# MasterVVK/qwen3-tts-axera-russian

Hardware: AMD Instinct MI355X
Metric: 12Hz codec-tokens/s (codec frames/s, 16 codes each) + RTF, Qwen3-TTS-0.6B (higher is better)
Workload: dtype f16 weights/KV, f32 accumulate (talker+CP); vocoder exact fp32 (f32 MFMA); 1 GPU; configs[2]/[3]: batch=32 mixed ru/en prompts per GPU, 64 frames/utterance/step (prefill + hipGraph decode loop), utterance-sharded DP over 1 GPU(s); batch_per_gpu=32

## Files before the change

### qwen3_tts_axera_russian_amd/csrc/q3_attn.hip

```cpp
#include "q3_kdev.h"

namespace q3 {

template <int MODE, int APRE>
__global__ void __launch_bounds__(1024) attn_kernel(AttnArgs a) {
    constexpr int D = 128;
    Q3_FETCH_ARGS("s"(a.qkv), "s"(a.ld), "s"(a.row0), "s"(a.q_norm), "s"(a.k_norm), "s"(a.eps), "s"(a.rope_cos), "s"(a.rope_sin),
                  "s"(a.slot), "s"(a.pos), "s"(a.slot_base), "s"(a.slot_stride), "s"(a.pos_base), "s"(a.pos_stride), "s"(a.kc),
                  "s"(a.vc), "s"(a.n_ctx), "s"(a.n_kv), "s"(a.n_heads), "s"(a.out), "s"(a.scale), "s"(a.valid_mod), "s"(a.valid_n));
    Q3_TL(30 + MODE);
    const int r = a.row0 + blockIdx.x, g = blockIdx.y;
    if (a.valid_mod > 0 && (r % a.valid_mod) >= a.valid_n) return;
    const int tid = threadIdx.x, lane = tid & 63, w = tid >> 6;
    const int nwv = blockDim.x >> 6;
    const int slot = a.slot ? uniform_load(a.slot + r) : a.slot_base + r * a.slot_stride;
    const int pos = a.pos ? uniform_load(a.pos + r) : a.pos_base + r * a.pos_stride;
    __shared__ float qs[2][D];
    __shared__ float knew[D], vnew[D];
    extern __shared__ __attribute__((aligned(16))) float dyn[];
    float* pm = dyn;
    float* pl = dyn + 2 * nwv;
    float* pacc = dyn + 4 * nwv;
    float* row = a.qkv + (size_t)r * a.ld;
    const size_t cbase = ((size_t)slot * a.n_kv + g) * (size_t)a.n_ctx * D;
    const int T = (MODE == ATTN_FUSED) ? pos : pos + 1;
    const int l16 = tid & 15, grp = tid >> 4, ngrp = blockDim.x >> 4;
    const half_t* kbase = a.kc + cbase;
    const half_t* vbase = a.vc + cbase;

    float x0 = 0.f, x1 = 0.f, gm0 = 1.f, gm1 = 1.f, cs = 1.f, sn = 0.f;
    if (MODE != ATTN_ATTEND && w < 4) {
        const float* src = w < 2 ? row + (size_t)(2 * g + w) * D
                         : w == 2 ? row + (size_t)(a.n_heads + g) * D
                                  : row + (size_t)(a.n_heads + a.n_kv + g) * D;
        x0 = src[lane];
        x1 = src[lane + 64];
        if (w < 3) {
            const float* gam = w < 2 ? a.q_norm : a.k_norm;
            gm0 = gam[lane];
            gm1 = gam[lane + 64];
            cs = a.rope_cos[(size_t)pos * 64 + lane];
            sn = a.rope_sin[(size_t)pos * 64 + lane];
        }
    }
    float qpre = 0.f;
    if (MODE == ATTN_ATTEND && tid < 2 * D) qpre = row[(size_t)(2 * g) * D + tid];
    h8 kpre[APRE], vpre[APRE];
    if (MODE != ATTN_PREP) {
#pragma unroll
        for (int i = 0; i < APRE; i++) {
            const int t = grp + i * ngrp;
            if (t < T) {
                kpre[i] = *(const h8*)(kbase + (size_t)t * D + l16 * 8);
                vpre[i] = *(const h8*)(vbase + (size_t)t * D + l16 * 8);
            }
        }
    }
    __builtin_amdgcn_sched_barrier(0);
    Q3_PH(0);

    if (MODE != ATTN_ATTEND) {
        if (w < 4) {
            if (w < 3) {
                float ss = wave_sum(x0 * x0 + x1 * x1);
                const float iv = 1.0f / sqrtf(ss / (float)D + a.eps);
                x0 = (x0 * iv) * gm0;
                x1 = (x1 * iv) * gm1;
                const float y0 = x0 * cs - x1 * sn;
                const float y1 = x1 * cs + x0 * sn;
                x0 = y0;
                x1 = y1;
            }
            if (w < 2) {
                if (MODE == ATTN_PREP) {
                    float* dst = row + (size_t)(2 * g + w) * D;
                    dst[lane] = x0;
                    dst[lane + 64] = x1;
                } else {
                    qs[w][lane] = x0;
                    qs[w][lane + 64] = x1;
                }
            } else {
                const half_t h0 = sat_half(x0), h1 = sat_half(x1);
                half_t* cd = (w == 2 ? a.kc : a.vc) + cbase + (size_t)pos * D;
                cd[lane] = h0;
                cd[lane + 64] = h1;
                float* nd = w == 2 ? knew : vnew;
                nd[lane] = (float)h0;
                nd[lane + 64] = (float)h1;
            }
        }
        if (MODE == ATTN_PREP) return;
    } else {
        if (tid < 2 * D) qs[tid / D][tid % D] = qpre;
    }
    __syncthreads();
    Q3_PH(1);

    float q0[8], q1[8];
#pragma unroll
    for (int j = 0; j < 8; j++) {
        q0[j] = qs[0][l16 * 8 + j] * a.scale;
        q1[j] = qs[1][l16 * 8 + j] * a.scale;
    }
    float m0 = -INFINITY, m1 = -INFINITY, l0 = 0.f, l1 = 0.f;
    float a0[8], a1[8];
#pragma unroll
    for (int j = 0; j < 8; j++) a0[j] = a1[j] = 0.f;

    auto step = [&](const h8& kk, const h8& vv) {
        float d0 = 0.f, d1 = 0.f;
#pragma unroll
        for (int j = 0; j < 8; j++) {
            const float kf = (float)kk[j];
            d0 += q0[j] * kf;
            d1 += q1[j] * kf;
        }
        group_sum_down2<16>(d0, d1);
        const float n0 = fmaxf(m0, d0), n1 = fmaxf(m1, d1);
        const float c0 = __expf(m0 - n0), c1 = __expf(m1 - n1);
        const float p0 = __expf(d0 - n0), p1 = __expf(d1 - n1);
        l0 = l0 * c0 + p0;
        l1 = l1 * c1 + p1;
#pragma unroll
        for (int j = 0; j < 8; j++) {
            const float vf = (float)vv[j];
            a0[j] = a0[j] * c0 + p0 * vf;
            a1[j] = a1[j] * c1 + p1 * vf;
        }
        m0 = n0;
        m1 = n1;
    };
#pragma unroll
    for (int i = 0; i < APRE; i++) {
        const int t = grp + i * ngrp;
        if (t < T) step(kpre[i], vpre[i]);
    }
#pragma unroll 2
    for (int t = grp + APRE * ngrp; t < T; t += ngrp) {
        const h8 kk = *(const h8*)(kbase + (size_t)t * D + l16 * 8);
        const h8 vv = *(const h8*)(vbase + (size_t)t * D + l16 * 8);
        step(kk, vv);
    }
    if (MODE == ATTN_FUSED && grp == 0) {
        h8 kk, vv;
#pragma unroll
        for (int j = 0; j < 8; j++) {
            kk[j] = (half_t)knew[l16 * 8 + j];
            vv[j] = (half_t)vnew[l16 * 8 + j];
        }
        step(kk, vv);
    }
    asm volatile("" ::"v"(a0[0]), "v"(l0));
    Q3_PH(2);
#pragma unroll
    for (int o = 16; o <= 32; o <<= 1) {
        const float om0 = __shfl_xor(m0, o, 64), om1 = __shfl_xor(m1, o, 64);
        const float ol0 = __shfl_xor(l0, o, 64), ol1 = __shfl_xor(l1, o, 64);
        const float n0 = fmaxf(m0, om0), n1 = fmaxf(m1, om1);
        const float c0 = (m0 == -INFINITY) ? 0.f : __expf(m0 - n0), d0 = (om0 == -INFINITY) ? 0.f : __expf(om0 - n0);
        const float c1 = (m1 == -INFINITY) ? 0.f : __expf(m1 - n1), d1 = (om1 == -INFINITY) ? 0.f : __expf(om1 - n1);
        l0 = l0 * c0 + ol0 * d0;
        l1 = l1 * c1 + ol1 * d1;
#pragma unroll
        for (int j = 0; j < 8; j++) {
            const float oa0 = __shfl_xor(a0[j], o, 64), oa1 = __shfl_xor(a1[j], o, 64);
            a0[j] = a0[j] * c0 + oa0 * d0;
            a1[j] = a1[j] * c1 + oa1 * d1;
        }
        m0 = n0;
        m1 = n1;
    }
    if (lane < 16) {
#pragma unroll
        for (int j = 0; j < 8; j++) {
            pacc[(w * 2 + 0) * D + lane * 8 + j] = a0[j];
            pacc[(w * 2 + 1) * D + lane * 8 + j] = a1[j];
        }
        if (lane == 0) {
            pm[w * 2 + 0] = m0;
            pm[w * 2 + 1] = m1;
            pl[w * 2 + 0] = l0;
            pl[w * 2 + 1] = l1;
        }
    }
    __syncthreads();
    Q3_PH(3);
    if (tid < 2 * D) {
        const int hh = tid / D, d = tid % D;
        float M = -INFINITY;
        for (int i = 0; i < nwv; i++) M = fmaxf(M, pm[i * 2 + hh]);
        float L = 0.f, o = 0.f;
        for (int i = 0; i < nwv; i++) {
            const float mi = pm[i * 2 + hh];
            const float c = (mi == -INFINITY) ? 0.f : __expf(mi - M);
            L += pl[i * 2 + hh] * c;
            o += pacc[(i * 2 + hh) * D + d] * c;
        }
        a.out[frag_idx(r, (2 * g + hh) * D + d, a.n_heads * D)] = sat_half(o / L);
    }
}

constexpr int ATTN_SHORT_MAX_T = 15;
static int g_attn_short = 1;
int set_attn_short(int on) { g_attn_short = on; return 0; }
__global__ void __launch_bounds__(256)
    attn_short_kernel(float* __restrict__ p_qkv, int p_ld, int p_row0, int p_n_heads, int p_n_kv,
                      const float* __restrict__ p_q_norm, const float* __restrict__ p_k_norm,
                      const float* __restrict__ p_rope_cos, const float* __restrict__ p_rope_sin, int p_pos_base,
                      int p_slot_base, AttnArgs a) {
    constexpr int D = 128, NE = ATTN_SHORT_MAX_T + 1;
    a.qkv = p_qkv;
    a.ld = p_ld;
    a.row0 = p_row0;
    a.n_heads = p_n_heads;
    a.n_kv = p_n_kv;
    a.q_norm = p_q_norm;
    a.k_norm = p_k_norm;
    a.rope_cos = p_rope_cos;
    a.rope_sin = p_rope_sin;
    a.pos_base = p_pos_base;
    a.slot_base = p_slot_base;
    Q3_FETCH_ARGS("s"(a.eps), "s"(a.slot), "s"(a.slot_stride), "s"(a.kc), "s"(a.vc), "s"(a.n_ctx), "s"(a.out), "s"(a.scale));
    Q3_TL(33);
    const int r = a.row0 + blockIdx.x, g = blockIdx.y;
    const int tid = threadIdx.x, lane = tid & 63, w = tid >> 6;
    const int slot = a.slot ? uniform_load(a.slot + r) : a.slot_base + r * a.slot_stride;
    const int T = a.pos_base;
    __shared__ float qs[2][D];
    __shared__ float knew[D];
    __shared__ __attribute__((aligned(16))) half_t vs[NE][D];
    __shared__ __attribute__((aligned(16))) float sc[2][NE];
    float* row = a.qkv + (size_t)r * a.ld;
    const size_t cbase = ((size_t)slot * a.n_kv + g) * (size_t)a.n_ctx * D;
    const int l16 = tid & 15, grp = tid >> 4;
    const int hh = tid >> 7, d = tid & 127;
    float x0 = 0.f, x1 = 0.f, gm0 = 1.f, gm1 = 1.f, cs = 1.f, sn = 0.f;
    {
        const float* src = w < 2 ? row + (size_t)(2 * g + w) * D
                         : w == 2 ? row + (size_t)(a.n_heads + g) * D
                                  : row + (size_t)(a.n_heads + a.n_kv + g) * D;
        x0 = src[lane];
        x1 = src[lane + 64];
        if (w < 3) {
            const float* gam = w < 2 ? a.q_norm : a.k_norm;
            gm0 = gam[lane];
            gm1 = gam[lane + 64];
            cs = a.rope_cos[(size_t)T * 64 + lane];
            sn = a.rope_sin[(size_t)T * 64 + lane];
        }
    }
    h8 kpre, vpre;
    if (grp < T) {
        kpre = *(const h8*)(a.kc + cbase + (size_t)grp * D + l16 * 8);
        vpre = *(const h8*)(a.vc + cbase + (size_t)grp * D + l16 * 8);
    }
    __builtin_amdgcn_sched_barrier(0);
    Q3_PH(0);
    if (w < 3) {
        float ss = wave_sum(x0 * x0 + x1 * x1);
        const float iv = 1.0f / sqrtf(ss / (float)D + a.eps);
        x0 = (x0 * iv) * gm0;
        x1 = (x1 * iv) * gm1;
        const float y0 = x0 * cs - x1 * sn;
        const float y1 = x1 * cs + x0 * sn;
        x0 = y0;
        x1 = y1;
    }
    if (w < 2) {
        qs[w][lane] = x0;
        qs[w][lane + 64] = x1;
    } else {
        const half_t h0 = sat_half(x0), h1 = sat_half(x1);
        half_t* cd = (w == 2 ? a.kc : a.vc) + cbase + (size_t)T * D;
        cd[lane] = h0;
        cd[lane + 64] = h1;
        if (w == 2) {
            knew[lane] = (float)h0;
            knew[lane + 64] = (float)h1;
        } else {
            vs[T][lane] = h0;
            vs[T][lane + 64] = h1;
        }
    }
    if (grp < T) *(h8*)(&vs[grp][l16 * 8]) = vpre;
    __syncthreads();
    Q3_PH(1);
    if (grp <= T) {
        float d0 = 0.f, d1 = 0.f;
#pragma unroll
        for (int j = 0; j < 8; j++) {
            const float kf = grp < T ? (float)kpre[j] : knew[l16 * 8 + j];
            d0 += (qs[0][l16 * 8 + j] * a.scale) * kf;
            d1 += (qs[1][l16 * 8 + j] * a.scale) * kf;
        }
        group_sum_down2<16>(d0, d1);
        if (l16 == 0) {
            sc[0][grp] = d0;
            sc[1][grp] = d1;
        }
    }
    __syncthreads();
    Q3_PH(2);
    float sv[NE];
#pragma unroll
    for (int e4 = 0; e4 < NE; e4 += 4) {
        const float4 t4 = *(const float4*)(&sc[hh][e4]);
        sv[e4] = t4.x;
        sv[e4 + 1] = t4.y;
        sv[e4 + 2] = t4.z;
        sv[e4 + 3] = t4.w;
    }
    float m = -INFINITY;
#pragma unroll
    for (int e = 0; e < NE; e++) m = fmaxf(m, e <= T ? sv[e] : -INFINITY);
    float L = 0.f, o = 0.f;
#pragma unroll
    for (int e = 0; e < NE; e++) {
        const float p = e <= T ? __expf(sv[e] - m) : 0.f;
        const float vf = e <= T ? (float)vs[e][d] : 0.f;
        L += p;
        o += p * vf;
    }
    Q3_PH(3);
    a.out[frag_idx(r, (2 * g + hh) * D + d, a.n_heads * D)] = sat_half(o / L);
}

__global__ void __launch_bounds__(256) attn_tile_mfma_kernel(AttnArgs a) {
    constexpr int D = 128, QP = 136, VP = 72, CH = 64;
    constexpr float LO = 2048.0f, ILO = 1.0f / 2048.0f;
    Q3_TL(35);
    const int g = blockIdx.y, tid = threadIdx.x, lane = tid & 63, w = tid >> 6;
    const int c = lane & 15, q4 = lane >> 4;
    int row0, nrows, slot, pos0;
    if (a.tiles) {
        const int4 t = *(const int4*)(a.tiles + 4 * blockIdx.x);
        row0 = t.x; nrows = t.y; slot = t.z; pos0 = t.w;
    } else {
        row0 = a.row0 + blockIdx.x * 16;
        nrows = a.R - blockIdx.x * 16 < 16 ? a.R - blockIdx.x * 16 : 16;
        slot = a.slot_base;
        pos0 = a.pos_base + blockIdx.x * 16;
    }
    extern __shared__ __attribute__((aligned(16))) char smem[];
    half_t* qh = (half_t*)smem;
    half_t* ql = qh + 32 * QP;
    half_t* ks = ql + 32 * QP;
    half_t* vs = ks + CH * QP;
    half_t* ph = vs + CH * QP;
    half_t* pl = ph + 32 * VP;
    float* red = (float*)(pl + 32 * VP);
    float* red2 = red + 4 * 32;
    const size_t cbase = ((size_t)slot * a.n_kv + g) * (size_t)a.n_ctx * D;
    const int T = pos0 + nrows;
    h8 kreg[4], vreg[4];
    auto load_chunk = [&](int c0) {
#pragma unroll
        for (int it = 0; it < 4; it++) {
            const int idx = tid + it * 256, kr = idx >> 4, d8 = (idx & 15) * 8;
            kreg[it] = vreg[it] = (h8){0, 0, 0, 0, 0, 0, 0, 0};
            if (c0 + kr < T) {
                kreg[it] = *(const h8*)(a.kc + cbase + (size_t)(c0 + kr) * D + d8);
                vreg[it] = *(const h8*)(a.vc + cbase + (size_t)(c0 + kr) * D + d8);
            }
        }
    };
    auto store_chunk = [&]() {
#pragma unroll
        for (int it = 0; it < 4; it++) {
            const int idx = tid + it * 256, kr = idx >> 4, d8 = (idx & 15) * 8;
            *(h8*)(ks + kr * QP + d8) = kreg[it];
            *(h8*)(vs + kr * QP + d8) = vreg[it];
        }
    };
    load_chunk(0);
    for (int idx = tid; idx < 32 * (D / 8); idx += 256) {
        const int qr = idx / (D / 8), d8 = (idx - qr * (D / 8)) * 8, i = qr & 15, hh = qr >> 4;
        h8 hi = {0, 0, 0, 0, 0, 0, 0, 0}, lo = hi;
        if (i < nrows) {
            const float* src = a.qkv + (size_t)(row0 + i) * a.ld + (size_t)(2 * g + hh) * D + d8;
            const float4 v0 = *(const float4*)src, v1 = *(const float4*)(src + 4);
            const float e[8] = {v0.x, v0.y, v0.z, v0.w, v1.x, v1.y, v1.z, v1.w};
#pragma unroll
            for (int j = 0; j < 8; j++) {
                const float x = e[j] * a.scale;
                hi[j] = sat_half(x);
                lo[j] = (half_t)((x - (float)hi[j]) * LO);
            }
        }
        *(h8*)(qh + qr * QP + d8) = hi;
        *(h8*)(ql + qr * QP + d8) = lo;
    }
    float mrow[2][4], lrow[2][4];
    f4 oh[2][2], ol[2][2];
#pragma unroll
    for (int qb = 0; qb < 2; qb++)
#pragma unroll
        for (int r = 0; r < 4; r++) {
            mrow[qb][r] = -INFINITY;
            lrow[qb][r] = 0.f;
        }
#pragma unroll
    for (int qb = 0; qb < 2; qb++)
#pragma unroll
        for (int j = 0; j < 2; j++) oh[qb][j] = ol[qb][j] = (f4){0.f, 0.f, 0.f, 0.f};
    for (int c0 = 0; c0 < T; c0 += CH) {
        __syncthreads();
        store_chunk();
        if (c0 + CH < T) load_chunk(c0 + CH);
        __syncthreads();
        f4 sh[2], sl[2];
        sh[0] = sh[1] = sl[0] = sl[1] = (f4){0.f, 0.f, 0.f, 0.f};
#pragma unroll
        for (int kb = 0; kb < 4; kb++) {
            const h8 bk = *(const h8*)(ks + (16 * w + c) * QP + kb * 32 + q4 * 8);
#pragma unroll
            for (int qb = 0; qb < 2; qb++) {
                const h8 ahi = *(const h8*)(qh + (16 * qb + c) * QP + kb * 32 + q4 * 8);
                const h8 alo = *(const h8*)(ql + (16 * qb + c) * QP + kb * 32 + q4 * 8);
                sh[qb] = __builtin_amdgcn_mfma_f32_16x16x32_f16(ahi, bk, sh[qb], 0, 0, 0);
                sl[qb] = __builtin_amdgcn_mfma_f32_16x16x32_f16(alo, bk, sl[qb], 0, 0, 0);
            }
        }
        const int key = c0 + 16 * w + c;
        float sc[2][4], mx[2][4];
#pragma unroll
        for (int qb = 0; qb < 2; qb++)
#pragma unroll
            for (int r = 0; r < 4; r++) {
                const int i = 4 * q4 + r;
                float v = sh[qb][r] + sl[qb][r] * ILO;
                if (!(i < nrows && key <= pos0 + i)) v = -INFINITY;
                sc[qb][r] = v;
                const float x = group_max_up<16>(v);
                mx[qb][r] = x;
                if (c == 0) red[w * 32 + 16 * qb + i] = x;
            }
        __syncthreads();
        float corr[2][4];
#pragma unroll
        for (int qb = 0; qb < 2; qb++)
#pragma unroll
            for (int r = 0; r < 4; r++) {
                const int qr = 16 * qb + 4 * q4 + r;
                const float cm = fmaxf(fmaxf(red[qr], red[32 + qr]), fmaxf(red[64 + qr], red[96 + qr]));
                const float mo = mrow[qb][r], mn = fmaxf(mo, cm);
                corr[qb][r] = (mo == -INFINITY) ? 0.f : __expf(mo - mn);
                const float p = (sc[qb][r] == -INFINITY) ? 0.f : __expf(sc[qb][r] - mn);
                const half_t hi = (half_t)p;
                ph[qr * VP + 16 * w + c] = hi;
                pl[qr * VP + 16 * w + c] = (half_t)((p - (float)hi) * LO);
                const float ssum = group_sum_up<16>(p);
                if (c == 0) red2[w * 32 + qr] = ssum;
                mrow[qb][r] = mn;
            }
        __syncthreads();
#pragma unroll
        for (int qb = 0; qb < 2; qb++)
#pragma unroll
            for (int r = 0; r < 4; r++) {
                const int qr = 16 * qb + 4 * q4 + r;
                lrow[qb][r] = lrow[qb][r] * corr[qb][r] + ((red2[qr] + red2[32 + qr]) + (red2[64 + qr] + red2[96 + qr]));
#pragma unroll
                for (int j = 0; j < 2; j++) {
                    oh[qb][j][r] *= corr[qb][r];
                    ol[qb][j][r] *= corr[qb][r];
                }
            }
#pragma unroll
        for (int kst = 0; kst < 2; kst++) {
#pragma unroll
            for (int j = 0; j < 2; j++) {
                typedef __fp16 hv4 __attribute__((__vector_size__(4 * sizeof(__fp16))));
                const half_t* vb = vs + (kst * 32 + 8 * q4 + (c >> 2)) * QP + 32 * w + 16 * j + 4 * (c & 3);
                const hv4 t0 = __builtin_amdgcn_ds_read_tr16_b64_v4f16((__attribute__((address_space(3))) hv4*)vb);
                const hv4 t1 = __builtin_amdgcn_ds_read_tr16_b64_v4f16((__attribute__((address_space(3))) hv4*)(vb + 4 * QP));
                h8 bv;
#pragma unroll
                for (int e = 0; e < 4; e++) {
                    bv[e] = (half_t)t0[e];
                    bv[4 + e] = (half_t)t1[e];
                }
#pragma unroll
                for (int qb = 0; qb < 2; qb++) {
                    const h8 ahi = *(const h8*)(ph + (16 * qb + c) * VP + kst * 32 + q4 * 8);
                    const h8 alo = *(const h8*)(pl + (16 * qb + c) * VP + kst * 32 + q4 * 8);
                    oh[qb][j] = __builtin_amdgcn_mfma_f32_16x16x32_f16(ahi, bv, oh[qb][j], 0, 0, 0);
                    ol[qb][j] = __builtin_amdgcn_mfma_f32_16x16x32_f16(alo, bv, ol[qb][j], 0, 0, 0);
                }
            }
        }
    }
#pragma unroll
    for (int qb = 0; qb < 2; qb++)
#pragma unroll
        for (int r = 0; r < 4; r++) {
            const int i = 4 * q4 + r;
            if (i < nrows) {
                const float inv = 1.0f / lrow[qb][r];
#pragma unroll
                for (int j = 0; j < 2; j++) {
                    const float o = (oh[qb][j][r] + ol[qb][j][r] * ILO) * inv;
                    a.out[frag_idx(row0 + i, (2 * g + qb) * D + 32 * w + 16 * j + c, a.n_heads * D)] = sat_half(o);
                }
            }
        }
}

int launch_attn(hipStream_t s, const AttnArgs& a, int mode) {
    if (a.R <= 0) return 0;
    if (a.n_heads != 2 * a.n_kv) {
        Q3_LOG("attn: only GQA group 2 (16q/8kv) is built, got %d/%d", a.n_heads, a.n_kv);
        return -1;
    }
    if (g_attn_short && mode == ATTN_FUSED && !a.pos && a.pos_stride == 0 && a.pos_base >= 0 &&
        a.pos_base <= ATTN_SHORT_MAX_T && a.pos_base < a.n_ctx) {
        AttnArgs a3 = a;
        a3.tl_node = tl_next_node();
        hipLaunchKernelGGL(attn_short_kernel, dim3(a.R, a.n_kv), dim3(256), 0, s, a3.qkv, a3.ld, a3.row0, a3.n_heads, a3.n_kv,
                           a3.q_norm, a3.k_norm, a3.rope_cos, a3.rope_sin, a3.pos_base, a3.slot_base, a3);
        Q3_HIP(hipGetLastError(), -1);
        return 0;
    }
    if (mode == ATTN_ATTEND && a.n_tiles > 0) {
        constexpr size_t lds = (size_t)(2 * 32 * 136 + 2 * 64 * 136 + 2 * 32 * 72) * 2 + 8 * 32 * 4;
        static bool attr = false;
        if (!attr) {
            Q3_HIP(hipFuncSetAttribute((const void*)attn_tile_mfma_kernel, hipFuncAttributeMaxDynamicSharedMemorySize, (int)lds), -1);
            attr = true;
        }
        AttnArgs a5 = a;
        a5.tl_node = tl_next_node();
        hipLaunchKernelGGL(attn_tile_mfma_kernel, dim3(a.n_tiles, a.n_kv), dim3(256), lds, s, a5);
        Q3_HIP(hipGetLastError(), -1);
        return 0;
    }
    int threads = a.threads;
    const int fit = 65536 / (a.R * a.n_kv);
    if (threads > fit) threads = fit / 64 * 64;
    if (threads < 256) threads = 256;
    if (threads > 1024) threads = 1024;
    const size_t lds = ((size_t)(threads / 64) * (4 + 2 * 128)) * sizeof(float);
    AttnArgs a2 = a;
    a2.tl_node = tl_next_node();
    dim3 grid(a.R, a.n_kv);
#define Q3_ATTN(MODE_)                                                                                   \
    {                                                                                                    \
        if (threads <= 256)                                                                              \
            hipLaunchKernelGGL((attn_kernel<MODE_, 8>), grid, dim3(256), mode == ATTN_PREP ? 0 : lds, s, a2); \
        else                                                                                             \
            hipLaunchKernelGGL((attn_kernel<MODE_, 4>), grid, dim3(mode == ATTN_PREP ? 256 : threads),   \
                               mode == ATTN_PREP ? 0 : lds, s, a2);                                      \
    }
    if (mode == ATTN_FUSED) Q3_ATTN(ATTN_FUSED)
    else if (mode == ATTN_PREP) Q3_ATTN(ATTN_PREP)
    else Q3_ATTN(ATTN_ATTEND)
#undef Q3_ATTN
    Q3_HIP(hipGetLastError(), -1);
    return 0;
}

}
```

### qwen3_tts_axera_russian_amd/csrc/q3_cp.h

```cpp
#pragma once
#include "q3_model.h"

namespace q3 {

struct CpFrameIO {
    int* codes = nullptr;
    const int* n_frames = nullptr;
    int frame_cap = 1;
    float* fb_h = nullptr;
    float* fb_ssq = nullptr;
    half_t* fb_xh = nullptr;
    const float* fb_gamma = nullptr;
    const float* pad_embed = nullptr;
    const float* text_rows = nullptr;
    const int* text_avail = nullptr;
    int text_cap = 0;
    const int* held = nullptr;
    float temperature = 0.f;
    int top_k = 50;
    unsigned long long seed = 0;
    const unsigned long long* seed_ptr = nullptr;
    const int* forced = nullptr;
    const SlotParams* slots = nullptr;
    const SlotRules* rules = nullptr;
    float* scores = nullptr;
};

int cp_seed_row0(const Work& w, int R, int row0 = 0, int R_total = 0);
int cp_frame(hipStream_t s, const Model& m, Work& w, KVCache& kv, int R, const CpFrameIO& io, int row0 = 0,
             int R_total = 0);

}
```

### qwen3_tts_axera_russian_amd/csrc/q3_cp_api.hip

```cpp
#include "../../include/qwen3tts_cp.h"
#include "q3_cp.h"

namespace q3 {

static bool two_row_enabled() {
    static const bool on = !(getenv("Q3_CP_TWO_ROW") && atoi(getenv("Q3_CP_TWO_ROW")) == 0);
    return on;
}

int cp_seed_row0(const Work& w, int R, int row0, int R_total) {
    (void)R;
    (void)row0;
    if (R_total <= 0) R_total = R;
    const int B16 = (R_total + 15) / 16 * 16;
    const bool two = two_row_enabled() && 2 * B16 <= w.max_rows;
    return two ? B16 : 0;
}

int cp_frame(hipStream_t s, const Model& m, Work& w, KVCache& kv, int R, const CpFrameIO& io, int row0, int R_total) {
    const ModelCfg& c = m.cfg;
    if (R_total <= 0) R_total = R;
    const int H = c.hidden, G = c.cp_groups;
    const int seed0 = cp_seed_row0(w, R, row0, R_total);
    RowMap rm;
    rm.slot_base = 0;
    rm.slot_stride = 1;
    rm.pos_stride = 0;
    if (seed0 > 0 && (row0 != 0 || R_total != R)) {
        RowMap r0;
        r0.slot_base = -seed0;
        r0.slot_stride = 1;
        r0.pos_base = 0;
        r0.pos_stride = 0;
        r0.same_slot_rows = true;
        if (run_stack(s, m, m.cp, w, kv, R, r0, 256, seed0 + row0)) return -1;
        if (launch_gather_embed(s, m.talker_emb, c.talker_vocab, H, io.codes, 0, io.n_frames, io.frame_cap, 0, w.h, w.ssq, R,
                                row0, R_total, io.forced, w.xh, m.cp.L[0].in_ln))
            return -1;
        RowMap r1 = rm;
        r1.pos_base = 1;
        r1.same_slot_rows = true;
        if (run_stack(s, m, m.cp, w, kv, R, r1, 256, row0)) return -1;
    } else if (seed0 > 0) {
        const int R16 = seed0;
        if (w.map_R16 != R16) {
            std::vector<int> slot(2 * R16), pos(2 * R16);
            for (int i = 0; i < 2 * R16; i++) {
                slot[i] = i % R16;
                pos[i] = i < R16 ? 1 : 0;
            }
            Q3_HIP(hipMemcpyAsync(w.map_slot, slot.data(), sizeof(int) * 2 * R16, hipMemcpyHostToDevice, s), -1);
            Q3_HIP(hipMemcpyAsync(w.map_pos, pos.data(), sizeof(int) * 2 * R16, hipMemcpyHostToDevice, s), -1);
            Q3_HIP(hipStreamSynchronize(s), -1);
            w.map_R16 = R16;
        }
        if (launch_gather_embed(s, m.talker_emb, c.talker_vocab, H, io.codes, 0, io.n_frames, io.frame_cap, 0, w.h, w.ssq, R,
                                row0, R_total, io.forced, w.xh, m.cp.L[0].in_ln))
            return -1;
        RowMap r2;
        r2.slot = w.map_slot;
        r2.pos = w.map_pos;
        r2.same_slot_rows = true;
        r2.valid_mod = R16;
        r2.valid_n = R;
        if (run_stack(s, m, m.cp, w, kv, R16 + R, r2, 256, 0)) return -1;
    } else {
        rm.pos_base = 0;
        if (run_stack(s, m, m.cp, w, kv, R, rm, 256, row0)) return -1;
        if (launch_gather_embed(s, m.talker_emb, c.talker_vocab, H, io.codes, 0, io.n_frames, io.frame_cap, 0, w.h, w.ssq, R,
                                row0, R_total, io.forced, w.xh, m.cp.L[0].in_ln))
            return -1;
        rm.pos_base = 1;
        if (run_stack(s, m, m.cp, w, kv, R, rm, 256, row0)) return -1;
    }
    const bool qkv_tab = m.cp_qkv_serves(R);
    for (int g = 0; g < G; g++) {
        if (g > 0) {
            rm.pos_base = g + 1;
            rm.skip_qkv0 = qkv_tab;
            if (run_stack(s, m, m.cp, w, kv, R, rm, 256, row0)) return -1;
        }
        LinArgs a;
        a.wp = m.cp_head[g].wp;
        a.N = c.cp_vocab;
        a.K = H;
        a.M = row0 + R;
        a.m_begin = row0;
        a.nt = 0;
        a.x16 = w.xh;
        a.ssq = w.ssq;
        a.ssq_parts = H / 16;
        a.eps = c.eps;
        a.y = w.logits;
        a.ldy = c.cp_vocab;
        if (launch_linear(s, a, PRO_NORM, EPI_STORE)) return -1;
        CpArgmaxArgs x;
        x.logits = w.logits;
        x.V = c.cp_vocab;
        x.R = R;
        x.row0 = row0;
        x.R_total = R_total;
        x.H = H;
        x.group = g;
        x.codes = io.codes;
        x.n_frames = io.n_frames;
        x.frame_cap = io.frame_cap;
        x.temperature = io.temperature;
        x.top_k = io.top_k;
        x.seed = io.seed;
        x.seed_ptr = io.seed_ptr;
        x.forced = io.forced;
        x.slots = io.slots;
        x.held = io.held;
        x.rules = io.rules;
        x.scores = io.scores;
        if (g + 1 < G) {
            x.next_table = m.cp_emb[g];
            x.h_out = w.h;
            x.ssq_out = w.ssq;
            x.xh_out = w.xh;
            x.gamma_next = m.cp.L[0].in_ln;
            if (qkv_tab) {
                x.next_qkv = m.cp_qkv_rows(g);
                x.qkv_out = w.qkv;
                x.qkv_ld = (c.n_heads + 2 * c.n_kv) * c.head_dim;
            }
        } else if (io.fb_h) {
            x.talker_emb = m.talker_emb;
            x.talker_vocab = c.talker_vocab;
            x.cp_tables = m.d_cp_emb_ptrs;
            x.pad_embed = io.pad_embed;
            x.text_rows = io.text_rows;
            x.text_avail = io.text_avail;
            x.text_cap = io.text_cap;
            x.n_groups = G;
            x.h_out = io.fb_h;
            x.ssq_out = io.fb_ssq;
            x.xh_out = io.fb_xh;
            x.gamma_next = io.fb_gamma;
        }
        if (launch_cp_argmax(s, x)) return -1;
    }
    return 0;
}

}

using namespace q3;

namespace {

struct CpHandle {
    Model* m = nullptr;
    int max_batch = 1;
    KVCache kv;
    Work w;
    hipStream_t s = nullptr;
    int *d_codes = nullptr, *d_nframes = nullptr;
    std::vector<int> h_codes;
    GraphExec graph;
    int graph_rows = 0;
    int step_next_pos = 0;
};

}

extern "C" {

void* cp_load(const char* weights, const char* embeddings_dir, int max_batch) {
    if (!weights) return nullptr;
    if (max_batch <= 0) max_batch = 1;
    hipStream_t s = nullptr;
    if (hipStreamCreate(&s) != hipSuccess) return nullptr;
    Model* m = model_load(weights, false, true, embeddings_dir, s);
    if (!m) {
        hipStreamDestroy(s);
        return nullptr;
    }
    CpHandle* h = new CpHandle();
    h->m = m;
    h->s = s;
    h->max_batch = max_batch;
    const ModelCfg& c = m->cfg;
    bool ok = kv_alloc(h->kv, c.cp_layers, max_batch, c.n_kv, c.cp_groups + 1, h->s) == 0;
    ok = ok && work_alloc(h->w, c, 2 * ((max_batch + 15) / 16 * 16), c.cp_ffn, c.cp_vocab, h->s) == 0;
    ok = ok && hipMalloc((void**)&h->d_codes, sizeof(int) * 16 * max_batch) == hipSuccess;
    ok = ok && hipMalloc((void**)&h->d_nframes, sizeof(int) * max_batch) == hipSuccess;
    if (ok) {
        std::vector<int> ones(max_batch, 1);
        ok = hipMemcpyAsync(h->d_nframes, ones.data(), sizeof(int) * max_batch, hipMemcpyHostToDevice, h->s) == hipSuccess &&
             hipStreamSynchronize(h->s) == hipSuccess;
    }
    if (!ok) {
        Q3_LOG("cp_load: allocation failed");
        cp_free(h);
        return nullptr;
    }
    h->h_codes.resize((size_t)16 * max_batch);
    return h;
}

void cp_free(void* hh) {
    CpHandle* h = (CpHandle*)hh;
    if (!h) return;
    if (h->s) hipStreamSynchronize(h->s);
    h->graph.reset();
    kv_free(h->kv);
    work_free(h->w);
    if (h->d_codes) hipFree(h->d_codes);
    if (h->d_nframes) hipFree(h->d_nframes);
    if (h->s) hipStreamDestroy(h->s);
    model_free(h->m);
    delete h;
}

int cp_hidden_size(void* hh) {
    CpHandle* h = (CpHandle*)hh;
    return h ? h->m->cfg.hidden : 0;
}

int cp_predict_batch(void* hh, const float* hidden, const int32_t* code_0, int n_rows, float temperature, int top_k,
                     uint64_t seed, int32_t* out_codes) {
    CpHandle* h = (CpHandle*)hh;
    if (!h || !hidden || !code_0 || !out_codes || n_rows <= 0 || n_rows > h->max_batch) return -1;
    const bool stochastic = temperature > 1e-6f;
    const Model& m = *h->m;
    const int H = m.cfg.hidden, G = m.cfg.cp_groups, R = n_rows;
    for (int r = 0; r < R; r++) {
        h->h_codes[(size_t)r * 16] = code_0[r];
        for (int j = 1; j < 16; j++) h->h_codes[(size_t)r * 16 + j] = -1;
    }
    Q3_HIP(hipMemcpyAsync(h->d_codes, h->h_codes.data(), sizeof(int) * 16 * R, hipMemcpyHostToDevice, h->s), -1);
    Q3_HIP(hipMemcpyAsync(h->w.rows_in, hidden, sizeof(float) * (size_t)R * H, hipMemcpyHostToDevice, h->s), -1);
    CpFrameIO io;
    io.codes = h->d_codes;
    io.n_frames = h->d_nframes;
    io.frame_cap = 1;
    io.temperature = temperature;
    io.top_k = top_k;
    io.seed = seed;
    auto body = [&]() -> int {
        if (launch_ssq_rows(h->s, h->w.rows_in, h->w.h, h->w.ssq, R, H, h->w.xh, m.cp.L[0].in_ln,
                            cp_seed_row0(h->w, R)))
            return -1;
        return cp_frame(h->s, m, h->w, h->kv, R, io);
    };
    if (stochastic) {
        if (body()) return -1;
    } else if (!h->graph.e || h->graph_rows != R) {
        if (body()) return -1;
        Q3_HIP(hipStreamSynchronize(h->s), -1);
        if (h->graph.capture(h->s, hipStreamCaptureModeThreadLocal, "cp_predict", body)) return -1;
        h->graph_rows = R;
    } else {
        Q3_HIP(hipGraphLaunch(h->graph.e, h->s), -1);
    }
    Q3_HIP(hipMemcpyAsync(h->h_codes.data(), h->d_codes, sizeof(int) * 16 * R, hipMemcpyDeviceToHost, h->s), -1);
    Q3_HIP(hipStreamSynchronize(h->s), -1);
    for (int r = 0; r < R; r++)
        for (int g = 0; g < G; g++) out_codes[(size_t)r * G + g] = h->h_codes[(size_t)r * 16 + 1 + g];
    return 0;
}

int cp_predict(void* hh, const float* hidden, int32_t code_0, float temperature, int top_k, uint64_t seed,
               int32_t* out_codes) {
    return cp_predict_batch(hh, hidden, &code_0, 1, temperature, top_k, seed, out_codes);
}

int cp_step(void* hh, const float* embed, int position, float* out_hidden) {
    CpHandle* h = (CpHandle*)hh;
    if (!h || !embed || !out_hidden) return -1;
    const Model& m = *h->m;
    const int H = m.cfg.hidden;
    if (position < 0 || position > m.cfg.cp_groups) return -1;
    Q3_HIP(hipMemcpyAsync(h->w.rows_in, embed, sizeof(float) * H, hipMemcpyHostToDevice, h->s), -1);
    if (launch_ssq_rows(h->s, h->w.rows_in, h->w.h, h->w.ssq, 1, H, h->w.xh, m.cp.L[0].in_ln)) return -1;
    RowMap rm;
    rm.pos_base = position;
    if (run_stack(h->s, m, m.cp, h->w, h->kv, 1, rm, 256)) return -1;
    FinalNormArgs f;
    f.h = h->w.h;
    f.ssq = h->w.ssq;
    f.ssq_parts = H / 16;
    f.gamma = m.cp.final_norm;
    f.eps = m.cfg.eps;
    f.R = 1;
    f.H = H;
    f.out_f32 = h->w.hidden_f32;
    if (launch_final_norm(h->s, f)) return -1;
    Q3_HIP(hipMemcpyAsync(out_hidden, h->w.hidden_f32, sizeof(float) * H, hipMemcpyDeviceToHost, h->s), -1);
    Q3_HIP(hipStreamSynchronize(h->s), -1);
    return 0;
}

int cp_lm_head(void* hh, int group, const float* hidden, float* logits_out) {
    CpHandle* h = (CpHandle*)hh;
    if (!h || !hidden || !logits_out) return -1;
    const Model& m = *h->m;
    const int H = m.cfg.hidden, V = m.cfg.cp_vocab;
    if (group < 0 || group >= m.cfg.cp_groups) return -1;
    std::vector<uint16_t> h16((size_t)16 * H, 0);
    for (int i = 0; i < H; i++) h16[frag_idx(0, i, H)] = f2h_sat(hidden[i]);
    Q3_HIP(hipMemcpyAsync(h->w.hidden_f16, h16.data(), h16.size() * 2, hipMemcpyHostToDevice, h->s), -1);
    LinArgs a;
    a.wp = m.cp_head[group].wp;
    a.N = V;
    a.K = H;
    a.M = 1;
    a.x16 = h->w.hidden_f16;
    a.y = h->w.logits;
    a.ldy = V;
    if (launch_linear(h->s, a, PRO_F16, EPI_STORE)) return -1;
    Q3_HIP(hipMemcpyAsync(logits_out, h->w.logits, sizeof(float) * V, hipMemcpyDeviceToHost, h->s), -1);
    Q3_HIP(hipStreamSynchronize(h->s), -1);
    return V;
}

}
```

### qwen3_tts_axera_russian_amd/csrc/q3_engine.hip

```cpp
#include "../../include/qwen3tts_engine.h"
#include "q3_cp.h"
#include "q3_engine_host.h"

#include <algorithm>
#include <chrono>
#include <cmath>
#include <memory>
#include <tuple>

using namespace q3;

namespace {

struct Sampling {
    float t_temp = 0.f, t_top_p = 0.95f, c_temp = 0.f;
    int t_top_k = 50, c_top_k = 50;
};
struct FrameState {
    int B = 0, ignore_eos = 0, cap_frames = 0, chains = 0;
    int text_cap = 0;
    Sampling smp;
    unsigned long long seed = 0;
    const int* forced = nullptr;
    const SlotParams* slots = nullptr;
    const float* text_rows = nullptr;
    const int* text_avail = nullptr;
    int* held = nullptr;
    const SlotRules* rules = nullptr;
    unsigned* seen = nullptr;
    float* scores = nullptr;
    auto key() const {
        return std::tie(B, ignore_eos, cap_frames, chains, text_cap, smp.t_temp, smp.t_top_p, smp.c_temp, smp.t_top_k, smp.c_top_k,
                        seed, forced, slots, text_rows, text_avail, held, rules, seen, scores);
    }
    bool operator==(const FrameState& o) const { return key() == o.key(); }
};
static_assert(sizeof(FrameState) == 10 * 4 + 8 + 8 * sizeof(void*), "FrameState: a new field belongs in key() too");

struct TextRows {
    DeviceAllocs mem;
    float* rows = nullptr;
    int* avail = nullptr;
    int* held = nullptr;
    int cap = 0;
    bool hold = false;
};
struct RuleSets {
    DeviceAllocs mem;
    SlotRules* rules = nullptr;
    unsigned* seen = nullptr;
    int seen_words = 0;
    std::vector<SlotRules> defaults;
};
struct Scores {
    DeviceAllocs mem;
    PinnedAllocs pin;
    float* d = nullptr;
    float* h = nullptr;
};
struct PrefixPool {
    DeviceAllocs mem;
    half_t* kv = nullptr;
    float* state = nullptr;
};

struct Engine {
    Model* m = nullptr;
    int max_batch = 0, n_ctx = 0, max_frames = 0;
    hipStream_t s = nullptr;
    KVCache kv_t, kv_c;
    Work wt, wc;
    int prefill_rows = 0;
    DeviceAllocs mem;
    PinnedAllocs pin;
    int *d_slot = nullptr, *d_pos = nullptr;
    int* d_tiles = nullptr;
    int* d_prompt = nullptr;
    int *d_iota = nullptr;
    int *d_past = nullptr, *d_npast = nullptr, *d_ntext = nullptr, *d_done = nullptr, *d_nframes = nullptr;
    int *d_pos0 = nullptr, *d_posdec = nullptr, *d_lastrow = nullptr;
    int* d_codes = nullptr;
    int* d_forced = nullptr;
    bool forced_on = false;
    unsigned long long* d_seed = nullptr;
    unsigned long long n_requests = 0, req_seed = 0, n_refills = 0;
    float* d_pad = nullptr;
    int B = 0, ignore_eos = 0;
    GraphExec graph[8];
    FrameState captured;
    hipEvent_t ev0 = nullptr, ev1 = nullptr;
    float last_run_ms = 0.f, last_prefill_ms = 0.f, last_host_launch_ms = 0.f;
    int* h_done = nullptr;
    int* h_read = nullptr;
    Sampling smp;
    unsigned long long seed = 0;
    int n_chains = 1;
    bool use_prio = false;
    int prio_hi = 0;
    hipStream_t cs[8] = {nullptr};
    hipEvent_t ev_fork = nullptr, ev_join[8] = {nullptr};
    bool slot_mode = false;
    SlotParams* d_slots = nullptr;
    SlotBook book;
    std::vector<SlotParams> h_sp;
    int up_i[2] = {0, 0};
    std::unique_ptr<TextRows> text;
    std::unique_ptr<RuleSets> rules;
    std::unique_ptr<Scores> scores;
    std::unique_ptr<PrefixPool> pool;
    PrefixIndex pfx;
    size_t pfx_entry_elems() const { return (size_t)kv_t.n_layers * 2 * kv_t.n_kv * pfx.max_rows() * 128; }

    int cap_frames = 0, frames_run = 0;
    int frames_hi = 0;
    bool hold() const { return text && text->hold; }
    int frames_recorded() const { return std::min(slot_mode ? book.frames_hi() : frames_hi, max_frames); }
    int generated(int b, int n_past) const { return slot_mode ? book.generated(b, n_past) : n_past; }
    int budget(int b) const { return slot_mode ? book[b].budget : cap_frames; }
    int room() const { return slot_mode ? book.room(hold(), max_frames) : std::min(cap_frames, max_frames) - frames_run; }
    void advance(int steps) {
        if (slot_mode) return book.advance(steps, hold(), max_frames);
        frames_run += steps;
        frames_hi += steps;
    }

    int chains_eff() const {
        const int nc = n_chains < 1 ? 1 : n_chains;
        return (nc > 1 && B % (16 * nc) == 0) ? nc : 1;
    }
    FrameState frame_state() const {
        FrameState f;
        f.B = B;
        f.ignore_eos = ignore_eos;
        f.cap_frames = cap_frames;
        f.chains = chains_eff();
        f.smp = smp;
        f.seed = seed;
        f.forced = forced_on ? d_forced : nullptr;
        if (slot_mode) {
            f.slots = d_slots;
            if (text) {
                f.text_rows = text->rows;
                f.text_avail = text->avail;
                f.text_cap = text->cap;
                if (text->hold) f.held = text->held;
            }
            if (rules) {
                f.rules = rules->rules;
                f.seen = rules->seen;
            }
        }
        if (scores) f.scores = scores->d;
        return f;
    }
};

unsigned long long mix_seed(unsigned long long seed, unsigned long long k, unsigned long long golden) {
    unsigned long long z = seed + golden * k;
    z = (z ^ (z >> 30)) * 0xBF58476D1CE4E5B9ull;
    z = (z ^ (z >> 27)) * 0x94D049BB133111EBull;
    return z ^ (z >> 31);
}

int talker_final_norm(Engine* e, hipStream_t st, int row0, int R, const int* row_map, int copy_row_off) {
    const Model& m = *e->m;
    const int H = m.cfg.hidden;
    FinalNormArgs f;
    f.h = e->wt.h;
    f.ssq = e->wt.ssq;
    f.ssq_parts = H / 16;
    f.gamma = m.talker.final_norm;
    f.eps = m.cfg.eps;
    f.R = R;
    f.row0 = row0;
    f.H = H;
    f.row_map = row_map;
    f.out_f32 = e->wt.hidden_f32;
    f.out_f16 = e->wt.hidden_f16;
    f.out_copy = e->wc.h;
    f.out_copy_ssq = e->wc.ssq;
    f.out_copy_xh = e->wc.xh;
    f.out_copy_gamma = m.cp.L[0].in_ln;
    f.out_copy_row_off = copy_row_off;
    return launch_final_norm(st, f);
}

int codec_head(Engine* e, hipStream_t st, int row0, int R) {
    const Model& m = *e->m;
    LinArgs a;
    a.wp = m.talker_head.wp;
    a.N = m.cfg.talker_vocab;
    a.K = m.cfg.hidden;
    a.M = row0 + R;
    a.m_begin = row0;
    a.nt = 1;
    a.x16 = e->wt.hidden_f16;
    a.y = e->wt.logits;
    a.ldy = m.cfg.talker_vocab;
    return launch_linear(st, a, PRO_F16, EPI_STORE);
}

int frame_chain(Engine* e, const FrameState& f, hipStream_t st, int row0, int R) {
    const Model& m = *e->m;
    TalkerSampleArgs sa;
    sa.logits = e->wt.logits;
    sa.V = m.cfg.talker_vocab;
    sa.R = R;
    sa.row0 = row0;
    sa.R_total = f.B;
    sa.audio_vocab = m.cfg.cp_vocab;
    sa.eos = m.cfg.codec_eos;
    sa.past = e->d_past;
    sa.n_past = e->d_npast;
    sa.n_text = e->d_ntext;
    sa.done = e->d_done;
    sa.codes = e->d_codes;
    sa.n_frames = e->d_nframes;
    sa.frame_cap = e->max_frames;
    sa.pos0 = e->d_pos0;
    sa.pos = e->d_posdec;
    sa.ignore_eos = f.ignore_eos;
    sa.max_frames = f.cap_frames;
    sa.temperature = f.smp.t_temp;
    sa.top_k = f.smp.t_top_k;
    sa.top_p = f.smp.t_top_p;
    sa.seed = f.seed;
    sa.seed_ptr = e->d_seed;
    sa.forced = f.forced;
    sa.slots = f.slots;
    sa.text_avail = f.held ? f.text_avail : nullptr;
    sa.held = f.held;
    sa.rules = f.rules;
    sa.seen = f.seen;
    sa.scores = f.scores;
    if (launch_talker_sample(st, sa)) return -1;
    CpFrameIO io;
    io.codes = e->d_codes;
    io.n_frames = e->d_nframes;
    io.frame_cap = e->max_frames;
    io.fb_h = e->wt.h;
    io.fb_ssq = e->wt.ssq;
    io.fb_xh = e->wt.xh;
    io.fb_gamma = m.talker.L[0].in_ln;
    io.pad_embed = e->d_pad;
    io.text_rows = f.text_rows;
    io.text_avail = f.text_avail;
    io.text_cap = f.text_cap;
    io.held = f.held;
    io.temperature = f.smp.c_temp;
    io.top_k = f.smp.c_top_k;
    io.seed = f.seed ^ 0x5851F42D4C957F2Dull;
    io.seed_ptr = e->d_seed;
    io.forced = f.forced;
    io.slots = f.slots;
    io.rules = f.rules;
    io.scores = f.scores;
    if (cp_frame(st, m, e->wc, e->kv_c, R, io, row0, f.B)) return -1;
    RowMap rm;
    rm.slot_base = 0;
    rm.slot_stride = 1;
    rm.pos = e->d_posdec;
    rm.rows_total = f.B;
    if (run_stack(st, m, m.talker, e->wt, e->kv_t, R, rm, 1024, row0)) return -1;
    return talker_final_norm(e, st, row0, R, nullptr, cp_seed_row0(e->wc, R, row0, f.B)) || codec_head(e, st, row0, R) ? -1 : 0;
}

void chain_rows(const Engine* e, int c, int& row0, int& R) {
    const int nc = e->chains_eff();
    row0 = 0;
    for (int i = 0; i < c; i++) row0 += e->B / nc + (i < e->B % nc ? 1 : 0);
    R = e->B / nc + (c < e->B % nc ? 1 : 0);
}

bool make_stream(const Engine* e, hipStream_t* st) {
    return (e->use_prio ? hipStreamCreateWithPriority(st, hipStreamNonBlocking, e->prio_hi)
                        : hipStreamCreateWithFlags(st, hipStreamNonBlocking)) == hipSuccess;
}

int ensure_chains(Engine* e, int n) {
    if (n < 2) return 0;
    if (!e->ev_fork) Q3_HIP(hipEventCreateWithFlags(&e->ev_fork, hipEventDisableTiming), -1);
    for (int c = 0; c < n; c++) {
        if (!e->cs[c] && !make_stream(e, &e->cs[c])) return -1;
        if (!e->ev_join[c]) Q3_HIP(hipEventCreateWithFlags(&e->ev_join[c], hipEventDisableTiming), -1);
    }
    return 0;
}

hipStream_t chain_stream(const Engine* e, int c) { return e->chains_eff() == 1 ? e->s : e->cs[c]; }

int frame_eager(Engine* e, const FrameState& f) {
    for (int c = 0; c < f.chains; c++) {
        int row0, R;
        chain_rows(e, c, row0, R);
        if (frame_chain(e, f, chain_stream(e, c), row0, R)) return -1;
    }
    return 0;
}

int fork_chains(Engine* e) {
    const int nc = e->chains_eff();
    if (nc == 1) return 0;
    Q3_HIP(hipEventRecord(e->ev_fork, e->s), -1);
    for (int c = 0; c < nc; c++) Q3_HIP(hipStreamWaitEvent(e->cs[c], e->ev_fork, 0), -1);
    return 0;
}
int join_chains(Engine* e) {
    const int nc = e->chains_eff();
    if (nc == 1) return 0;
    for (int c = 0; c < nc; c++) {
        Q3_HIP(hipEventRecord(e->ev_join[c], e->cs[c]), -1);
        Q3_HIP(hipStreamWaitEvent(e->s, e->ev_join[c], 0), -1);
    }
    return 0;
}

template <class F>
int timed_prefill(Engine* e, F&& body) {
    Q3_HIP(hipEventRecord(e->ev0, e->s), -1);
    if (body()) return -1;
    Q3_HIP(hipEventRecord(e->ev1, e->s), -1);
    Q3_HIP(hipStreamSynchronize(e->s), -1);
    hipEventElapsedTime(&e->last_prefill_ms, e->ev0, e->ev1);
    return 0;
}

}

extern "C" {

void q3e_free(void* ee) {
    Engine* e = (Engine*)ee;
    if (!e) return;
    if (e->s) hipStreamSynchronize(e->s);
    for (auto& g : e->graph) g.reset();
    kv_free(e->kv_t);
    kv_free(e->kv_c);
    work_free(e->wt);
    work_free(e->wc);
    for (int c = 0; c < 8; c++) {
        if (e->cs[c]) hipStreamDestroy(e->cs[c]);
        if (e->ev_join[c]) hipEventDestroy(e->ev_join[c]);
    }
    if (e->ev_fork) hipEventDestroy(e->ev_fork);
    if (e->ev0) hipEventDestroy(e->ev0);
    if (e->ev1) hipEventDestroy(e->ev1);
    if (e->s) hipStreamDestroy(e->s);
    if (e->m) model_free(e->m);
    delete e;
}

void* q3e_create(const char* weights, int max_batch, int n_ctx, int max_frames) {
    if (!weights || max_batch <= 0 || n_ctx <= 0 || max_frames <= 0) return nullptr;
    Engine* e = new Engine();
    int prio_lo = 0, prio_hi = 0;
    e->use_prio = !(getenv("Q3_STREAM_PRIO") && atoi(getenv("Q3_STREAM_PRIO")) == 0) &&
                  hipDeviceGetStreamPriorityRange(&prio_lo, &prio_hi) == hipSuccess && prio_lo != prio_hi;
    e->prio_hi = prio_hi;
    if (!make_stream(e, &e->s)) {
        Q3_LOG("q3e_create: no stream");
        q3e_free(e);
        return nullptr;
    }
    Model* m = model_load(weights, true, true, nullptr, e->s);
    if (!m) {
        q3e_free(e);
        return nullptr;
    }
    e->m = m;
    if (n_ctx > m->max_pos) {
        Q3_LOG("q3e_create: n_ctx=%d exceeds the RoPE table (%d)", n_ctx, m->max_pos);
        q3e_free(e);
        return nullptr;
    }
    e->max_batch = max_batch;
    e->n_ctx = n_ctx;
    e->max_frames = max_frames;
    const ModelCfg& c = m->cfg;
    e->prefill_rows = max_batch > 2048 ? max_batch : 2048;
    bool ok = hipEventCreate(&e->ev0) == hipSuccess && hipEventCreate(&e->ev1) == hipSuccess;
    if (const char* nc = getenv("Q3_CHAINS")) e->n_chains = atoi(nc) < 1 ? 1 : atoi(nc) > 8 ? 8 : atoi(nc);
    else e->n_chains = 1;
    ok = ok && ensure_chains(e, e->n_chains) == 0;
    ok = ok && kv_alloc(e->kv_t, c.talker_layers, max_batch, c.n_kv, n_ctx, e->s) == 0;
    ok = ok && kv_alloc(e->kv_c, c.cp_layers, max_batch, c.n_kv, c.cp_groups + 1, e->s) == 0;
    ok = ok && work_alloc(e->wt, c, e->prefill_rows, c.talker_ffn, c.talker_vocab, e->s) == 0;
    ok = ok && work_alloc(e->wc, c, 2 * ((max_batch + 15) / 16 * 16), c.cp_ffn, c.cp_vocab, e->s) == 0;
    const size_t mb = max_batch, pr = e->prefill_rows;
    const std::pair<int**, size_t> ints[] = {
        {&e->d_slot, pr},   {&e->d_pos, pr},   {&e->d_tiles, 4 * pr}, {&e->d_prompt, 16 * pr}, {&e->d_iota, mb},
        {&e->d_past, 32 * mb}, {&e->d_npast, mb}, {&e->d_ntext, mb}, {&e->d_done, mb}, {&e->d_nframes, mb},
        {&e->d_pos0, mb},   {&e->d_posdec, mb}, {&e->d_lastrow, mb},   {&e->d_codes, 16 * mb * max_frames}};
    for (const auto& a : ints) ok = ok && e->mem.alloc(a.first, sizeof(int) * a.second);
    ok = ok && e->mem.alloc_zeroed(&e->d_pad, sizeof(float) * c.hidden, e->s);
    ok = ok && e->mem.alloc_zeroed(&e->d_seed, sizeof(unsigned long long) * mb, e->s);
    ok = ok && e->pin.alloc(&e->h_done, sizeof(int) * mb) && e->pin.alloc(&e->h_read, sizeof(int) * (mb + 16 * mb * max_frames));
    if (ok) {
        std::vector<int> iota(max_batch);
        for (int i = 0; i < max_batch; i++) iota[i] = i;
        ok = hipMemcpyAsync(e->d_iota, iota.data(), sizeof(int) * max_batch, hipMemcpyHostToDevice, e->s) == hipSuccess;
        ok = hipStreamSynchronize(e->s) == hipSuccess && ok;
    }
    if (!ok) {
        Q3_LOG("q3e_create: allocation failed");
        q3e_free(e);
        return nullptr;
    }
    return e;
}

int q3e_set_sampling(void* ee, float talker_temperature, int talker_top_k, float talker_top_p, float cp_temperature,
                     int cp_top_k, uint64_t seed) {
    Engine* e = (Engine*)ee;
    if (!e) return -1;
    e->smp = {talker_temperature, talker_top_p, cp_temperature, talker_top_k, cp_top_k};
    e->seed = seed;
    e->n_requests = 0;
    return 0;
}

int q3e_set_forced_codes(void* ee, const int32_t* forced, int n_frames) {
    Engine* e = (Engine*)ee;
    if (!e) return -1;
    const bool on = forced != nullptr && n_frames > 0;
    if (on && e->slot_mode) {
        Q3_LOG("q3e_set_forced_codes: not for a per-slot batch (q3e_open)");
        return -1;
    }
    if (on) {
        if (e->B <= 0 || n_frames > e->max_frames) return -1;
        const size_t total = (size_t)e->max_frames * e->max_batch * 16;
        if (!e->d_forced && !e->mem.alloc(&e->d_forced, sizeof(int) * total)) {
            Q3_LOG("q3e_set_forced_codes: allocation of %zu bytes failed", sizeof(int) * total);
            return -1;
        }
        Q3_HIP(hipMemsetAsync(e->d_forced, 0xff, sizeof(int) * total, e->s), -1);
        Q3_HIP(hipMemcpyAsync(e->d_forced, forced, sizeof(int) * 16 * (size_t)e->B * n_frames, hipMemcpyHostToDevice, e->s), -1);
        Q3_HIP(hipStreamSynchronize(e->s), -1);
    }
    e->forced_on = on;
    return 0;
}

int q3e_set_chains(void* ee, int n) {
    Engine* e = (Engine*)ee;
    if (!e || n < 1 || n > 8) return -1;
    if (n != e->n_chains) {
        if (ensure_chains(e, n)) return -1;
        e->n_chains = n;
    }
    return 0;
}

int q3e_set_pad_embed(void* ee, const float* pad) {
    Engine* e = (Engine*)ee;
    if (!e || !pad) return -1;
    Q3_HIP(hipMemcpyAsync(e->d_pad, pad, sizeof(float) * e->m->cfg.hidden, hipMemcpyHostToDevice, e->s), -1);
    Q3_HIP(hipStreamSynchronize(e->s), -1);
    return 0;
}

static int prefill_final_norm(Engine* e, int row0, int R, int B_total) {
    return talker_final_norm(e, e->s, row0, R, e->d_lastrow, cp_seed_row0(e->wc, B_total, 0, B_total));
}

static int prompt_launch(Engine* e, int slot, int T, int row0, bool rows) {
    const Model& m = *e->m;
    PromptRowsArgs a;
    a.codes = e->d_prompt;
    a.T = T;
    a.past = e->d_past + 32 * (size_t)slot;
    a.n_past = e->d_npast + slot;
    a.talker_emb = m.talker_emb;
    a.talker_vocab = m.cfg.talker_vocab;
    a.cp_tables = m.d_cp_emb_ptrs;
    a.cp_vocab = m.cfg.cp_vocab;
    a.n_groups = m.cfg.cp_groups;
    a.pad_embed = e->d_pad;
    if (e->rules) {
        a.seen = e->rules->seen + (size_t)(slot < 0 ? 0 : slot) * e->rules->seen_words;
        a.seen_vocab = m.cfg.cp_vocab;
    }
    if (rows) {
        a.h = e->wt.h;
        a.ssq = e->wt.ssq;
        a.xh = e->wt.xh;
        a.gamma = m.talker.L[0].in_ln;
        a.row0 = row0;
        a.max_rows = e->prefill_rows;
        a.H = m.cfg.hidden;
    }
    if (slot < 0 || slot >= e->max_batch || T > e->prefill_rows) return -1;
    return launch_prompt_rows(e->s, a);
}

static int prefill_ids(Engine* e, int n, const int* ids, const float* prefix, const int32_t* n_rows, int B_total, int n_prompt = 0) {
    if (n_prompt && (n != 1 || n_prompt >= n_rows[0])) return -1;
    const Model& m = *e->m;
    const int H = m.cfg.hidden;
    size_t row_off = 0;
    int u0 = 0;
    std::vector<int> slot, pos, tiles, last(n);
    while (u0 < n) {
        int u1 = u0, rows = 0;
        while (u1 < n && rows + n_rows[u1] <= e->prefill_rows) rows += n_rows[u1++];
        slot.resize(rows);
        pos.resize(rows);
        int r = 0;
        tiles.clear();
        bool contiguous = true;
        for (int u = u0; u < u1; u++) {
            const int b = ids[u];
            if (u > u0 && b != ids[u - 1] + 1) contiguous = false;
            for (int i = 0; i < n_rows[u]; i += 16) {
                const int nn = n_rows[u] - i < 16 ? n_rows[u] - i : 16;
                const int t4[4] = {r + i, nn, b, i};
                tiles.insert(tiles.end(), t4, t4 + 4);
            }
            for (int i = 0; i < n_rows[u]; i++, r++) {
                slot[r] = b;
                pos[r] = i;
            }
            last[u] = r - 1;
        }
        const int up_rows = rows - n_prompt;
        Q3_HIP(hipMemcpyAsync(e->wt.rows_in, prefix + row_off * H, sizeof(float) * (size_t)up_rows * H, hipMemcpyHostToDevice, e->s), -1);
        Q3_HIP(hipMemcpyAsync(e->d_slot, slot.data(), sizeof(int) * rows, hipMemcpyHostToDevice, e->s), -1);
        Q3_HIP(hipMemcpyAsync(e->d_pos, pos.data(), sizeof(int) * rows, hipMemcpyHostToDevice, e->s), -1);
        Q3_HIP(hipMemcpyAsync(e->d_tiles, tiles.data(), sizeof(int) * tiles.size(), hipMemcpyHostToDevice, e->s), -1);
        if (contiguous) {
            Q3_HIP(hipMemcpyAsync(e->d_lastrow + ids[u0], last.data() + u0, sizeof(int) * (u1 - u0), hipMemcpyHostToDevice, e->s), -1);
        } else {
            for (int u = u0; u < u1; u++)
// ... 701 lines not shown
```

### qwen3_tts_axera_russian_amd/csrc/q3_kernels.h

```cpp
#pragma once
#include "q3_common.h"
#include "q3_frag.h"

namespace q3 {

enum { PRO_F16 = 0, PRO_NORM = 1 };
enum { EPI_STORE = 0, EPI_RESID = 1, EPI_SWIGLU = 2 };

struct LinArgs {
    int tl_node = -1;
    const half_t* wp = nullptr;
    int N = 0, K = 0, M = 0;
    int m_begin = 0;
    int swap_grid = 0;
    int nt = 0;
    const half_t* x16 = nullptr;
    const float* ssq = nullptr;
    int ssq_parts = 0;
    float eps = 1e-6f;
    float* y = nullptr;
    int ldy = 0;
    float* h_out = nullptr;
    float* ssq_out = nullptr;
    half_t* xh_out = nullptr;
    const float* gamma = nullptr;
    half_t* act = nullptr;
};
int launch_linear(hipStream_t s, const LinArgs& a, int pro, int epi);
int linear_decode_kbw(int K, int N, int rows);

int launch_pack_linear(hipStream_t s, const half_t* src, int N, int K, half_t* dst, int tile_off,
                       int tile_stride);

enum { ATTN_FUSED = 0, ATTN_PREP = 1, ATTN_ATTEND = 2 };
struct AttnArgs {
    int tl_node = -1;
    float* qkv = nullptr;
    int ld = 0, R = 0, row0 = 0;
    const float* q_norm = nullptr;
    const float* k_norm = nullptr;
    float eps = 1e-6f;
    const float* rope_cos = nullptr;
    const float* rope_sin = nullptr;
    const int* slot = nullptr;
    const int* pos = nullptr;
    int slot_base = 0, slot_stride = 0, pos_base = 0, pos_stride = 0;
    half_t* kc = nullptr;
    half_t* vc = nullptr;
    int n_ctx = 0, n_kv = 0, n_heads = 0;
    half_t* out = nullptr;
    float scale = 0.f;
    int threads = 256;
    int valid_mod = 0, valid_n = 0;
    const int* tiles = nullptr;
    int n_tiles = 0;
};
int launch_attn(hipStream_t s, const AttnArgs& a, int mode);

int launch_ssq_rows(hipStream_t s, const float* rows, float* h, float* ssq, int R, int H, half_t* xh = nullptr,
                    const float* gamma = nullptr, int dst_row0 = 0);

struct FinalNormArgs {
    int tl_node = -1;
    const float* h = nullptr;
    const float* ssq = nullptr;
    int ssq_parts = 0;
    const float* gamma = nullptr;
    float eps = 1e-6f;
    int R = 0, H = 0, row0 = 0;
    const int* row_map = nullptr;
    int src_off = 0;
    float* out_f32 = nullptr;
    half_t* out_f16 = nullptr;
    float* out_copy = nullptr;
    float* out_copy_ssq = nullptr;
    int out_copy_row_off = 0;
    half_t* out_copy_xh = nullptr;
    const float* out_copy_gamma = nullptr;
};
int launch_final_norm(hipStream_t s, const FinalNormArgs& a);

int launch_gather_embed(hipStream_t s, const float* table, int V, int H, const int* tok, int tok_stride,
                        const int* n_frames, int frame_cap, int col, float* h, float* ssq, int R, int row0 = 0,
                        int R_total = 0, const int* forced = nullptr, half_t* xh = nullptr, const float* gamma = nullptr);

struct PrefixMoveArgs {
    half_t* kc = nullptr;
    half_t* vc = nullptr;
    size_t layer_stride = 0;
    int n_layers = 0, n_kv = 0, n_ctx = 0;
    int slot = 0, n_rows = 0;
    half_t* entry = nullptr;
    int max_rows = 0;
    float* state = nullptr;
    float* h = nullptr;
    float* ssq = nullptr;
    int h_row = 0, H = 0;
    int restore = 0;
};
int launch_prefix_move(hipStream_t s, const PrefixMoveArgs& a);

struct SlotParams {
    int max_frames = 0;
    float t_temp = 0.f;
    int t_top_k = 0;
    float t_top_p = 1.f;
    float c_temp = 0.f;
    int c_top_k = 0;
    unsigned long long seed = 0;
    int no_row = 1;
    int flags = 0;
    int prompt = 0;
};

struct SlotRules {
    float rep_penalty = 1.2f;
    int rep_window = 30;
    float eos_boost = 15.f;
    float eos_force = 2.f;
    int min_past = 0;
    float cp_top_p = 1.f;
};

struct TalkerSampleArgs {
    int tl_node = -1;
    const float* logits = nullptr;
    int V = 0, R = 0, row0 = 0, R_total = 0;
    int audio_vocab = 2048, eos = 2150;
    int* past = nullptr;
    int* n_past = nullptr;
    const int* n_text = nullptr;
    int* done = nullptr;
    int* codes = nullptr;
    int* n_frames = nullptr;
    int frame_cap = 0;
    const int* pos0 = nullptr;
    int* pos = nullptr;
    int ignore_eos = 0;
    int max_frames = 0;
    float rep_penalty = 1.2f;
    float temperature = 0.f, top_p = 0.95f;
    int top_k = 50;
    unsigned long long seed = 0;
    const unsigned long long* seed_ptr = nullptr;
    const int* forced = nullptr;
    const SlotParams* slots = nullptr;
    const int* text_avail = nullptr;
    int* held = nullptr;
    const SlotRules* rules = nullptr;
    unsigned* seen = nullptr;
    float* scores = nullptr;
};
int launch_talker_sample(hipStream_t s, const TalkerSampleArgs& a);

struct CpArgmaxArgs {
    int tl_node = -1;
    const float* logits = nullptr;
    int V = 0, R = 0, H = 0, row0 = 0, R_total = 0;
    int group = 0;
    int* codes = nullptr;
    const int* n_frames = nullptr;
    int frame_cap = 0;
    const float* next_table = nullptr;
    float* h_out = nullptr;
    float* ssq_out = nullptr;
    half_t* xh_out = nullptr;
    const float* gamma_next = nullptr;
    const float* next_qkv = nullptr;
    float* qkv_out = nullptr;
    int qkv_ld = 0;
    const float* talker_emb = nullptr;
    int talker_vocab = 0;
    const float* const* cp_tables = nullptr;
    const float* pad_embed = nullptr;
    int n_groups = 15;
    float temperature = 0.f;
    int top_k = 50;
    unsigned long long seed = 0;
    const unsigned long long* seed_ptr = nullptr;
    const int* forced = nullptr;
    const SlotParams* slots = nullptr;
    const float* text_rows = nullptr;
    const int* text_avail = nullptr;
    int text_cap = 0;
    const int* held = nullptr;
    const SlotRules* rules = nullptr;
    float* scores = nullptr;
};
int launch_cp_argmax(hipStream_t s, const CpArgmaxArgs& a);

int launch_feedback(hipStream_t s, const int* codes16, int R, const float* talker_emb, int talker_vocab,
                    const float* const* cp_tables, int cp_vocab, int n_groups, const float* pad_embed,
                    float* h_out, float* ssq_out, int H, half_t* xh_out = nullptr, const float* gamma = nullptr);

struct PromptRowsArgs {
    const int* codes = nullptr;
    int T = 0;
    int* past = nullptr;
    int* n_past = nullptr;
    unsigned* seen = nullptr;
    int seen_vocab = 0;
    const float* talker_emb = nullptr;
    int talker_vocab = 0;
    const float* const* cp_tables = nullptr;
    int cp_vocab = 0, n_groups = 15;
    const float* pad_embed = nullptr;
    float* h = nullptr;
    float* ssq = nullptr;
    half_t* xh = nullptr;
    const float* gamma = nullptr;
    int row0 = 0, max_rows = 0, H = 0;
};
int launch_prompt_rows(hipStream_t s, const PromptRowsArgs& a);

int tl_next_node();

int set_linear_tuning(int K, int mt16, int kbw);
int set_linear_split_rows(int on);
int set_linear_narrow8(int on);
int set_linear_wide_tiles(int on);
int set_attn_short(int on);
int set_gemm_min_rows(int n);
int set_gemm_glds(int on);
int reset_linear_knobs();
const char* last_linear_variant();

}
```

### qwen3_tts_axera_russian_amd/csrc/q3_model.h

```cpp
#pragma once
#include "q3_kernels.h"

namespace q3 {

struct DevLinear {
    half_t* wp = nullptr;
    int N = 0, K = 0;
};

struct DevLayer {
    DevLinear qkv, o, gu, down;
    float *in_ln = nullptr, *post_ln = nullptr, *q_norm = nullptr, *k_norm = nullptr;
};

struct DevStack {
    std::vector<DevLayer> L;
    float* final_norm = nullptr;
    const float* tail_gamma = nullptr;
    int ffn = 0;
    int nt = 0;
    size_t weight_bytes = 0;
};

struct Model {
    ModelCfg cfg;
    int device = 0;
    bool has_talker = false, has_cp = false;
    DevStack talker, cp;
    float* talker_emb = nullptr;
    DevLinear talker_head;
    std::vector<float*> cp_emb;
    std::vector<DevLinear> cp_head;
    const float** d_cp_emb_ptrs = nullptr;
    float* cp_qkv_tab = nullptr;
    int cp_qkv_kbw = 0;
    const float* cp_qkv_rows(int group) const {
        return cp_qkv_tab + (size_t)group * cfg.cp_vocab * ((cfg.n_heads + 2 * cfg.n_kv) * cfg.head_dim);
    }
    bool cp_qkv_serves(int rows) const {
        return cp_qkv_tab && linear_decode_kbw(cfg.hidden, (cfg.n_heads + 2 * cfg.n_kv) * cfg.head_dim, rows) == cp_qkv_kbw;
    }
    float *rope_cos = nullptr, *rope_sin = nullptr;
    int max_pos = 0;
    std::vector<void*> allocs;
    size_t device_bytes = 0;
};

Model* model_load(const char* path, bool want_talker, bool want_cp, const char* aux_dir = nullptr, hipStream_t s = nullptr);
void model_free(Model* m);

int launch_dequant(hipStream_t s, uint32_t type, const uint8_t* blocks, size_t n_rows, size_t K, half_t* out_f16, float* out_f32,
                   int* flag);

struct KVCache {
    half_t *k = nullptr, *v = nullptr;
    int n_layers = 0, n_slots = 0, n_kv = 0, n_ctx = 0, head_dim = 128;
    size_t layer_stride() const { return (size_t)n_slots * n_kv * n_ctx * head_dim; }
    size_t bytes() const { return layer_stride() * n_layers * sizeof(half_t) * 2; }
};
int kv_alloc(KVCache& kv, int n_layers, int n_slots, int n_kv, int n_ctx, hipStream_t s = nullptr);
void kv_free(KVCache& kv);
int kv_zero(hipStream_t s, KVCache& kv);

struct Work {
    int max_rows = 0, hidden = 0;
    float* rows_in = nullptr;
    float *h = nullptr, *ssq = nullptr, *qkv = nullptr;
    half_t* xh = nullptr;
    half_t *attn = nullptr, *act = nullptr;
    float* hidden_f32 = nullptr;
    half_t* hidden_f16 = nullptr;
    float* logits = nullptr;
    int *map_slot = nullptr, *map_pos = nullptr;
    int map_R16 = 0;
};
int work_alloc(Work& w, const ModelCfg& c, int max_rows, int ffn, int max_vocab, hipStream_t s = nullptr);
void work_free(Work& w);
int work_zero(hipStream_t s, Work& w, const ModelCfg& c, int ffn, int max_vocab);

struct RowMap {
    const int* slot = nullptr;
    const int* pos = nullptr;
    int slot_base = 0, slot_stride = 0, pos_base = 0, pos_stride = 0;
    bool same_slot_rows = false;
    int valid_mod = 0, valid_n = 0;
    const int* tiles = nullptr;
    int n_tiles = 0;
    bool skip_qkv0 = false;
    int rows_total = 0;
};

int run_stack(hipStream_t s, const Model& m, const DevStack& st, Work& w, KVCache& kv, int R,
              const RowMap& rm, int attn_threads, int row0 = 0);

struct GraphExec {
    hipGraph_t g = nullptr;
    hipGraphExec_t e = nullptr;
    void reset();
    template <class F>
    int capture(hipStream_t s, hipStreamCaptureMode mode, const char* who, F&& body) {
        reset();
        Q3_HIP(hipStreamBeginCapture(s, mode), -1);
        return end_capture(s, body(), who);
    }

private:
    int end_capture(hipStream_t s, int body_rc, const char* who);
};

}
```

### qwen3_tts_axera_russian_amd/csrc/q3_model.hip

```cpp
#include "q3_model.h"

#include <cmath>

namespace q3 {

namespace {

struct Loader {
    Model* m;
    const Pack& p;
    hipStream_t s = nullptr;
    half_t* stage = nullptr;
    size_t stage_elems = 0;
    std::vector<uint16_t> host16;
    uint8_t* raw = nullptr;
    size_t raw_bytes = 0;
    hipEvent_t dq_ev[2] = {nullptr, nullptr};
    int dq_launches = 0;
    float dq_ms = 0.f;
    size_t dq_bytes = 0;
    bool ok = true;

    bool up(void* d, const void* src, size_t bytes) {
        return hipMemcpyAsync(d, src, bytes, hipMemcpyHostToDevice, s) == hipSuccess && hipStreamSynchronize(s) == hipSuccess;
// ... 270 lines not shown
        if (!m->talker_emb) {
            Q3_LOG("weight file lacks talker.codec_embedding (code_0 embedding of the code predictor)");
            L.ok = false;
        }
        if (L.ok) L.build_cp_qkv_table();
        m->has_cp = L.ok;
    }
    if (L.ok) {
        m->max_pos = 8192;
        const int half = c.head_dim / 2;
        std::vector<float> cs((size_t)m->max_pos * half), sn((size_t)m->max_pos * half);
        for (int i = 0; i < half; i++) {
            const float inv_freq = 1.0f / powf((float)c.rope_theta, (float)(2 * i) / (float)c.head_dim);
            for (int pos = 0; pos < m->max_pos; pos++) {
                const float ang = (float)pos * inv_freq;
                cs[(size_t)pos * half + i] = cosf(ang);
                sn[(size_t)pos * half + i] = sinf(ang);
            }
        }
        m->rope_cos = (float*)L.dalloc(cs.size() * 4);
        m->rope_sin = (float*)L.dalloc(sn.size() * 4);
        if (L.ok) {
            if (!L.up(m->rope_cos, cs.data(), cs.size() * 4)) L.ok = false;
            if (!L.up(m->rope_sin, sn.data(), sn.size() * 4)) L.ok = false;
        }
    }
    hipStreamSynchronize(L.s);
    if (L.stage) hipFree(L.stage);
    if (L.raw) hipFree(L.raw);
    for (hipEvent_t e : L.dq_ev)
        if (e) hipEventDestroy(e);
    if (L.dq_launches && L.ok)
        Q3_LOG("%s: %d quantised tensors (%.1f MB of blocks) dequantised on the GPU: %d launches, %.3f ms of GPU time", path,
               L.dq_launches, L.dq_bytes / 1e6, L.dq_launches, L.dq_ms);
    if (!stream) hipStreamDestroy(L.s);
    if (!L.ok) {
        model_free(m);
        return nullptr;
    }
    return m;
}

void model_free(Model* m) {
    if (!m) return;
    for (void* d : m->allocs) hipFree(d);
    delete m;
}

int kv_alloc(KVCache& kv, int n_layers, int n_slots, int n_kv, int n_ctx, hipStream_t s) {
    kv.n_layers = n_layers;
    kv.n_slots = n_slots;
    kv.n_kv = n_kv;
    kv.n_ctx = n_ctx;
    const size_t bytes = kv.layer_stride() * n_layers * sizeof(half_t);
    Q3_HIP(hipMalloc((void**)&kv.k, bytes), -1);
    Q3_HIP(hipMalloc((void**)&kv.v, bytes), -1);
    Q3_HIP(hipMemsetAsync(kv.k, 0, bytes, s), -1);
    Q3_HIP(hipMemsetAsync(kv.v, 0, bytes, s), -1);
    Q3_HIP(hipStreamSynchronize(s), -1);
    return 0;
}
void kv_free(KVCache& kv) {
    if (kv.k) hipFree(kv.k);
    if (kv.v) hipFree(kv.v);
    kv.k = kv.v = nullptr;
}

int kv_zero(hipStream_t s, KVCache& kv) {
    const size_t bytes = kv.layer_stride() * kv.n_layers * sizeof(half_t);
    Q3_HIP(hipMemsetAsync(kv.k, 0, bytes, s), -1);
    Q3_HIP(hipMemsetAsync(kv.v, 0, bytes, s), -1);
    return 0;
}

int work_zero(hipStream_t s, Work& w, const ModelCfg& c, int ffn, int max_vocab) {
    const size_t R = (size_t)w.max_rows;
    const int qkv_ld = (c.n_heads + 2 * c.n_kv) * c.head_dim;
    Q3_HIP(hipMemsetAsync(w.rows_in, 0, R * c.hidden * 4, s), -1);
    Q3_HIP(hipMemsetAsync(w.h, 0, R * c.hidden * 4, s), -1);
    Q3_HIP(hipMemsetAsync(w.ssq, 0, R * (c.hidden / 16) * 4, s), -1);
    Q3_HIP(hipMemsetAsync(w.xh, 0, R * c.hidden * 2, s), -1);
    Q3_HIP(hipMemsetAsync(w.qkv, 0, R * qkv_ld * 4, s), -1);
    Q3_HIP(hipMemsetAsync(w.attn, 0, R * c.n_heads * c.head_dim * 2, s), -1);
    Q3_HIP(hipMemsetAsync(w.act, 0, R * ffn * 2, s), -1);
    Q3_HIP(hipMemsetAsync(w.hidden_f32, 0, R * c.hidden * 4, s), -1);
    Q3_HIP(hipMemsetAsync(w.hidden_f16, 0, R * c.hidden * 2, s), -1);
    Q3_HIP(hipMemsetAsync(w.logits, 0, R * max_vocab * 4, s), -1);
    return 0;
}

int work_alloc(Work& w, const ModelCfg& c, int max_rows, int ffn, int max_vocab, hipStream_t s) {
    max_rows = (max_rows + 127) / 128 * 128;
    w.max_rows = max_rows;
    w.hidden = c.hidden;
    const size_t R = (size_t)max_rows;
    const int qkv_ld = (c.n_heads + 2 * c.n_kv) * c.head_dim;
    Q3_HIP(hipMalloc((void**)&w.rows_in, R * c.hidden * 4), -1);
    Q3_HIP(hipMalloc((void**)&w.h, R * c.hidden * 4), -1);
    Q3_HIP(hipMemsetAsync(w.h, 0, R * c.hidden * 4, s), -1);
    Q3_HIP(hipMalloc((void**)&w.ssq, R * (c.hidden / 16) * 4), -1);
    Q3_HIP(hipMalloc((void**)&w.xh, R * c.hidden * 2), -1);
    Q3_HIP(hipMemsetAsync(w.xh, 0, R * c.hidden * 2, s), -1);
    Q3_HIP(hipMalloc((void**)&w.qkv, R * qkv_ld * 4), -1);
    Q3_HIP(hipMalloc((void**)&w.attn, R * c.n_heads * c.head_dim * 2), -1);
    Q3_HIP(hipMemsetAsync(w.attn, 0, R * c.n_heads * c.head_dim * 2, s), -1);
    Q3_HIP(hipMalloc((void**)&w.act, R * ffn * 2), -1);
    Q3_HIP(hipMemsetAsync(w.act, 0, R * ffn * 2, s), -1);
    Q3_HIP(hipMalloc((void**)&w.hidden_f32, R * c.hidden * 4), -1);
    Q3_HIP(hipMalloc((void**)&w.hidden_f16, R * c.hidden * 2), -1);
    Q3_HIP(hipMemsetAsync(w.hidden_f16, 0, R * c.hidden * 2, s), -1);
    Q3_HIP(hipMalloc((void**)&w.logits, R * max_vocab * 4), -1);
    Q3_HIP(hipMalloc((void**)&w.map_slot, R * 4), -1);
    Q3_HIP(hipMalloc((void**)&w.map_pos, R * 4), -1);
    Q3_HIP(hipStreamSynchronize(s), -1);
    w.map_R16 = 0;
    return 0;
}
void work_free(Work& w) {
    void* ps[] = {w.rows_in, w.h, w.ssq, w.xh, w.qkv, w.attn, w.act, w.hidden_f32, w.hidden_f16, w.logits, w.map_slot, w.map_pos};
    for (void* p : ps)
        if (p) hipFree(p);
    w = Work();
}

int run_stack(hipStream_t s, const Model& m, const DevStack& st, Work& w, KVCache& kv, int R, const RowMap& rm,
              int attn_threads, int row0) {
    const ModelCfg& c = m.cfg;
    const int H = c.hidden, D = c.head_dim;
    const int qkv_ld = (c.n_heads + 2 * c.n_kv) * D;
    if (row0 % 16) {
        Q3_LOG("run_stack: row0=%d must be a multiple of 16 (fragment-ordered activations)", row0);
        return -1;
    }
    if (row0 + R > w.max_rows) {
        Q3_LOG("run_stack: %d rows > workspace %d", R, w.max_rows);
        return -1;
    }
    for (size_t li = 0; li < st.L.size(); li++) {
        const DevLayer& L = st.L[li];
        LinArgs a;
        a = LinArgs();
        a.wp = L.qkv.wp;
        a.N = L.qkv.N;
        a.K = H;
        a.M = row0 + R;
        a.m_begin = row0;
        a.nt = st.nt;
        a.x16 = w.xh;
        a.ssq = w.ssq;
        a.ssq_parts = H / 16;
        a.eps = c.eps;
        a.y = w.qkv;
        a.ldy = qkv_ld;
        if (!(li == 0 && rm.skip_qkv0) && launch_linear(s, a, PRO_NORM, EPI_STORE)) return -1;
        AttnArgs t;
        t.qkv = w.qkv;
        t.ld = qkv_ld;
        t.R = R;
        t.row0 = row0;
        t.q_norm = L.q_norm;
        t.k_norm = L.k_norm;
        t.eps = c.eps;
        t.rope_cos = m.rope_cos;
        t.rope_sin = m.rope_sin;
        t.slot = rm.slot;
        t.pos = rm.pos;
        t.slot_base = rm.slot_base;
        t.slot_stride = rm.slot_stride;
        t.pos_base = rm.pos_base;
        t.pos_stride = rm.pos_stride;
        t.kc = kv.k + li * kv.layer_stride();
        t.vc = kv.v + li * kv.layer_stride();
        t.n_ctx = kv.n_ctx;
        t.n_kv = c.n_kv;
        t.n_heads = c.n_heads;
        t.out = w.attn;
        t.scale = 1.0f / sqrtf((float)D);
        t.threads = attn_threads;
        if (rm.rows_total > R) {
            const int fit = 65536 / (rm.rows_total * c.n_kv);
            if (t.threads > fit) t.threads = fit / 64 * 64;
            if (t.threads < 256) t.threads = 256;
        }
        t.valid_mod = rm.valid_mod;
        t.valid_n = rm.valid_n;
        if (rm.same_slot_rows && R > 1) {
            if (launch_attn(s, t, ATTN_PREP)) return -1;
            if (rm.tiles && rm.n_tiles > 0) {
                t.tiles = rm.tiles;
                t.n_tiles = rm.n_tiles;
            } else if (!rm.slot && !rm.pos && rm.slot_stride == 0 && rm.pos_stride == 1 && rm.valid_mod == 0) {
                t.tiles = nullptr;
                t.n_tiles = (R + 15) / 16;
            }
            if (launch_attn(s, t, ATTN_ATTEND)) return -1;
        } else {
            if (launch_attn(s, t, ATTN_FUSED)) return -1;
        }
        a = LinArgs();
        a.wp = L.o.wp;
        a.N = H;
        a.K = L.o.K;
        a.M = row0 + R;
        a.m_begin = row0;
        a.nt = st.nt;
        a.x16 = w.attn;
        a.h_out = w.h;
        a.ssq_out = w.ssq;
        a.xh_out = w.xh;
        a.gamma = L.post_ln;
        if (launch_linear(s, a, PRO_F16, EPI_RESID)) return -1;
        a = LinArgs();
        a.wp = L.gu.wp;
        a.N = L.gu.N;
        a.K = H;
        a.M = row0 + R;
        a.m_begin = row0;
        a.nt = st.nt;
        a.x16 = w.xh;
        a.ssq = w.ssq;
        a.ssq_parts = H / 16;
        a.eps = c.eps;
        a.act = w.act;
        if (launch_linear(s, a, PRO_NORM, EPI_SWIGLU)) return -1;
        a = LinArgs();
        a.wp = L.down.wp;
        a.N = H;
        a.K = L.down.K;
        a.M = row0 + R;
        a.m_begin = row0;
        a.nt = st.nt;
        a.x16 = w.act;
        a.h_out = w.h;
        a.ssq_out = w.ssq;
        a.gamma = li + 1 < st.L.size() ? st.L[li + 1].in_ln : st.tail_gamma;
        a.xh_out = a.gamma ? w.xh : nullptr;
        if (launch_linear(s, a, PRO_F16, EPI_RESID)) return -1;
    }
    return 0;
}

void GraphExec::reset() {
    if (e) hipGraphExecDestroy(e);
    if (g) hipGraphDestroy(g);
    e = nullptr;
    g = nullptr;
}

int GraphExec::end_capture(hipStream_t s, int body_rc, const char* who) {
    const hipError_t er = hipStreamEndCapture(s, &g);
    if (body_rc || er != hipSuccess) {
        Q3_LOG("%s: graph capture failed", who);
        return -1;
    }
    Q3_HIP(hipGraphInstantiate(&e, g, nullptr, nullptr, 0), -1);
    return 0;
}

}
```

### qwen3_tts_axera_russian_amd/csrc/q3_sample.hip

```cpp
#include "q3_kdev.h"

namespace q3 {

__device__ __forceinline__ void block_argmax(float& v, int& idx, float* sv, int* si) {
    group_argmax_down<64>(v, idx);
    const int w = threadIdx.x >> 6, nw = blockDim.x >> 6;
    if ((threadIdx.x & 63) == 0) {
        sv[w] = v;
        si[w] = idx;
    }
    __syncthreads();
    v = sv[0];
    idx = si[0];
    for (int i = 1; i < nw; i++)
        if (sv[i] > v || (sv[i] == v && si[i] < idx)) {
            v = sv[i];
            idx = si[i];
        }
    __syncthreads();
}

__device__ __forceinline__ float uniform01(unsigned long long seed, unsigned row, unsigned frame, unsigned group) {
    unsigned long long z = seed + 0x9E3779B97F4A7C15ull * (1ull + row + ((unsigned long long)frame << 20) +
                                                            ((unsigned long long)group << 44));
    z = (z ^ (z >> 30)) * 0xBF58476D1CE4E5B9ull;
    z = (z ^ (z >> 27)) * 0x94D049BB133111EBull;
    z = z ^ (z >> 31);
    return (float)(z >> 40) * (1.0f / 16777216.0f);
}

__device__ __forceinline__ float nan_as_inf(float l) { return l != l ? INFINITY : l; }

constexpr int SAMPLE_SEL_CAP = 64;
constexpr int SAMPLE_SORT_CAP = 4096;
__host__ __device__ __forceinline__ int effective_top_k(int top_k, int n) { return (top_k <= 0 || top_k > n) ? n : top_k; }
__host__ __device__ __forceinline__ int sample_sort_len(int n) {
    int p = 64;
    while (p < n) p <<= 1;
    return p;
}
static size_t sample_lds_bytes(int n, int top_k, float temperature) {
    if (!(temperature > 1e-6f)) return 0;
    return effective_top_k(top_k, n) <= SAMPLE_SEL_CAP ? (size_t)n * 4 : (size_t)sample_sort_len(n) * 8;
}

__device__ int block_sample_topk(float* lg, int n, int top_k, float temperature, float top_p, float u, float* sv,
                                 int* si, float* selv, int* seli) {
    __shared__ int chosen;
    top_k = effective_top_k(top_k, n);
    const float inv_t = 1.0f / fmaxf(temperature, 1e-6f);
    if (top_k <= SAMPLE_SEL_CAP) {
        int found = 0;
        for (int k = 0; k < top_k; k++) {
            float best = -INFINITY;
            int bidx = 0x7fffffff;
            for (int v = threadIdx.x; v < n; v += blockDim.x) {
                const float l = lg[v];
                if (l > best) {
                    best = l;
                    bidx = v;
                }
            }
            block_argmax(best, bidx, sv, si);
            if (bidx >= n) break;
            if (threadIdx.x == 0) {
                selv[k] = best;
                seli[k] = bidx;
                lg[bidx] = -INFINITY;
            }
            found = k + 1;
            __syncthreads();
        }
        if (threadIdx.x == 0) {
            int pick = 0;
            if (found > 0 && !(selv[0] < INFINITY)) pick = seli[0];
            else if (found > 0) {
                const float top = selv[0];
                float sum = 0.f;
                for (int k = 0; k < found; k++) {
                    selv[k] = expf((selv[k] - top) * inv_t);
                    sum += selv[k];
                }
                int keep = found;
                if (top_p > 0.f && top_p < 1.f) {
                    float c = 0.f;
                    for (int k = 0; k < found; k++) {
                        c += selv[k] / sum;
                        if (c >= top_p) {
                            keep = k + 1;
                            break;
                        }
                    }
                    sum = 0.f;
                    for (int k = 0; k < keep; k++) sum += selv[k];
                }
                float c = 0.f;
                pick = seli[keep - 1];
                const float target = u * sum;
                for (int k = 0; k < keep; k++) {
                    c += selv[k];
                    if (target < c) {
                        pick = seli[k];
                        break;
                    }
                }
            }
            chosen = pick;
        }
        __syncthreads();
        return chosen;
    }
    const int n2 = sample_sort_len(n);
    int* li = (int*)(lg + n2);
    for (int v = threadIdx.x; v < n2; v += blockDim.x) {
        if (v >= n) lg[v] = -INFINITY;
        li[v] = v;
    }
    __syncthreads();
    for (int k2 = 2; k2 <= n2; k2 <<= 1)
        for (int j = k2 >> 1; j > 0; j >>= 1) {
            for (int i = threadIdx.x; i < n2; i += blockDim.x) {
                const int ixj = i ^ j;
                if (ixj > i) {
                    const float a0 = lg[i], a1 = lg[ixj];
                    const int i0 = li[i], i1 = li[ixj];
                    const bool before = a0 > a1 || (a0 == a1 && i0 < i1);
                    const bool desc = (i & k2) == 0;
                    if (desc ? !before : before) {
                        lg[i] = a1;
                        lg[ixj] = a0;
                        li[i] = i1;
                        li[ixj] = i0;
                    }
                }
            }
            __syncthreads();
        }
    if (threadIdx.x == 0) {
        int pick = li[0] < n ? li[0] : 0;
        const float top = lg[0];
        if (top < INFINITY && top > -INFINITY) {
            float sum = 0.f;
            int found = 0;
            for (int k = 0; k < top_k; k++) {
                if (!(lg[k] > -INFINITY)) break;
                lg[k] = expf((lg[k] - top) * inv_t);
                sum += lg[k];
                found = k + 1;
            }
            int keep = found;
            if (top_p > 0.f && top_p < 1.f) {
                float c = 0.f;
                for (int k = 0; k < found; k++) {
                    c += lg[k] / sum;
                    if (c >= top_p) {
                        keep = k + 1;
                        break;
                    }
                }
                sum = 0.f;
                for (int k = 0; k < keep; k++) sum += lg[k];
            }
            float c = 0.f;
            pick = li[keep - 1];
            const float target = u * sum;
            for (int k = 0; k < keep; k++) {
                c += lg[k];
                if (target < c) {
                    pick = li[k];
                    break;
                }
            }
        }
        chosen = pick;
    }
    __syncthreads();
    return chosen;
}

template <class T>
__device__ __forceinline__ T uniform_entry(const T* p, int r) {
    static_assert(sizeof(T) % 4 == 0, "the entry is read as words");
    constexpr int NW = (int)(sizeof(T) / 4);
    const __attribute__((address_space(4))) int* q = (const __attribute__((address_space(4))) int*)(p + r);
    int w[NW];
#pragma unroll
    for (int i = 0; i < NW; i++) w[i] = q[i];
    T e;
    __builtin_memcpy(&e, w, sizeof(e));
    return e;
}
__device__ __forceinline__ SlotParams uniform_slot(const SlotParams* p, int r) { return uniform_entry(p, r); }
__device__ __forceinline__ SlotRules uniform_rules(const SlotRules* p, int r) { return uniform_entry(p, r); }

template <bool SLOTS, bool RULES = false, bool SCORES = false>
__device__ __forceinline__ void talker_sample_row(const TalkerSampleArgs& a) {
    Q3_TL(42);
    __shared__ float sv[16];
    __shared__ int si[16];
    __shared__ float sc_wm[SCORES ? 16 : 1], sc_ws[SCORES ? 16 : 1];
    float sc_m = -INFINITY, sc_s = 0.f;
    __shared__ int win[32];
    __shared__ int nwin;
    const int r = a.row0 + blockIdx.x;
    const int RT = a.R_total > 0 ? a.R_total : a.R;
    const int np = uniform_load(a.n_past + r);
    const int nt = uniform_load(a.n_text + r);
    const bool was_done = uniform_load(a.done + r) != 0;
    float temperature = a.temperature, top_p = a.top_p;
    int top_k = a.top_k, max_frames = a.max_frames;
    int slot_flags = 0;
    if constexpr (SLOTS) {
        const SlotParams sp = uniform_slot(a.slots, r);
        temperature = sp.t_temp;
        top_p = sp.t_top_p;
        top_k = sp.t_top_k;
        max_frames = sp.max_frames;
        slot_flags = sp.flags;
        if (a.text_avail) {
            const int avail = uniform_load(a.text_avail + r);
            const int gen = np - sp.prompt;
            const bool held = (slot_flags & 3) == 3 && !was_done && gen >= 1 && gen >= avail && np < max_frames;
            if (threadIdx.x == 0) a.held[r] = held ? 1 : 0;
            if (held) return;
        }
    }
    float rep_penalty = a.rep_penalty;
    int rep_window = 30;
    double eos_boost = 15.0, eos_force = 2.0;
    bool add_boost = true, may_force = true, eos_early = false;
    const unsigned* seen_row = nullptr;
    if constexpr (RULES) {
        if (a.rules) {
            const SlotRules ru = uniform_rules(a.rules, r);
            rep_penalty = ru.rep_penalty;
            rep_window = ru.rep_window < 0 ? 0 : ru.rep_window > 30 ? 30 : ru.rep_window;
            eos_boost = (double)ru.eos_boost;
            eos_force = (double)ru.eos_force;
            add_boost = ru.eos_boost != 0.f;
            may_force = ru.eos_force != 0.f;
            eos_early = np < ru.min_past;
            if (rep_window == 0) seen_row = a.seen + (size_t)r * ((a.audio_vocab + 31) / 32);
        }
    }
    if (threadIdx.x == 0) nwin = np < rep_window ? np : rep_window;
    if (threadIdx.x < rep_window && threadIdx.x < np) {
        win[threadIdx.x] = a.past[r * 32 + ((np - 1 - threadIdx.x) & 31)];
    }
    __syncthreads();
    double progress = 0.0;
    float boost = 0.f;
    bool force_eos = false;
    if (nt > 0) {
        const double expected = (double)nt * 3.0;
        progress = (double)np / expected;
        if (progress > 0.8) {
            double b = (progress - 0.8) / 0.7;
            if (b > 1.0) b = 1.0;
            boost = (float)(b * eos_boost);
        }
        if (may_force && progress > eos_force) force_eos = true;
    }
    const bool eos_masked = a.ignore_eos || (SLOTS && (slot_flags & 2)) || (RULES && eos_early);
    float best = -INFINITY;
    int bidx = 0x7fffffff;
    const int nw_ = nwin;
    extern __shared__ float slg[];
    __shared__ float selv[64];
    __shared__ int seli[64];
    const bool stochastic = temperature > 1e-6f;
    for (int v = threadIdx.x; v < a.V; v += blockDim.x) {
        float l = nan_as_inf(a.logits[(size_t)r * a.V + v]);
        if constexpr (SCORES) {
            if ((v < a.audio_vocab || v == a.eos) && l > -INFINITY) {
                if (l > sc_m) {
                    sc_s = sc_s * expf(sc_m - l) + 1.f;
                    sc_m = l;
                } else {
                    sc_s += expf(l - sc_m);
                }
            }
        }
        if (v >= a.audio_vocab && v != a.eos) l = -1e10f;
        if (v == a.eos) {
            if (eos_masked) l = -1e10f;
            else if (nt > 0 && progress > 0.8 && add_boost) l += boost;
        }
        bool rep = false;
        for (int i = 0; i < nw_; i++) rep |= (win[i] == v);
        if constexpr (RULES)
            if (seen_row && v < a.audio_vocab) rep = (seen_row[v >> 5] >> (v & 31)) & 1u;
        if (rep) l = l > 0.f ? __fdiv_rn(l, rep_penalty) : l * rep_penalty;
        if (stochastic) slg[v] = l;
        if (l > best || (l == best && v < bidx)) {
            best = l;
            bidx = v;
        }
    }
    if constexpr (SCORES) {
        const float wm = wave_max(sc_m);
        const float ws = wave_sum(sc_m > -INFINITY ? sc_s * expf(sc_m - wm) : 0.f);
        if ((threadIdx.x & 63) == 0) {
            sc_wm[threadIdx.x >> 6] = wm;
            sc_ws[threadIdx.x >> 6] = ws;
        }
    }
    if (stochastic) {
        __syncthreads();
        float u;
        if constexpr (SLOTS) {
            const SlotParams sp = uniform_slot(a.slots, r);
            u = uniform01(sp.seed, sp.no_row ? 0u : (unsigned)r, (unsigned)a.n_frames[r], 0u);
        } else {
            u = uniform01(a.seed_ptr ? a.seed_ptr[r] : a.seed, (unsigned)r, (unsigned)a.n_frames[r], 0u);
        }
        bidx = block_sample_topk(slg, a.V, top_k, temperature, top_p, u, sv, si, selv, seli);
    } else {
        block_argmax(best, bidx, sv, si);
        if (bidx >= a.V) bidx = a.eos;
    }
    if (threadIdx.x == 0) {
        int code = bidx;
        if (force_eos && !eos_masked) code = a.eos;
        bool fin = was_done || code == a.eos || code >= a.audio_vocab || (max_frames > 0 && np >= max_frames);
        const int f = a.n_frames[r];
        if (!SLOTS || !fin || f <= a.frame_cap) a.n_frames[r] = f + 1;
        const bool keep = f < a.frame_cap;
        int* fc = a.codes + ((size_t)(keep ? f : 0) * RT + r) * 16;
        int used = code;
        if (a.forced && keep && !fin) {
            const int fz = a.forced[((size_t)f * RT + r) * 16];
            if (fz >= 0) used = fz;
        }
        if (fin || !keep) {
            a.done[r] = 1;
            if (keep) fc[0] = -1;
        } else {
            fc[0] = code;
            if constexpr (SCORES) {
                if (a.scores) {
                    const int nw = blockDim.x >> 6;
                    float m = sc_wm[0], sum = 0.f;
                    for (int i = 1; i < nw; i++) m = fmaxf(m, sc_wm[i]);
                    for (int i = 0; i < nw; i++) sum += sc_wm[i] > -INFINITY ? sc_ws[i] * expf(sc_wm[i] - m) : 0.f;
                    float zu = -INFINITY;
                    if (used >= 0 && used < a.V && (used < a.audio_vocab || used == a.eos))
                        zu = nan_as_inf(a.logits[(size_t)r * a.V + used]);
                    a.scores[((size_t)f * RT + r) * 16] = (m < INFINITY && m > -INFINITY) ? zu - m - logf(sum) : __builtin_nanf("");
                }
            }
            a.past[r * 32 + (np & 31)] = used;
            if constexpr (RULES)
                if (a.seen && used >= 0 && used < a.audio_vocab)
                    a.seen[(size_t)r * ((a.audio_vocab + 31) / 32) + (used >> 5)] |= 1u << (used & 31);
            a.n_past[r] = np + 1;
            a.pos[r] = a.pos0[r] + np;
        }
    }
}
__global__ void talker_sample_kernel(TalkerSampleArgs a) { talker_sample_row<false>(a); }
__global__ void talker_sample_kernel_slots(TalkerSampleArgs a) { talker_sample_row<true>(a); }
__global__ void talker_sample_kernel_rules(TalkerSampleArgs a) { talker_sample_row<true, true>(a); }
__global__ void talker_sample_kernel_scores(TalkerSampleArgs a) { talker_sample_row<false, false, true>(a); }
__global__ void talker_sample_kernel_slots_scores(TalkerSampleArgs a) { talker_sample_row<true, false, true>(a); }
__global__ void talker_sample_kernel_rules_scores(TalkerSampleArgs a) { talker_sample_row<true, true, true>(a); }

static size_t sample_lds_bytes_slots(int n) { return (size_t)sample_sort_len(n) * 8; }

static int sample_vocab_refused(const char* who, bool slots, int V, float temperature, int top_k) {
    if (slots && V > SAMPLE_SORT_CAP) {
        Q3_LOG("%s: a vocabulary of %d is beyond the per-slot sampler (sort cap %d)", who, V, SAMPLE_SORT_CAP);
        return -1;
    }
    if (temperature > 1e-6f && effective_top_k(top_k, V) > SAMPLE_SEL_CAP && V > SAMPLE_SORT_CAP) {
        Q3_LOG("%s: top_k=%d over a vocabulary of %d is beyond the device sampler (sort cap %d)", who, top_k, V, SAMPLE_SORT_CAP);
        return -1;
    }
    return 0;
}

int launch_talker_sample(hipStream_t s, const TalkerSampleArgs& a) {
    if (a.R <= 0) return 0;
    if ((a.text_avail && !a.held) || ((a.text_avail || a.held) && !a.slots)) {
        Q3_LOG("talker_sample: text_avail / held need each other and per-slot mode (text_avail %p, held %p, slots %p)",
               (const void*)a.text_avail, (const void*)a.held, (const void*)a.slots);
        return -1;
    }
    if ((a.rules || a.seen) && (!a.slots || (a.rules && !a.seen) || a.audio_vocab <= 0)) {
        Q3_LOG("talker_sample: rules need seen, and both per-slot mode (rules %p, seen %p, slots %p)", (const void*)a.rules,
               (const void*)a.seen, (const void*)a.slots);
        return -1;
    }
    if (sample_vocab_refused("talker_sample", a.slots != nullptr, a.V, a.temperature, a.top_k)) return -1;
    const size_t lds = a.slots ? sample_lds_bytes_slots(a.V) : sample_lds_bytes(a.V, a.top_k, a.temperature);
    TalkerSampleArgs a2 = a;
    a2.tl_node = tl_next_node();
    static void (*const kernels[2][3])(TalkerSampleArgs) = {
        {talker_sample_kernel, talker_sample_kernel_slots, talker_sample_kernel_rules},
        {talker_sample_kernel_scores, talker_sample_kernel_slots_scores, talker_sample_kernel_rules_scores}};
    hipLaunchKernelGGL(kernels[a.scores ? 1 : 0][(a.rules || a.seen) ? 2 : a.slots ? 1 : 0], dim3(a.R), dim3(256), lds, s, a2);
    Q3_HIP(hipGetLastError(), -1);
    return 0;
}

template <bool SLOTS, bool RULES = false, bool SCORES = false>
__device__ __forceinline__ void cp_argmax_row(const CpArgmaxArgs& a) {
    if constexpr (SLOTS)
        Q3_FETCH_ARGS("s"(a.logits), "s"(a.V), "s"(a.H), "s"(a.row0), "s"(a.R_total), "s"(a.R), "s"(a.group), "s"(a.codes), "s"(a.n_frames),
                      "s"(a.frame_cap), "s"(a.next_table), "s"(a.h_out), "s"(a.ssq_out), "s"(a.xh_out), "s"(a.gamma_next),
                      "s"(a.talker_emb), "s"(a.slots), "s"(a.forced), "s"(a.next_qkv), "s"(a.qkv_out), "s"(a.qkv_ld),
                      "s"(a.text_rows), "s"(a.text_avail), "s"(a.text_cap), "s"(a.held));
    else
        Q3_FETCH_ARGS("s"(a.logits), "s"(a.V), "s"(a.H), "s"(a.row0), "s"(a.R_total), "s"(a.R), "s"(a.group), "s"(a.codes), "s"(a.n_frames),
                      "s"(a.frame_cap), "s"(a.next_table), "s"(a.h_out), "s"(a.ssq_out), "s"(a.xh_out), "s"(a.gamma_next),
                      "s"(a.talker_emb), "s"(a.temperature), "s"(a.forced), "s"(a.next_qkv), "s"(a.qkv_out), "s"(a.qkv_ld));
    Q3_TL(43);
    __shared__ float sv[4];
    __shared__ int si[4];
    const int r = a.row0 + blockIdx.x, tid = threadIdx.x;
    const int RT = a.R_total > 0 ? a.R_total : a.R;
    float best = -INFINITY;
    int bidx = 0x7fffffff;
    const float4* lg = (const float4*)(a.logits + (size_t)r * a.V);
    const int n4 = a.V / 4;
    float4 l0 = make_float4(-INFINITY, -INFINITY, -INFINITY, -INFINITY), l1 = l0;
    if (tid < n4) l0 = lg[tid];
    if (tid + 256 < n4) l1 = lg[tid + 256];
    const int nf_r = uniform_load(a.n_frames + r);
    float temperature = a.temperature;
    int top_k = a.top_k;
    int text_avail = 0;
    int held = 0;
    if constexpr (SLOTS) {
        if (a.held) held = uniform_load(a.held + r);
        const SlotParams sp = uniform_slot(a.slots, r);
        temperature = sp.c_temp;
        top_k = sp.c_top_k;
        if (a.talker_emb && a.text_rows) text_avail = uniform_load(a.text_avail + r);
    }
    Q3_PH(0);
    {
        const float e[8] = {nan_as_inf(l0.x), nan_as_inf(l0.y), nan_as_inf(l0.z), nan_as_inf(l0.w),
                            nan_as_inf(l1.x), nan_as_inf(l1.y), nan_as_inf(l1.z), nan_as_inf(l1.w)};
#pragma unroll
        for (int j = 0; j < 8; j++) {
            const int idx = (j < 4 ? tid : tid + 256) * 4 + (j & 3);
            if (e[j] > best) {
                best = e[j];
                bidx = idx;
            }
        }
    }
    for (int v4 = tid + 512; v4 < n4; v4 += 256) {
        const float4 l = lg[v4];
        const float e[4] = {nan_as_inf(l.x), nan_as_inf(l.y), nan_as_inf(l.z), nan_as_inf(l.w)};
#pragma unroll
        for (int j = 0; j < 4; j++)
            if (e[j] > best) {
                best = e[j];
                bidx = v4 * 4 + j;
            }
    }
    group_argmax_down<64>(best, bidx);
    if ((tid & 63) == 0) {
        sv[tid >> 6] = best;
        si[tid >> 6] = bidx;
    }
    __syncthreads();
    Q3_PH(1);
    best = sv[0];
    bidx = si[0];
#pragma unroll
    for (int i = 1; i < 4; i++)
        if (sv[i] > best || (sv[i] == best && si[i] < bidx)) {
            best = sv[i];
            bidx = si[i];
        }
    const float sc_m = best;
    float sc_sum = 0.f;
    if constexpr (SCORES) {
        __shared__ float sc_ws[4];
        const float e[8] = {nan_as_inf(l0.x), nan_as_inf(l0.y), nan_as_inf(l0.z), nan_as_inf(l0.w),
                            nan_as_inf(l1.x), nan_as_inf(l1.y), nan_as_inf(l1.z), nan_as_inf(l1.w)};
        float s = 0.f;
#pragma unroll
        for (int j = 0; j < 8; j++) s += expf(e[j] - sc_m);
        for (int v4 = tid + 512; v4 < n4; v4 += 256) {
            const float4 l = lg[v4];
            s += expf(nan_as_inf(l.x) - sc_m);
            s += expf(nan_as_inf(l.y) - sc_m);
            s += expf(nan_as_inf(l.z) - sc_m);
            s += expf(nan_as_inf(l.w) - sc_m);
        }
        s = wave_sum(s);
        if ((tid & 63) == 0) sc_ws[tid >> 6] = s;
        __syncthreads();
        sc_sum = ((sc_ws[0] + sc_ws[1]) + sc_ws[2]) + sc_ws[3];
    }
    if (temperature > 1e-6f) {
        extern __shared__ float slg[];
        __shared__ float selv[64];
        __shared__ int seli[64];
        __shared__ float sv2[16];
        __shared__ int si2[16];
        __syncthreads();
        for (int v = tid; v < a.V; v += 256) slg[v] = nan_as_inf(a.logits[(size_t)r * a.V + v]);
        __syncthreads();
        float u;
        if constexpr (SLOTS) {
            const SlotParams sp = uniform_slot(a.slots, r);
            u = uniform01(sp.seed, sp.no_row ? 0u : (unsigned)r, (unsigned)nf_r, 1u + (unsigned)a.group);
        } else {
            u = uniform01(a.seed_ptr ? a.seed_ptr[r] : a.seed, (unsigned)r, (unsigned)nf_r, 1u + (unsigned)a.group);
        }
        float top_p = 0.f;
        if constexpr (RULES) top_p = uniform_rules(a.rules, r).cp_top_p;
        bidx = block_sample_topk(slg, a.V, top_k, temperature, top_p, u, sv2, si2, selv, seli);
    }
    if (bidx < 0 || bidx >= a.V) bidx = 0;
    int f = nf_r - 1;
    if (f < 0) f = 0;
    const bool keep = f < a.frame_cap;
    if (!keep) f = a.frame_cap - 1;
    int* fc = a.codes + ((size_t)f * RT + r) * 16;
    if (SLOTS && held) {
        bidx = fc[1 + a.group];
        if (bidx < 0 || bidx >= a.V) bidx = 0;
    } else if (tid == 0 && keep) fc[1 + a.group] = bidx;
    const int* fz = (a.forced && keep) ? a.forced + ((size_t)f * RT + r) * 16 : nullptr;
    if (fz && fz[1 + a.group] >= 0) bidx = fz[1 + a.group];
    if constexpr (SCORES) {
        if (a.scores && tid == 0 && keep && !(SLOTS && held)) {
            const float zu = bidx >= 0 && bidx < a.V ? nan_as_inf(a.logits[(size_t)r * a.V + bidx]) : -INFINITY;
            a.scores[((size_t)f * RT + r) * 16 + 1 + a.group] =
                (sc_m < INFINITY && sc_m > -INFINITY) ? zu - sc_m - logf(sc_sum) : __builtin_nanf("");
        }
    }
    Q3_PH(2);
    if (a.talker_emb) {
        const float* last = a.pad_embed;
        if constexpr (SLOTS)
            if (nf_r >= 1 && nf_r - 1 < text_avail) last = a.text_rows + ((size_t)r * a.text_cap + (nf_r - 1)) * a.H;
        feedback_row(fc, r, a.talker_emb, a.talker_vocab, a.cp_tables, a.V, a.n_groups, last,
                     a.h_out, a.ssq_out, a.H, a.group, bidx, fz, a.xh_out, a.gamma_next);
    } else if (a.next_table) {
        const bool ok = bidx < a.V;
        const int t = ok ? bidx : 0;
        const float4 zero = make_float4(0.f, 0.f, 0.f, 0.f);
        const float* erow = a.next_table + (size_t)t * a.H;
        const int ne4 = a.H / 4;
        if (a.next_qkv) {
            constexpr int QV = 4;
            const int nq4 = a.qkv_ld / 4;
            const float4* tq = (const float4*)(a.next_qkv + (size_t)t * a.qkv_ld);
            float4* dq = (float4*)(a.qkv_out + (size_t)r * a.qkv_ld);
            float4 ev = *(const float4*)(erow + (tid < ne4 ? tid : 0) * 4);
            float4 qv[QV];
#pragma unroll
            for (int j = 0; j < QV; j++) {
                const int i = tid + 256 * j;
                qv[j] = tq[i < nq4 ? i : 0];
            }
            if (!ok) {
                ev = zero;
#pragma unroll
                for (int j = 0; j < QV; j++) qv[j] = zero;
            }
            if (tid < ne4) store_row_ssq(a.h_out, a.ssq_out, r, a.H, tid, ev, a.xh_out, a.gamma_next);
#pragma unroll
            for (int j = 0; j < QV; j++) {
                const int i = tid + 256 * j;
                if (i < nq4) dq[i] = qv[j];
            }
            for (int k4 = tid + 256; k4 < ne4; k4 += 256) {
                float4 v = *(const float4*)(erow + k4 * 4);
                if (!ok) v = zero;
                store_row_ssq(a.h_out, a.ssq_out, r, a.H, k4, v, a.xh_out, a.gamma_next);
            }
            for (int i = tid + 256 * QV; i < nq4; i += 256) {
                float4 v = tq[i];
                if (!ok) v = zero;
                dq[i] = v;
            }
        } else {
            for (int k4 = tid; k4 < ne4; k4 += 256) {
                float4 v = *(const float4*)(erow + k4 * 4);
                if (!ok) v = zero;
                store_row_ssq(a.h_out, a.ssq_out, r, a.H, k4, v, a.xh_out, a.gamma_next);
            }
        }
    }
}
__global__ void __launch_bounds__(256) cp_argmax_kernel(CpArgmaxArgs a) { cp_argmax_row<false>(a); }
__global__ void __launch_bounds__(256) cp_argmax_kernel_slots(CpArgmaxArgs a) { cp_argmax_row<true>(a); }
__global__ void __launch_bounds__(256) cp_argmax_kernel_rules(CpArgmaxArgs a) { cp_argmax_row<true, true>(a); }
__global__ void __launch_bounds__(256) cp_argmax_kernel_scores(CpArgmaxArgs a) { cp_argmax_row<false, false, true>(a); }
__global__ void __launch_bounds__(256) cp_argmax_kernel_slots_scores(CpArgmaxArgs a) { cp_argmax_row<true, false, true>(a); }
__global__ void __launch_bounds__(256) cp_argmax_kernel_rules_scores(CpArgmaxArgs a) { cp_argmax_row<true, true, true>(a); }

int launch_cp_argmax(hipStream_t s, const CpArgmaxArgs& a) {
    if (a.R <= 0) return 0;
    if (a.V % 4) {
        Q3_LOG("cp_argmax: a vocabulary of %d is not a multiple of 4", a.V);
        return -1;
    }
    if (((a.text_rows || a.text_avail || a.held) && !a.slots) || (a.text_rows && (!a.text_avail || a.text_cap <= 0))) {
        Q3_LOG("cp_argmax: text_rows / text_avail / held need per-slot mode, text_rows needs text_avail and text_cap > 0 "
               "(text_rows %p, text_avail %p, text_cap %d, held %p, slots %p)", (const void*)a.text_rows,
               (const void*)a.text_avail, a.text_cap, (const void*)a.held, (const void*)a.slots);
        return -1;
    }
    if (a.rules && !a.slots) {
        Q3_LOG("cp_argmax: rules need per-slot mode (rules %p, slots %p)", (const void*)a.rules, (const void*)a.slots);
        return -1;
    }
    if (sample_vocab_refused("cp_argmax", a.slots != nullptr, a.V, a.temperature, a.top_k)) return -1;
    const size_t lds = a.slots ? sample_lds_bytes_slots(a.V) : sample_lds_bytes(a.V, a.top_k, a.temperature);
    CpArgmaxArgs a2 = a;
    a2.tl_node = tl_next_node();
    static void (*const kernels[2][3])(CpArgmaxArgs) = {
        {cp_argmax_kernel, cp_argmax_kernel_slots, cp_argmax_kernel_rules},
        {cp_argmax_kernel_scores, cp_argmax_kernel_slots_scores, cp_argmax_kernel_rules_scores}};
    hipLaunchKernelGGL(kernels[a.scores ? 1 : 0][a.rules ? 2 : a.slots ? 1 : 0], dim3(a.R), dim3(256), lds, s, a2);
    Q3_HIP(hipGetLastError(), -1);
    return 0;
}

}
```

### qwen3_tts_axera_russian_amd/csrc/q3_test_api.hip

```cpp
#include "q3_enc.h"
#include "q3_model.h"
#include "q3_spk.h"
#include "q3_voc_ops.h"
#include "q3_xlane.h"
#include <chrono>
#include <cstring>
#include <vector>

using namespace q3;

namespace q3 {
template <int OP, int WIDTH>
__global__ void __launch_bounds__(256) xlane_case_kernel(const float* __restrict__ in, int n, float* __restrict__ out_new,
                                                         float* __restrict__ out_shfl) {
    const int i = blockIdx.x * blockDim.x + threadIdx.x;
    const float v = in[i];
    if (OP == 0) {
        out_new[i] = group_sum_down<WIDTH, WIDTH / 2, XlDpp>(v);
        out_shfl[i] = group_sum_down<WIDTH, WIDTH / 2, XlShfl>(v);
    } else if (OP == 1) {
        out_new[i] = group_max_down<WIDTH, WIDTH / 2, XlDpp>(v);
        out_shfl[i] = group_max_down<WIDTH, WIDTH / 2, XlShfl>(v);
    } else {
        float va = v, vb = v;
// ... 1448 lines not shown
    if (rc) return -1;
    Q3_HIP(hipDeviceSynchronize(), -1);
    if (!o.down()) return -1;
    memcpy(out, o.h.data(), o.words * 4);
    return o.tail() ? -3 : 0;
}
extern "C" int q3t_spk_rowmean_case(const float* x, int C, const int* n_f, int B, float* out) { return spk_reduce_case(0, nullptr, x, C, n_f, B, out); }
extern "C" int q3t_spk_rowstat_case(const float* x, int C, const int* n_f, int B, float* stat) { return spk_reduce_case(1, nullptr, x, C, n_f, B, stat); }
extern "C" int q3t_spk_attnpool_case(const float* z, const float* x, int C, const int* n_f, int B, float* pooled) {
    return spk_reduce_case(2, z, x, C, n_f, B, pooled);
}

extern "C" int q3t_spk_matvec_case(const float* w, const float* bias, const float* in, int I, int O, int act, int B, float* out) {
    if (!w || !in || !out || I < 1 || O < 1 || O > 4 * 65535 || B < 1 || B > 65535 || act < 0 || act > 2 || (long long)I * O > OP_MAX_WORDS ||
        (long long)B * std::max(I, O) > OP_MAX_WORDS)
        return -2;
    DBuf dw, db, di;
    OpOut o;
    if (!dw.up(w, (size_t)I * O * 4) || !di.up(in, (size_t)B * I * 4) || !o.init((size_t)B * O)) return -1;
    if (bias && !db.up(bias, (size_t)O * 4)) return -1;
    Q3_HIP(hipDeviceSynchronize(), -1);
    if (spk_launch_matvec(nullptr, (const float*)dw.p, bias ? (const float*)db.p : nullptr, (const float*)di.p, o.p(), I, O, act, B)) return -1;
    Q3_HIP(hipDeviceSynchronize(), -1);
    if (!o.down()) return -1;
    memcpy(out, o.h.data(), o.words * 4);
    return o.tail() ? -3 : 0;
}

extern "C" int q3t_spk_se_apply_case(const float* h, const float* gate, const float* res, int C, int L, int Cy2, int c02, int B, float* y1,
                                     float* y2) {
    if (!h || !gate || !res || !y1 || !y2 || B < 1 || B > 65535 || C < 1 || C > 65535 || L < 1 || L > (1 << 20) || c02 < 0 || c02 + C > Cy2)
        return -2;
    const int ld = (int)spk_pitch(L);
    if ((long long)B * Cy2 * ld > OP_MAX_WORDS) return -2;
    const size_t n = (size_t)B * C * ld;
    DBuf dh, dg, dr;
    OpOut o1, o2;
    if (!dh.up(h, n * 4) || !dg.up(gate, (size_t)B * C * 4) || !dr.up(res, n * 4) || !o1.init(n) || !o2.init((size_t)B * Cy2 * ld)) return -1;
    Q3_HIP(hipDeviceSynchronize(), -1);
    if (spk_launch_se_apply(nullptr, (const float*)dh.p, (const float*)dg.p, (const float*)dr.p, o1.p(), o2.p(), Cy2, c02, C, ld, B)) return -1;
    Q3_HIP(hipDeviceSynchronize(), -1);
    if (!o1.down() || !o2.down()) return -1;
    memcpy(y1, o1.h.data(), n * 4);
    return (o1.tail() + o2.slice(y2, B, Cy2, c02, C, ld)) ? -3 : 0;
}

extern "C" int q3t_spk_att_act_case(const float* x, const float* bias, int C, int L, int B, float* y) {
    if (!x || !bias || !y || B < 1 || B > 65535 || C < 1 || C > 65535 || L < 1 || L > (1 << 20)) return -2;
    const int ld = (int)spk_pitch(L);
    if ((long long)B * C * ld > OP_MAX_WORDS) return -2;
    const size_t n = (size_t)B * C * ld;
    DBuf dx, db;
    OpOut o;
    if (!dx.up(x, n * 4) || !db.up(bias, (size_t)B * C * 4) || !o.init(n)) return -1;
    Q3_HIP(hipDeviceSynchronize(), -1);
    if (spk_launch_att_act(nullptr, (const float*)dx.p, (const float*)db.p, o.p(), C, ld, B)) return -1;
    Q3_HIP(hipDeviceSynchronize(), -1);
    if (!o.down()) return -1;
    memcpy(y, o.h.data(), n * 4);
    return o.tail() ? -3 : 0;
}

extern "C" int q3t_enc_unfold_case(const float* x, int B, int Cin, const int* lens, int k, int s, int replicate, int elu, float* y) {
    if (!x || !y || Cin < 1 || s < 1 || k < s || k > 64 || (long long)Cin * k > 65535 || (replicate & ~1) || (elu & ~1)) return -2;
    const int L = op_longest(lens, B, 1);
    if (L < 0) return -2;
    const int Lout = (L + s - 1) / s, ldx = (int)enc_pitch(L), ldy = (int)enc_pitch(Lout);
    const size_t rows = (size_t)B * Cin * k;
    if ((long long)rows * ldy > OP_MAX_WORDS || (long long)B * Cin * ldx > OP_MAX_WORDS) return -2;
    const std::vector<float> hx = op_padded(x, (size_t)B * Cin, L, ldx);
    DBuf dx, dn;
    OpOut o;
    if (!dx.up(hx.data(), hx.size() * 4) || !dn.up(lens, (size_t)B * 4) || !o.init(rows * ldy)) return -1;
    Q3_HIP(hipDeviceSynchronize(), -1);
    if (enc_launch_unfold(nullptr, (const float*)dx.p, ldx, Cin, (const int*)dn.p, o.p(), Lout, k, s, replicate, elu, B)) return -1;
    Q3_HIP(hipDeviceSynchronize(), -1);
    if (!o.down()) return -1;
    int outside = o.tail();
    for (size_t r = 0; r < rows; r++) {
        memcpy(y + r * Lout, o.h.data() + r * ldy, (size_t)Lout * 4);
        for (int l = Lout; l < ldy; l++) outside += o.h[r * ldy + l] != OP_GUARD;
    }
    return outside ? -3 : 0;
}

extern "C" int q3t_enc_stream_unfold_case(const float* x, int B, int Cin, int skip, int n_in, int n_out, int k, int s, int replicate, int elu,
                                          int finish, float* hist, int max_streams, const int* streams, const int* before, float* y) {
    if (!x || !y || !hist || !streams || !before || B < 1 || B > 65535 || Cin < 1 || Cin > 65535 || s < 1 || k < s || k - 1 > 32 || skip < 0 ||
        n_in < 0 || n_out < 0 || (n_in == 0 && n_out == 0) || max_streams < B || (replicate & ~1) || (elu & ~1) || (finish & ~1))
        return -2;
    if ((long long)skip + n_in > (1 << 20) || (long long)max_streams * Cin * (k - 1) > OP_MAX_WORDS) return -2;
    std::vector<char> seen((size_t)max_streams, 0);
    for (int b = 0; b < B; b++) {
        if (streams[b] < 0 || streams[b] >= max_streams || seen[(size_t)streams[b]]++ || before[b] < 0 || before[b] > 0x7fffffff - n_in) return -2;
        const long long after = (long long)before[b] + n_in;
        if ((finish ? (after + s - 1) / s : after / s) - before[b] / s != n_out) return -2;
    }
    const int cols = skip + n_in, ldx = (int)enc_pitch(cols), ldy = (int)enc_pitch(n_out), H = k - 1;
    const size_t rows = (size_t)B * Cin * k, sf = (size_t)Cin * H, nh = (size_t)max_streams * sf;
    if ((long long)rows * ldy > OP_MAX_WORDS || (long long)B * Cin * ldx > OP_MAX_WORDS) return -2;
    const std::vector<float> hx = op_padded(x, (size_t)B * Cin, cols, ldx);
    OpOut o, oh;
    DBuf dx, ds, db;
    if (!dx.up(hx.data(), hx.size() * 4) || !ds.up(streams, (size_t)B * 4) || !db.up(before, (size_t)B * 4) || !o.init(rows * ldy)) return -1;
    oh.words = nh;
    oh.h.assign(nh + 32, OP_GUARD);
    for (int b = 0; b < B; b++) memcpy(oh.h.data() + (size_t)streams[b] * sf, hist + (size_t)streams[b] * sf, sf * 4);
    if (!oh.d.up(oh.h.data(), oh.h.size() * 4)) return -1;
    Q3_HIP(hipDeviceSynchronize(), -1);
    if (enc_stream_launch_unfold(nullptr, (const float*)dx.p, ldx, skip, Cin, n_in, o.p(), n_out, k, s, replicate, elu, finish, oh.p(),
                                 (long long)sf, (const int*)ds.p, (const int*)db.p, B))
        return -1;
    Q3_HIP(hipDeviceSynchronize(), -1);
    if (!o.down() || !oh.down()) return -1;
    int outside = o.tail() + oh.tail();
    for (size_t r = 0; r < rows; r++) {
        memcpy(y + r * n_out, o.h.data() + r * ldy, (size_t)n_out * 4);
        for (int l = n_out; l < ldy; l++) outside += o.h[r * ldy + l] != OP_GUARD;
    }
    for (int st = 0; st < max_streams; st++) {
        if (seen[(size_t)st]) memcpy(hist + (size_t)st * sf, oh.h.data() + (size_t)st * sf, sf * 4);
        else
            for (size_t i = 0; i < sf; i++) outside += oh.h[(size_t)st * sf + i] != OP_GUARD;
    }
    return outside ? -3 : 0;
}

extern "C" int q3t_enc_stream_emit_case(const float* y, int B, int C, int skip, int n, const int* off, int rows, float* out) {
    if (!y || !off || !out || B < 1 || B > 65535 || C < 1 || skip < 0 || n < 1 || n > 65535 || rows < 1 || (long long)rows * C > OP_MAX_WORDS ||
        (long long)B * C * enc_pitch((long)skip + n) > OP_MAX_WORDS)
        return -2;
    std::vector<char> owned((size_t)rows, 0);
    for (int b = 0; b < B; b++) {
        if (off[b] < 0 || (long long)off[b] + n > rows) return -2;
        for (int j = 0; j < n; j++)
            if (owned[(size_t)off[b] + j]++) return -2;
    }
    const int cols = skip + n, ld = (int)enc_pitch(cols);
    const std::vector<float> hy = op_padded(y, (size_t)B * C, cols, ld);
    DBuf dy, dn;
    OpOut o;
    if (!dy.up(hy.data(), hy.size() * 4) || !dn.up(off, (size_t)B * 4) || !o.init((size_t)rows * C)) return -1;
    Q3_HIP(hipDeviceSynchronize(), -1);
    if (enc_stream_launch_emit(nullptr, (const float*)dy.p, C, ld, skip, n, (const int*)dn.p, o.p(), B)) return -1;
    Q3_HIP(hipDeviceSynchronize(), -1);
    if (!o.down()) return -1;
    memcpy(out, o.h.data(), o.words * 4);
    int outside = o.tail();
    for (int r = 0; r < rows; r++)
        if (!owned[(size_t)r])
            for (int c = 0; c < C; c++) outside += o.h[(size_t)r * C + c] != OP_GUARD;
    return outside ? -3 : 0;
}
```

### qwen3_tts_axera_russian_amd/hiplib.py

```python
from __future__ import annotations

import ctypes
import os

from . import LIB_PATH, TEST_LIB_PATH

_lib = None
_test_lib = None

c_void_p, c_int, c_float, c_char_p = ctypes.c_void_p, ctypes.c_int, ctypes.c_float, ctypes.c_char_p
f32p = ctypes.POINTER(ctypes.c_float)
i32p = ctypes.POINTER(ctypes.c_int32)
i64p = ctypes.POINTER(ctypes.c_int64)
u16p = ctypes.POINTER(ctypes.c_uint16)
i16p = ctypes.POINTER(ctypes.c_int16)


class SlotParamsC(ctypes.Structure):
    _fields_ = [("max_frames", ctypes.c_int32), ("temperature", ctypes.c_float), ("top_k", ctypes.c_int32),
                ("top_p", ctypes.c_float), ("cp_temperature", ctypes.c_float), ("cp_top_k", ctypes.c_int32),
                ("seed", ctypes.c_uint64), ("utt", ctypes.c_int32), ("reserved", ctypes.c_int32)]


class KernelSlotParamsC(ctypes.Structure):
# ... 136 lines not shown
    _sig(lib, "voc_incr_last_split_launches", c_int, [c_void_p])
    _sig(lib, "voc_incr_last_redone", c_int, [c_void_p])
    _sig(lib, "voc_incr_snapshots", c_int, [c_void_p, c_int])
    _sig(lib, "voc_incr_save", c_int, [c_void_p, c_int, c_int])
    _sig(lib, "voc_incr_restore", c_int, [c_void_p, c_int, i32p, i32p])
    _sig(lib, "voc_incr_snapshot_frames", ctypes.c_int64, [c_void_p, c_int])
    _sig(lib, "voc_incr_last_restore_ms", c_float, [c_void_p])
    _sig(lib, "enc_load", c_void_p, [c_char_p, c_int, c_int])
    _sig(lib, "enc_free", None, [c_void_p])
    _sig(lib, "enc_num_quantizers", c_int, [c_void_p])
    _sig(lib, "enc_sample_rate", c_int, [c_void_p])
    _sig(lib, "enc_samples_per_frame", c_int, [c_void_p])
    _sig(lib, "enc_frames", c_int, [c_void_p, c_int])
    _sig(lib, "enc_encode", c_int, [c_void_p, f32p, i32p, c_int, i64p_, c_int, i32p])
    _sig(lib, "enc_last_ms", c_float, [c_void_p])
    _sig(lib, "enc_pcm_frames", c_int, [c_void_p, c_int, c_int])
    _sig(lib, "enc_encode_pcm", c_int, [c_void_p, c_void_p, c_int, c_int, c_int, i32p, c_int, i64p_, c_int, i32p])
    _sig(lib, "enc_debug_pcm", c_int, [c_void_p, c_void_p, c_int, c_int, c_int, i32p, c_int, f32p, i32p, i32p])
    _sig(lib, "enc_debug_shape", c_int, [c_void_p, i32p, c_int, c_int, i32p, i32p])
    _sig(lib, "enc_debug_run", c_int, [c_void_p, f32p, i32p, c_int, c_int, f32p, i32p, i32p])
    _sig(lib, "enc_resample_pcm", c_int, [c_void_p, c_void_p, c_int, c_int, c_int, i32p, c_int, f32p, c_int, i32p])
    _sig(lib, "spk_load", c_void_p, [c_char_p, c_int, c_int])
    _sig(lib, "spk_free", None, [c_void_p])
    _sig(lib, "spk_dim", c_int, [c_void_p])
    _sig(lib, "spk_sample_rate", c_int, [c_void_p])
    _sig(lib, "spk_min_samples", c_int, [c_void_p])
    _sig(lib, "spk_frames", c_int, [c_void_p, c_int])
    _sig(lib, "spk_embed", c_int, [c_void_p, f32p, i32p, c_int, f32p])
    _sig(lib, "spk_last_ms", c_float, [c_void_p])
    _sig(lib, "spk_last_launches", c_int, [c_void_p])
    _sig(lib, "enc_stream_create", c_void_p, [c_void_p, c_int, c_int])
    _sig(lib, "enc_stream_free", None, [c_void_p])
    _sig(lib, "enc_stream_reset", c_int, [c_void_p, c_int])
    _sig(lib, "enc_stream_push_max_frames", c_int, [c_void_p, c_int, i32p, i32p, i32p])
    _sig(lib, "enc_stream_push", c_int, [c_void_p, c_int, i32p, f32p, i32p, i32p, i64p_, ctypes.c_int64, i64p_])
    _sig(lib, "enc_stream_last_ms", c_float, [c_void_p])
    _sig(lib, "enc_stream_last_launches", c_int, [c_void_p])
    _sig(lib, "enc_stream_state_bytes", ctypes.c_int64, [c_void_p])
    _sig(lib, "enc_stream_device_bytes", ctypes.c_int64, [c_void_p])
    _sig(lib, "enc_stream_pcm_samples", ctypes.c_int64, [c_void_p, c_int, ctypes.c_int64, c_int])
    _sig(lib, "enc_stream_pcm_max_frames_in", c_int, [c_void_p, c_int])
    _sig(lib, "enc_stream_push_pcm_max_frames", c_int, [c_void_p, c_int, i32p, c_int, c_int, c_int, i32p, i32p])
    _sig(lib, "enc_stream_push_pcm", c_int, [c_void_p, c_int, i32p, c_void_p, c_int, c_int, c_int, i32p, i32p, i64p_, ctypes.c_int64,
                                             i64p_])
    _sig(lib, "enc_stream_pcm_device_bytes", ctypes.c_int64, [c_void_p])
    _sig(lib, "enc_stream_debug_push_pcm", c_int, [c_void_p, c_int, i32p, c_void_p, c_int, c_int, c_int, i32p, i32p, i64p_,
                                                   ctypes.c_int64, i64p_, f32p, i64p_])
    _sig(lib, "tfe_load", c_void_p, [c_char_p, c_char_p, c_int])
    _sig(lib, "tfe_free", None, [c_void_p])
    _sig(lib, "tfe_hidden_size", c_int, [c_void_p])
    _sig(lib, "tfe_text_vocab", c_int, [c_void_p])
    _sig(lib, "tfe_embed_text", c_int, [c_void_p, i32p, c_int, f32p])
    _sig(lib, "tfe_build_prefix", c_int, [c_void_p, i32p, c_int, i32p, f32p])
    _sig(lib, "tfe_tts_pad_embed", c_int, [c_void_p, f32p])
    _sig(lib, "tfe_build_prefix_stream", c_int, [c_void_p, ctypes.c_int32, i32p, f32p])
    _sig(lib, "tfe_tts_eos_embed", c_int, [c_void_p, f32p])
    _sig(lib, "tfe_build_prefix_spk", c_int, [c_void_p, i32p, c_int, i32p, f32p, f32p])
    _sig(lib, "tfe_build_prefix_stream_spk", c_int, [c_void_p, ctypes.c_int32, i32p, f32p, f32p])
    _sig(lib, "tfe_debug_stages", c_int, [c_void_p, i32p, c_int, u16p, f32p, u16p, f32p, i32p])
    _sig(lib, "q3_device_count", c_int, [])
    _sig(lib, "q3_device_compute_units", c_int, [])
    _sig(lib, "q3_set_device", c_int, [c_int])
    if path is None:
        _lib = lib
    return lib


def load_test():
    global _test_lib
    if _test_lib is not None:
        return _test_lib
    load()
    if not os.path.exists(TEST_LIB_PATH):
        raise RuntimeError(f"{TEST_LIB_PATH} not found: build it with `python -m qwen3_tts_axera_russian_amd.build`")
    lib = ctypes.CDLL(TEST_LIB_PATH)
    _sig(lib, "q3t_set_linear_tuning", c_int, [c_int, c_int, c_int])
    _sig(lib, "q3t_linear", c_int, [c_int, c_int, c_int, u16p, c_int, c_int, c_int, u16p, f32p, f32p, c_float,
                                    f32p, f32p, u16p, c_int])
    _sig(lib, "q3t_linear_case", c_int, [c_int, c_int, c_int, c_int, u16p, c_int, c_int, c_int, c_int, c_float, c_int,
                                         u16p, f32p, f32p, f32p, f32p, f32p, u16p, f32p, f32p, f32p, u16p, u16p])
    _sig(lib, "q3t_reset_linear_knobs", c_int, [])
    _sig(lib, "q3t_last_linear_variant", c_char_p, [])
    _sig(lib, "q3t_talker_sample", c_int, [f32p, c_int, i32p, c_int, c_int, c_int])
    u64, u64p = ctypes.c_uint64, ctypes.POINTER(ctypes.c_uint64)
    _sig(lib, "q3t_talker_sample_case", c_int, [f32p, c_int, c_int, c_int, c_int, i32p, i32p, i32p, i32p, i32p, i32p, i32p,
                                                i32p, c_int, i32p, c_int, c_int, c_int, c_int, c_float, c_float, c_int,
                                                c_float, u64, u64p, c_void_p])
    _sig(lib, "q3t_cp_sample_case", c_int, [f32p, c_int, c_int, c_int, c_int, c_int, i32p, i32p, c_int, i32p, c_float, c_int,
                                            u64, u64p, c_void_p, c_int, c_int, f32p, f32p, c_int, f32p, f32p, c_int, f32p,
                                            c_int, f32p, f32p, f32p, ctypes.POINTER(ctypes.c_uint16), f32p])
    talker_case = [f32p, c_int, c_int, c_int, c_int, i32p, i32p, i32p, i32p, i32p, i32p, i32p, i32p, c_int, i32p, c_int, c_int,
                   c_int, c_int, c_float, c_float, c_int, c_float, u64, u64p, c_void_p]
    cp_case = [f32p, c_int, c_int, c_int, c_int, c_int, i32p, i32p, c_int, i32p, c_float, c_int, u64, u64p, c_void_p, c_int,
               c_int, f32p, f32p, c_int, f32p, f32p, c_int, f32p, c_int, f32p, f32p, f32p, u16p, f32p]
    _sig(lib, "q3t_talker_sample_text_case", c_int, talker_case + [i32p, i32p])
    _sig(lib, "q3t_cp_sample_text_case", c_int, cp_case + [f32p, i32p, c_int, i32p])
    u32p = ctypes.POINTER(ctypes.c_uint32)
    _sig(lib, "q3t_talker_sample_rules_case", c_int, talker_case + [i32p, i32p, c_void_p, u32p])
    _sig(lib, "q3t_cp_sample_rules_case", c_int, cp_case + [f32p, i32p, c_int, i32p, c_void_p])
    _sig(lib, "q3t_talker_score_case", c_int, talker_case + [i32p, i32p, c_void_p, u32p, f32p])
    _sig(lib, "q3t_cp_score_case", c_int, cp_case + [f32p, i32p, c_int, i32p, c_void_p, f32p])
    _sig(lib, "q3t_prompt_rows_seen_case", c_int, [i32p, c_int, i32p, i32p, f32p, c_int, f32p, c_int, c_int, c_int, f32p, c_int,
                                                   c_int, c_int, c_int, c_int, f32p, f32p, f32p, u16p, c_int, u32p, c_int])
    _sig(lib, "q3t_final_norm_case", c_int, [f32p, f32p, c_int, c_int, c_int, f32p, c_float, c_int, c_int, i32p, c_int, c_int,
                                             c_int, c_int, c_int, f32p, f32p, u16p, f32p, f32p, u16p])
    _sig(lib, "q3t_gather_embed_case", c_int, [f32p, c_int, c_int, i32p, c_int, i32p, c_int, c_int, i32p, c_int, c_int, c_int,
                                               f32p, f32p, f32p, u16p])
    _sig(lib, "q3t_feedback_case", c_int, [i32p, c_int, f32p, c_int, f32p, c_int, c_int, f32p, c_int, f32p, f32p, f32p, u16p])
    _sig(lib, "q3t_prompt_rows_case", c_int, [i32p, c_int, i32p, i32p, f32p, c_int, f32p, c_int, c_int, c_int, f32p, c_int,
                                              c_int, c_int, c_int, c_int, f32p, f32p, f32p, u16p, c_int])
    _sig(lib, "q3t_prefix_move_case", c_int, [u16p, u16p, c_int, c_int, c_int, c_int, u16p, c_int, c_int, f32p, f32p, f32p,
                                              c_int, c_int, c_int, i32p])
    _sig(lib, "q3t_attn", c_int, [c_int, c_int, c_int, f32p, f32p, f32p, c_float, f32p, f32p, c_int, i32p, i32p, c_int,
                                  c_int, c_int, c_int, u16p, u16p, c_int, c_int, i32p, c_int, c_int, c_int, c_int, u16p])
    _sig(lib, "q3t_voc_attn", c_int, [c_int, f32p, f32p, c_int, c_int, c_int, c_int, c_int, c_float])
    _sig(lib, "q3t_xlane_case", c_int, [c_int, c_int, c_int, f32p, f32p, f32p])
    _sig(lib, "q3t_set_linear_split_rows", c_int, [c_int])
    _sig(lib, "q3t_set_linear_narrow8", c_int, [c_int])
    _sig(lib, "q3t_set_linear_wide_tiles", c_int, [c_int])
    _sig(lib, "q3t_set_attn_short", c_int, [c_int])
    _sig(lib, "q3t_set_gemm_min_rows", c_int, [c_int])
    _sig(lib, "q3t_set_gemm_glds", c_int, [c_int])
    _sig(lib, "q3t_inspect_weights", c_int, [ctypes.c_char_p, ctypes.c_char_p, ctypes.c_char_p, c_int])
    _sig(lib, "q3t_bench_linear", c_float, [c_int, c_int, c_int, c_int, c_int, c_int, c_int, c_int])
    _sig(lib, "q3t_bench_chain", c_float, [c_int, c_int, c_int, c_int, c_int, c_int])
    _sig(lib, "q3t_cp_model_load", c_void_p, [c_char_p])
    _sig(lib, "q3t_cp_model_free", None, [c_void_p])
    _sig(lib, "q3t_cp_qkv_ld", c_int, [c_void_p])
    _sig(lib, "q3t_cp_qkv_serves", c_int, [c_void_p, c_int])
    _sig(lib, "q3t_cp_qkv_tab", c_int, [c_void_p, c_int, i32p, c_int, f32p])
    _sig(lib, "q3t_cp_qkv_live", c_int, [c_void_p, c_int, i32p, c_int, c_int, f32p])
    _sig(lib, "q3t_enc_stream_embeddings", c_int, [c_void_p, c_int, i32p, f32p, i32p, i32p, i64p, ctypes.c_int64, i64p, f32p, i32p])
    i64s = ctypes.POINTER(ctypes.c_longlong)
    _sig(lib, "q3t_enc_stream_plan", c_int, [i32p, i32p, c_int, ctypes.c_longlong, ctypes.c_longlong, c_int, i64s, i64s, i64s])
    _sig(lib, "q3t_enc_rvq_tile", c_int, [c_int])
    _sig(lib, "q3t_enc_rvq_case", c_int, [f32p, c_int, c_int, c_int, c_int, c_int, c_int, c_int, f32p, i64p])
    _sig(lib, "q3t_enc_conv_in_case", c_int, [f32p, c_int, c_int, f32p, f32p, c_int, c_int, f32p, c_int, i32p, f32p])
    u8p = ctypes.POINTER(ctypes.c_uint8)
    _sig(lib, "q3t_dequant_case", c_int, [c_int, u8p, ctypes.c_longlong, c_int, c_int, c_int, c_int, u16p, f32p, i32p])
    _sig(lib, "q3t_spk_mel", c_int, [c_void_p, f32p, i32p, c_int, f32p, i32p, i32p])
    _sig(lib, "q3t_spk_stage", c_int, [c_void_p, f32p, i32p, c_int, c_int, f32p, i32p, i32p])
    _sig(lib, "q3t_spk_unfold_case", c_int, [f32p, c_int, c_int, f32p, c_int, c_int, i32p, c_int, c_int, c_int, c_int, f32p])
    _sig(lib, "q3t_spk_place_case", c_int, [f32p, c_int, c_int, c_int, c_int, c_int, c_int, c_int, c_int, f32p])
    _sig(lib, "q3t_spk_rowmean_case", c_int, [f32p, c_int, i32p, c_int, f32p])
    _sig(lib, "q3t_spk_rowstat_case", c_int, [f32p, c_int, i32p, c_int, f32p])
    _sig(lib, "q3t_spk_attnpool_case", c_int, [f32p, f32p, c_int, i32p, c_int, f32p])
    _sig(lib, "q3t_spk_matvec_case", c_int, [f32p, f32p, f32p, c_int, c_int, c_int, c_int, f32p])
    _sig(lib, "q3t_spk_se_apply_case", c_int, [f32p, f32p, f32p, c_int, c_int, c_int, c_int, c_int, f32p, f32p])
    _sig(lib, "q3t_spk_att_act_case", c_int, [f32p, f32p, c_int, c_int, c_int, f32p])
    _sig(lib, "q3t_enc_unfold_case", c_int, [f32p, c_int, c_int, i32p, c_int, c_int, c_int, c_int, f32p])
    _sig(lib, "q3t_enc_stream_unfold_case", c_int, [f32p, c_int, c_int, c_int, c_int, c_int, c_int, c_int, c_int, c_int, c_int, f32p, c_int,
                                                    i32p, i32p, f32p])
    _sig(lib, "q3t_enc_stream_emit_case", c_int, [f32p, c_int, c_int, c_int, c_int, i32p, c_int, f32p])
    _test_lib = lib
    return lib


def fptr(a):
    return a.ctypes.data_as(f32p)


def iptr(a):
    return a.ctypes.data_as(i32p)
```

Measured before the change: 10590 codec_frames/s.

## Fuse code-predictor argmax pick and embedding gather into short attention kernel

Adds a templated attention body with a pick variant that reads the previous group's logits, does the argmax decision, gathers the precomputed QKV row and embedding for the chosen code, and writes the next hidden row. This folds the separate cp_argmax and the following attention into one kernel per code-predictor group and skips the pos-1 gather_embed when it is already done. It also appears to fold the talker sample and embedding gather together, and it uses explicit FMA and contract-off pragmas to keep the arithmetic bit-exact across both paths. The cost is extra registers and logits loads in the attention kernel, plus a more complex set of conditions that must hold for the fused path to be taken.

```diff
diff --git a/qwen3_tts_axera_russian_amd/csrc/q3_attn.hip b/qwen3_tts_axera_russian_amd/csrc/q3_attn.hip
--- a/qwen3_tts_axera_russian_amd/csrc/q3_attn.hip
+++ b/qwen3_tts_axera_russian_amd/csrc/q3_attn.hip
@@ -1,4 +1,5 @@
 #include "q3_kdev.h"
+#include "q3_pick.h"
 
 namespace q3 {
 
@@ -204,25 +205,15 @@
 constexpr int ATTN_SHORT_MAX_T = 15;
 static int g_attn_short = 1;
 int set_attn_short(int on) { g_attn_short = on; return 0; }
-__global__ void __launch_bounds__(256)
-    attn_short_kernel(float* __restrict__ p_qkv, int p_ld, int p_row0, int p_n_heads, int p_n_kv,
-                      const float* __restrict__ p_q_norm, const float* __restrict__ p_k_norm,
-                      const float* __restrict__ p_rope_cos, const float* __restrict__ p_rope_sin, int p_pos_base,
-                      int p_slot_base, AttnArgs a) {
+int attn_short_enabled() { return g_attn_short; }
+template <bool PICK>
+__device__ __forceinline__ void attn_short_body(AttnArgs& a, const CpPickArgs& p) {
     constexpr int D = 128, NE = ATTN_SHORT_MAX_T + 1;
-    a.qkv = p_qkv;
-    a.ld = p_ld;
-    a.row0 = p_row0;
-    a.n_heads = p_n_heads;
-    a.n_kv = p_n_kv;
-    a.q_norm = p_q_norm;
-    a.k_norm = p_k_norm;
-    a.rope_cos = p_rope_cos;
-    a.rope_sin = p_rope_sin;
-    a.pos_base = p_pos_base;
-    a.slot_base = p_slot_base;
     Q3_FETCH_ARGS("s"(a.eps), "s"(a.slot), "s"(a.slot_stride), "s"(a.kc), "s"(a.vc), "s"(a.n_ctx), "s"(a.out), "s"(a.scale));
-    Q3_TL(33);
+    if constexpr (PICK)
+        Q3_FETCH_ARGS("s"(p.H), "s"(p.R_total), "s"(p.group), "s"(p.codes), "s"(p.frame_cap), "s"(p.forced), "s"(p.table),
+                      "s"(p.qkv_rows), "s"(p.h_out), "s"(p.ssq_out), "s"(p.xh_out), "s"(p.gamma_next));
+    Q3_TL(PICK ? 34 : 33);
     const int r = a.row0 + blockIdx.x, g = blockIdx.y;
     const int tid = threadIdx.x, lane = tid & 63, w = tid >> 6;
     const int slot = a.slot ? uniform_load(a.slot + r) : a.slot_base + r * a.slot_stride;
@@ -231,17 +222,31 @@
     __shared__ float knew[D];
     __shared__ __attribute__((aligned(16))) half_t vs[NE][D];
     __shared__ __attribute__((aligned(16))) float sc[2][NE];
-    float* row = a.qkv + (size_t)r * a.ld;
+    float* row = PICK ? nullptr : a.qkv + (size_t)r * a.ld;
     const size_t cbase = ((size_t)slot * a.n_kv + g) * (size_t)a.n_ctx * D;
     const int l16 = tid & 15, grp = tid >> 4;
     const int hh = tid >> 7, d = tid & 127;
+    __shared__ float pick_sv[PICK ? 4 : 1];
+    __shared__ int pick_si[PICK ? 4 : 1];
+    const float4* lg = nullptr;
+    int n4 = 0, nf_r = 0;
+    float4 l0 = make_float4(-INFINITY, -INFINITY, -INFINITY, -INFINITY), l1 = l0;
+    if constexpr (PICK) {
+        lg = (const float4*)(p.logits + (size_t)r * p.V);
+        n4 = p.V / 4;
+        if (tid < n4) l0 = lg[tid];
+        if (tid + 256 < n4) l1 = lg[tid + 256];
+        nf_r = uniform_load(p.n_frames + r);
+    }
     float x0 = 0.f, x1 = 0.f, gm0 = 1.f, gm1 = 1.f, cs = 1.f, sn = 0.f;
     {
-        const float* src = w < 2 ? row + (size_t)(2 * g + w) * D
-                         : w == 2 ? row + (size_t)(a.n_heads + g) * D
-                                  : row + (size_t)(a.n_heads + a.n_kv + g) * D;
-        x0 = src[lane];
-        x1 = src[lane + 64];
+        if constexpr (!PICK) {
+            const float* src = w < 2 ? row + (size_t)(2 * g + w) * D
+                             : w == 2 ? row + (size_t)(a.n_heads + g) * D
+                                      : row + (size_t)(a.n_heads + a.n_kv + g) * D;
+            x0 = src[lane];
+            x1 = src[lane + 64];
+        }
         if (w < 3) {
             const float* gam = w < 2 ? a.q_norm : a.k_norm;
             gm0 = gam[lane];
@@ -255,15 +260,41 @@
         kpre = *(const h8*)(a.kc + cbase + (size_t)grp * D + l16 * 8);
         vpre = *(const h8*)(a.vc + cbase + (size_t)grp * D + l16 * 8);
     }
+    float4 ev = make_float4(0.f, 0.f, 0.f, 0.f);
+    const float* erow = nullptr;
+    if constexpr (PICK) {
+        __builtin_amdgcn_sched_barrier(0);
+        const int RT = p.R_total > 0 ? p.R_total : a.R;
+        const CpDecision dec = cp_decide(l0, l1, lg, n4, p.V, nf_r, p.frame_cap, RT, r, p.group, p.codes, p.forced, 0,
+                                         tid == 0 && g == 0, pick_sv, pick_si, [](float, int&) {});
+        const bool ok = dec.id < p.V;
+        const int t = ok ? dec.id : 0;
+        const float* trow = p.qkv_rows + (size_t)t * a.ld;
+        const float* src = w < 2 ? trow + (size_t)(2 * g + w) * D
+                         : w == 2 ? trow + (size_t)(a.n_heads + g) * D
+                                  : trow + (size_t)(a.n_heads + a.n_kv + g) * D;
+        x0 = src[lane];
+        x1 = src[lane + 64];
+        if (!ok) x0 = x1 = 0.f;
+        if (g == 0) {
+            erow = p.table + (size_t)t * p.H;
+            ev = *(const float4*)(erow + (tid < p.H / 4 ? tid : 0) * 4);
+            if (!ok) {
+                ev = make_float4(0.f, 0.f, 0.f, 0.f);
+                erow = nullptr;
+            }
+        }
+    }
     __builtin_amdgcn_sched_barrier(0);
     Q3_PH(0);
     if (w < 3) {
-        float ss = wave_sum(x0 * x0 + x1 * x1);
-        const float iv = 1.0f / sqrtf(ss / (float)D + a.eps);
+#pragma clang fp contract(off)
+        float ss = wave_sum((x0 * x0) + (x1 * x1));
+        const float iv = 1.0f / sqrtf(__builtin_fmaf(ss, 1.0f / (float)D, a.eps));
         x0 = (x0 * iv) * gm0;
         x1 = (x1 * iv) * gm1;
-        const float y0 = x0 * cs - x1 * sn;
-        const float y1 = x1 * cs + x0 * sn;
+        const float y0 = __builtin_fmaf(x0, cs, -(x1 * sn));
+        const float y1 = (x1 * cs) + (x0 * sn);
         x0 = y0;
         x1 = y1;
     }
@@ -287,12 +318,13 @@
     __syncthreads();
     Q3_PH(1);
     if (grp <= T) {
+#pragma clang fp contract(off)
         float d0 = 0.f, d1 = 0.f;
 #pragma unroll
         for (int j = 0; j < 8; j++) {
             const float kf = grp < T ? (float)kpre[j] : knew[l16 * 8 + j];
-            d0 += (qs[0][l16 * 8 + j] * a.scale) * kf;
-            d1 += (qs[1][l16 * 8 + j] * a.scale) * kf;
+            d0 = __builtin_fmaf(qs[0][l16 * 8 + j] * a.scale, kf, d0);
+            d1 = __builtin_fmaf(qs[1][l16 * 8 + j] * a.scale, kf, d1);
         }
         group_sum_down2<16>(d0, d1);
         if (l16 == 0) {
@@ -315,15 +347,64 @@
 #pragma unroll
     for (int e = 0; e < NE; e++) m = fmaxf(m, e <= T ? sv[e] : -INFINITY);
     float L = 0.f, o = 0.f;
-#pragma unroll
-    for (int e = 0; e < NE; e++) {
-        const float p = e <= T ? __expf(sv[e] - m) : 0.f;
-        const float vf = e <= T ? (float)vs[e][d] : 0.f;
-        L += p;
-        o += p * vf;
+    {
+#pragma clang fp contract(off)
+#pragma unroll
+        for (int e = 0; e < NE; e++) {
+            const float p = e <= T ? __expf(sv[e] - m) : 0.f;
+            const float vf = e <= T ? (float)vs[e][d] : 0.f;
+            L = L + p;
+            o = o + (p * vf);
+        }
     }
     Q3_PH(3);
     a.out[frag_idx(r, (2 * g + hh) * D + d, a.n_heads * D)] = sat_half(o / L);
+    if constexpr (PICK) {
+        if (g == 0) {
+            const int ne4 = p.H / 4;
+            if (tid < ne4) store_row_ssq(p.h_out, p.ssq_out, r, p.H, tid, ev, p.xh_out, p.gamma_next);
+            for (int k4 = tid + 256; k4 < ne4; k4 += 256) {
+                const float4 v = erow ? *(const float4*)(erow + k4 * 4) : make_float4(0.f, 0.f, 0.f, 0.f);
+                store_row_ssq(p.h_out, p.ssq_out, r, p.H, k4, v, p.xh_out, p.gamma_next);
+            }
+        }
+    }
+}
+__global__ void __launch_bounds__(256)
+    attn_short_kernel(float* __restrict__ p_qkv, int p_ld, int p_row0, int p_n_heads, int p_n_kv,
+                      const float* __restrict__ p_q_norm, const float* __restrict__ p_k_norm,
+                      const float* __restrict__ p_rope_cos, const float* __restrict__ p_rope_sin, int p_pos_base,
+                      int p_slot_base, AttnArgs a) {
+    a.qkv = p_qkv;
+    a.ld = p_ld;
+    a.row0 = p_row0;
+    a.n_heads = p_n_heads;
+    a.n_kv = p_n_kv;
+    a.q_norm = p_q_norm;
+    a.k_norm = p_k_norm;
+    a.rope_cos = p_rope_cos;
+    a.rope_sin = p_rope_sin;
+    a.pos_base = p_pos_base;
+    a.slot_base = p_slot_base;
+    attn_short_body<false>(a, CpPickArgs());
+}
+__global__ void __launch_bounds__(256)
+    attn_short_kernel_pick(const float* __restrict__ p_logits, int p_V, int p_row0, const int* __restrict__ p_n_frames,
+                           const float* __restrict__ p_q_norm, const float* __restrict__ p_k_norm,
+                           const float* __restrict__ p_rope_cos, const float* __restrict__ p_rope_sin, int p_pos_base,
+                           int p_slot_base, int p_n_kv, AttnArgs a, CpPickArgs p) {
+    p.logits = p_logits;
+    p.V = p_V;
+    a.row0 = p_row0;
+    p.n_frames = p_n_frames;
+    a.q_norm = p_q_norm;
+    a.k_norm = p_k_norm;
+    a.rope_cos = p_rope_cos;
+    a.rope_sin = p_rope_sin;
+    a.pos_base = p_pos_base;
+    a.slot_base = p_slot_base;
+    a.n_kv = p_n_kv;
+    attn_short_body<true>(a, p);
 }
 
 __global__ void __launch_bounds__(256) attn_tile_mfma_kernel(AttnArgs a) {
@@ -560,4 +641,24 @@
     return 0;
 }
 
-}
+int launch_cp_pick_attn(hipStream_t s, const AttnArgs& a, const CpPickArgs& p) {
+    if (a.R <= 0) return 0;
+    const bool shape = a.n_heads == 2 * a.n_kv && a.ld == (a.n_heads + 2 * a.n_kv) * 128;
+    const bool shrt = g_attn_short && !a.pos && a.pos_stride == 0 && a.pos_base >= 1 && a.pos_base <= ATTN_SHORT_MAX_T &&
+                      a.pos_base < a.n_ctx && a.valid_mod == 0;
+    const bool pick = p.logits && p.V > 0 && p.V % 4 == 0 && p.H > 0 && p.H % 16 == 0 && p.group >= 0 && p.group < 15 && p.codes &&
+                      p.n_frames && p.table && p.qkv_rows && p.h_out && p.ssq_out && (p.xh_out != nullptr) == (p.gamma_next != nullptr);
+    if (!shape || !shrt || !pick) {
+        Q3_LOG("cp_pick_attn: not a pass this launch serves (heads %d/%d, ld %d, position %d, short kernel %d, V %d, H %d, group %d)",
+               a.n_heads, a.n_kv, a.ld, a.pos_base, g_attn_short, p.V, p.H, p.group);
+        return -1;
+    }
+    AttnArgs a3 = a;
+    a3.tl_node = tl_next_node();
+    hipLaunchKernelGGL(attn_short_kernel_pick, dim3(a.R, a.n_kv), dim3(256), 0, s, p.logits, p.V, a3.row0, p.n_frames, a3.q_norm,
+                       a3.k_norm, a3.rope_cos, a3.rope_sin, a3.pos_base, a3.slot_base, a3.n_kv, a3, p);
+    Q3_HIP(hipGetLastError(), -1);
+    return 0;
+}
+
+}
diff --git a/qwen3_tts_axera_russian_amd/csrc/q3_cp.h b/qwen3_tts_axera_russian_amd/csrc/q3_cp.h
--- a/qwen3_tts_axera_russian_amd/csrc/q3_cp.h
+++ b/qwen3_tts_axera_russian_amd/csrc/q3_cp.h
@@ -24,7 +24,10 @@
     const SlotParams* slots = nullptr;
     const SlotRules* rules = nullptr;
     float* scores = nullptr;
+    bool pick = false;
+    bool pos1_gathered = false;
 };
+bool cp_frame_picks(const Model& m, int R, const CpFrameIO& io);
 
 int cp_seed_row0(const Work& w, int R, int row0 = 0, int R_total = 0);
 int cp_frame(hipStream_t s, const Model& m, Work& w, KVCache& kv, int R, const CpFrameIO& io, int row0 = 0,
diff --git a/qwen3_tts_axera_russian_amd/csrc/q3_cp_api.hip b/qwen3_tts_axera_russian_amd/csrc/q3_cp_api.hip
--- a/qwen3_tts_axera_russian_amd/csrc/q3_cp_api.hip
+++ b/qwen3_tts_axera_russian_amd/csrc/q3_cp_api.hip
@@ -15,6 +15,11 @@
     const int B16 = (R_total + 15) / 16 * 16;
     const bool two = two_row_enabled() && 2 * B16 <= w.max_rows;
     return two ? B16 : 0;
+}
+
+bool cp_frame_picks(const Model& m, int R, const CpFrameIO& io) {
+    return io.pick && !io.slots && !io.rules && !io.scores && !io.held && !io.text_rows && !(io.temperature > 1e-6f) &&
+           m.cp_qkv_serves(R) && attn_short_enabled();
 }
 
 int cp_frame(hipStream_t s, const Model& m, Work& w, KVCache& kv, int R, const CpFrameIO& io, int row0, int R_total) {
@@ -34,7 +39,8 @@
         r0.pos_stride = 0;
         r0.same_slot_rows = true;
         if (run_stack(s, m, m.cp, w, kv, R, r0, 256, seed0 + row0)) return -1;
-        if (launch_gather_embed(s, m.talker_emb, c.talker_vocab, H, io.codes, 0, io.n_frames, io.frame_cap, 0, w.h, w.ssq, R,
+        if (!io.pos1_gathered &&
+            launch_gather_embed(s, m.talker_emb, c.talker_vocab, H, io.codes, 0, io.n_frames, io.frame_cap, 0, w.h, w.ssq, R,
                                 row0, R_total, io.forced, w.xh, m.cp.L[0].in_ln))
             return -1;
         RowMap r1 = rm;
@@ -54,7 +60,8 @@
             Q3_HIP(hipStreamSynchronize(s), -1);
             w.map_R16 = R16;
         }
-        if (launch_gather_embed(s, m.talker_emb, c.talker_vocab, H, io.codes, 0, io.n_frames, io.frame_cap, 0, w.h, w.ssq, R,
+        if (!io.pos1_gathered &&
+            launch_gather_embed(s, m.talker_emb, c.talker_vocab, H, io.codes, 0, io.n_frames, io.frame_cap, 0, w.h, w.ssq, R,
                                 row0, R_total, io.forced, w.xh, m.cp.L[0].in_ln))
             return -1;
         RowMap r2;
@@ -65,6 +72,10 @@
         r2.valid_n = R;
         if (run_stack(s, m, m.cp, w, kv, R16 + R, r2, 256, 0)) return -1;
     } else {
+        if (io.pos1_gathered) {
+            Q3_LOG("cp_frame: position 1's rows cannot be stored before position 0 has run in them");
+            return -1;
+        }
         rm.pos_base = 0;
         if (run_stack(s, m, m.cp, w, kv, R, rm, 256, row0)) return -1;
         if (launch_gather_embed(s, m.talker_emb, c.talker_vocab, H, io.codes, 0, io.n_frames, io.frame_cap, 0, w.h, w.ssq, R,
@@ -74,11 +85,32 @@
         if (run_stack(s, m, m.cp, w, kv, R, rm, 256, row0)) return -1;
     }
     const bool qkv_tab = m.cp_qkv_serves(R);
+    const bool pick = cp_frame_picks(m, R, io);
     for (int g = 0; g < G; g++) {
         if (g > 0) {
             rm.pos_base = g + 1;
             rm.skip_qkv0 = qkv_tab;
+            CpPickArgs pk;
+            if (pick) {
+                pk.logits = w.logits;
+                pk.V = c.cp_vocab;
+                pk.H = H;
+                pk.R_total = R_total;
+                pk.group = g - 1;
+                pk.codes = io.codes;
+                pk.n_frames = io.n_frames;
+                pk.frame_cap = io.frame_cap;
+                pk.forced = io.forced;
+                pk.table = m.cp_emb[g - 1];
+                pk.qkv_rows = m.cp_qkv_rows(g - 1);
+                pk.h_out = w.h;
+                pk.ssq_out = w.ssq;
+                pk.xh_out = w.xh;
+                pk.gamma_next = m.cp.L[0].in_ln;
+                rm.pick = &pk;
+            }
             if (run_stack(s, m, m.cp, w, kv, R, rm, 256, row0)) return -1;
+            rm.pick = nullptr;
         }
         LinArgs a;
         a.wp = m.cp_head[g].wp;
@@ -94,6 +126,7 @@
         a.y = w.logits;
         a.ldy = c.cp_vocab;
         if (launch_linear(s, a, PRO_NORM, EPI_STORE)) return -1;
+        if (pick && g + 1 < G) continue;
         CpArgmaxArgs x;
         x.logits = w.logits;
         x.V = c.cp_vocab;
@@ -161,6 +194,7 @@
     GraphExec graph;
     int graph_rows = 0;
     int step_next_pos = 0;
+    bool pick = true;
 };
 
 }
@@ -181,6 +215,7 @@
     h->m = m;
     h->s = s;
     h->max_batch = max_batch;
+    h->pick = !(getenv("Q3_CP_PICK") && atoi(getenv("Q3_CP_PICK")) == 0);
     const ModelCfg& c = m->cfg;
     bool ok = kv_alloc(h->kv, c.cp_layers, max_batch, c.n_kv, c.cp_groups + 1, h->s) == 0;
     ok = ok && work_alloc(h->w, c, 2 * ((max_batch + 15) / 16 * 16), c.cp_ffn, c.cp_vocab, h->s) == 0;
@@ -239,6 +274,7 @@
     io.temperature = temperature;
     io.top_k = top_k;
     io.seed = seed;
+    io.pick = h->pick;
     auto body = [&]() -> int {
         if (launch_ssq_rows(h->s, h->w.rows_in, h->w.h, h->w.ssq, R, H, h->w.xh, m.cp.L[0].in_ln,
                             cp_seed_row0(h->w, R)))
diff --git a/qwen3_tts_axera_russian_amd/csrc/q3_engine.hip b/qwen3_tts_axera_russian_amd/csrc/q3_engine.hip
--- a/qwen3_tts_axera_russian_amd/csrc/q3_engine.hip
+++ b/qwen3_tts_axera_russian_amd/csrc/q3_engine.hip
@@ -19,6 +19,8 @@
 struct FrameState {
     int B = 0, ignore_eos = 0, cap_frames = 0, chains = 0;
     int text_cap = 0;
+    int cp_pick = 0;
+    int fold_gather = 0;
     Sampling smp;
     unsigned long long seed = 0;
     const int* forced = nullptr;
@@ -30,12 +32,12 @@
     unsigned* seen = nullptr;
     float* scores = nullptr;
     auto key() const {
-        return std::tie(B, ignore_eos, cap_frames, chains, text_cap, smp.t_temp, smp.t_top_p, smp.c_temp, smp.t_top_k, smp.c_top_k,
+        return std::tie(B, ignore_eos, cap_frames, chains, text_cap, cp_pick, fold_gather, smp.t_temp, smp.t_top_p, smp.c_temp, smp.t_top_k, smp.c_top_k,
                         seed, forced, slots, text_rows, text_avail, held, rules, seen, scores);
     }
     bool operator==(const FrameState& o) const { return key() == o.key(); }
 };
-static_assert(sizeof(FrameState) == 10 * 4 + 8 + 8 * sizeof(void*), "FrameState: a new field belongs in key() too");
+static_assert(sizeof(FrameState) == 12 * 4 + 8 + 8 * sizeof(void*), "FrameState: a new field belongs in key() too");
 
 struct TextRows {
     DeviceAllocs mem;
@@ -95,6 +97,7 @@
     Sampling smp;
     unsigned long long seed = 0;
     int n_chains = 1;
+    bool cp_pick = true;
     bool use_prio = false;
     int prio_hi = 0;
     hipStream_t cs[8] = {nullptr};
@@ -151,6 +154,8 @@
             }
         }
         if (scores) f.scores = scores->d;
+        f.cp_pick = cp_pick ? 1 : 0;
+        f.fold_gather = cp_pick && !slot_mode && !scores && !(smp.c_temp > 1e-6f) && cp_seed_row0(wc, B, 0, B) > 0 ? 1 : 0;
         return f;
     }
 };
@@ -233,6 +238,15 @@
     sa.rules = f.rules;
     sa.seen = f.seen;
     sa.scores = f.scores;
+    if (f.fold_gather) {
+        sa.emb_table = m.talker_emb;
+        sa.emb_V = m.cfg.talker_vocab;
+        sa.emb_H = m.cfg.hidden;
+        sa.emb_h = e->wc.h;
+        sa.emb_ssq = e->wc.ssq;
+        sa.emb_xh = e->wc.xh;
+        sa.emb_gamma = m.cp.L[0].in_ln;
+    }
     if (launch_talker_sample(st, sa)) return -1;
     CpFrameIO io;
     io.codes = e->d_codes;
@@ -255,6 +269,8 @@
     io.slots = f.slots;
     io.rules = f.rules;
     io.scores = f.scores;
+    io.pick = f.cp_pick != 0;
+    io.pos1_gathered = f.fold_gather != 0;
     if (cp_frame(st, m, e->wc, e->kv_c, R, io, row0, f.B)) return -1;
     RowMap rm;
     rm.slot_base = 0;
@@ -379,6 +395,7 @@
     const ModelCfg& c = m->cfg;
     e->prefill_rows = max_batch > 2048 ? max_batch : 2048;
     bool ok = hipEventCreate(&e->ev0) == hipSuccess && hipEventCreate(&e->ev1) == hipSuccess;
+    e->cp_pick = !(getenv("Q3_CP_PICK") && atoi(getenv("Q3_CP_PICK")) == 0);
     if (const char* nc = getenv("Q3_CHAINS")) e->n_chains = atoi(nc) < 1 ? 1 : atoi(nc) > 8 ? 8 : atoi(nc);
     else e->n_chains = 1;
     ok = ok && ensure_chains(e, e->n_chains) == 0;
diff --git a/qwen3_tts_axera_russian_amd/csrc/q3_kernels.h b/qwen3_tts_axera_russian_amd/csrc/q3_kernels.h
--- a/qwen3_tts_axera_russian_amd/csrc/q3_kernels.h
+++ b/qwen3_tts_axera_russian_amd/csrc/q3_kernels.h
@@ -150,6 +150,12 @@
     const SlotRules* rules = nullptr;
     unsigned* seen = nullptr;
     float* scores = nullptr;
+    const float* emb_table = nullptr;
+    int emb_V = 0, emb_H = 0;
+    float* emb_h = nullptr;
+    float* emb_ssq = nullptr;
+    half_t* emb_xh = nullptr;
+    const float* emb_gamma = nullptr;
 };
 int launch_talker_sample(hipStream_t s, const TalkerSampleArgs& a);
 
@@ -189,6 +195,23 @@
 };
 int launch_cp_argmax(hipStream_t s, const CpArgmaxArgs& a);
 
+struct CpPickArgs {
+    const float* logits = nullptr;
+    int V = 0, H = 0, R_total = 0;
+    int group = 0;
+    int* codes = nullptr;
+    const int* n_frames = nullptr;
+    int frame_cap = 0;
+    const int* forced = nullptr;
+    const float* table = nullptr;
+    const float* qkv_rows = nullptr;
+    float* h_out = nullptr;
+    float* ssq_out = nullptr;
+    half_t* xh_out = nullptr;
+    const float* gamma_next = nullptr;
+};
+int launch_cp_pick_attn(hipStream_t s, const AttnArgs& a, const CpPickArgs& p);
+
 int launch_feedback(hipStream_t s, const int* codes16, int R, const float* talker_emb, int talker_vocab,
                     const float* const* cp_tables, int cp_vocab, int n_groups, const float* pad_embed,
                     float* h_out, float* ssq_out, int H, half_t* xh_out = nullptr, const float* gamma = nullptr);
@@ -220,6 +243,8 @@
 int set_linear_narrow8(int on);
 int set_linear_wide_tiles(int on);
 int set_attn_short(int on);
+int attn_short_enabled();
+int set_sample_bitmap(int on);
 int set_gemm_min_rows(int n);
 int set_gemm_glds(int on);
 int reset_linear_knobs();
diff --git a/qwen3_tts_axera_russian_amd/csrc/q3_model.h b/qwen3_tts_axera_russian_amd/csrc/q3_model.h
--- a/qwen3_tts_axera_russian_amd/csrc/q3_model.h
+++ b/qwen3_tts_axera_russian_amd/csrc/q3_model.h
@@ -87,6 +87,7 @@
     const int* tiles = nullptr;
     int n_tiles = 0;
     bool skip_qkv0 = false;
+    const CpPickArgs* pick = nullptr;
     int rows_total = 0;
 };
 
diff --git a/qwen3_tts_axera_russian_amd/csrc/q3_model.hip b/qwen3_tts_axera_russian_amd/csrc/q3_model.hip
--- a/qwen3_tts_axera_russian_amd/csrc/q3_model.hip
+++ b/qwen3_tts_axera_russian_amd/csrc/q3_model.hip
@@ -446,7 +446,8 @@
         a.eps = c.eps;
         a.y = w.qkv;
         a.ldy = qkv_ld;
-        if (!(li == 0 && rm.skip_qkv0) && launch_linear(s, a, PRO_NORM, EPI_STORE)) return -1;
+        const bool pick0 = li == 0 && rm.pick;
+        if (!(li == 0 && rm.skip_qkv0) && !pick0 && launch_linear(s, a, PRO_NORM, EPI_STORE)) return -1;
         AttnArgs t;
         t.qkv = w.qkv;
         t.ld = qkv_ld;
@@ -478,7 +479,13 @@
         }
         t.valid_mod = rm.valid_mod;
         t.valid_n = rm.valid_n;
-        if (rm.same_slot_rows && R > 1) {
+        if (pick0) {
+            if (rm.same_slot_rows) {
+                Q3_LOG("run_stack: the pick form serves rows that do not share a slot");
+                return -1;
+            }
+            if (launch_cp_pick_attn(s, t, *rm.pick)) return -1;
+        } else if (rm.same_slot_rows && R > 1) {
             if (launch_attn(s, t, ATTN_PREP)) return -1;
             if (rm.tiles && rm.n_tiles > 0) {
                 t.tiles = rm.tiles;
diff --git a/qwen3_tts_axera_russian_amd/csrc/q3_pick.h b/qwen3_tts_axera_russian_amd/csrc/q3_pick.h
--- /dev/null
+++ b/qwen3_tts_axera_russian_amd/csrc/q3_pick.h
@@ -0,0 +1,78 @@
+#pragma once
+#include "q3_kdev.h"
+
+namespace q3 {
+
+__device__ __forceinline__ float nan_as_inf(float l) { return l != l ? INFINITY : l; }
+
+struct CpDecision {
+    int id;
+    int f;
+    int* fc;
+    const int* fz;
+    bool keep;
+};
+
+template <class Draw>
+__device__ __forceinline__ CpDecision cp_decide(const float4& l0, const float4& l1, const float4* lg, int n4, int V, int nf_r,
+                                                int frame_cap, int RT, int r, int group, int* codes, const int* forced,
+                                                int held, bool record, float* sv, int* si, Draw&& draw) {
+    const int tid = threadIdx.x;
+    float best = -INFINITY;
+    int bidx = 0x7fffffff;
+    {
+        const float e[8] = {nan_as_inf(l0.x), nan_as_inf(l0.y), nan_as_inf(l0.z), nan_as_inf(l0.w),
+                            nan_as_inf(l1.x), nan_as_inf(l1.y), nan_as_inf(l1.z), nan_as_inf(l1.w)};
+#pragma unroll
+        for (int j = 0; j < 8; j++) {
+            const int idx = (j < 4 ? tid : tid + 256) * 4 + (j & 3);
+            if (e[j] > best) {
+                best = e[j];
+                bidx = idx;
+            }
+        }
+    }
+    for (int v4 = tid + 512; v4 < n4; v4 += 256) {
+        const float4 l = lg[v4];
+        const float e[4] = {nan_as_inf(l.x), nan_as_inf(l.y), nan_as_inf(l.z), nan_as_inf(l.w)};
+#pragma unroll
+        for (int j = 0; j < 4; j++)
+            if (e[j] > best) {
+                best = e[j];
+                bidx = v4 * 4 + j;
+            }
+    }
+    group_argmax_down<64>(best, bidx);
+    if ((tid & 63) == 0) {
+        sv[tid >> 6] = best;
+        si[tid >> 6] = bidx;
+    }
+    __syncthreads();
+    best = sv[0];
+    bidx = si[0];
+#pragma unroll
+    for (int i = 1; i < 4; i++)
+        if (sv[i] > best || (sv[i] == best && si[i] < bidx)) {
+            best = sv[i];
+            bidx = si[i];
+        }
+    draw(best, bidx);
+    if (bidx < 0 || bidx >= V) bidx = 0;
+    int f = nf_r - 1;
+    if (f < 0) f = 0;
+    CpDecision d;
+    d.keep = f < frame_cap;
+    if (!d.keep) f = frame_cap - 1;
+    d.f = f;
+    d.fc = codes + ((size_t)f * RT + r) * 16;
+    if (held) {
+        bidx = d.fc[1 + group];
+        if (bidx < 0 || bidx >= V) bidx = 0;
+    } else if (record && d.keep) d.fc[1 + group] = bidx;
+    d.fz = (forced && d.keep) ? forced + ((size_t)f * RT + r) * 16 : nullptr;
+    if (d.fz && d.fz[1 + group] >= 0) bidx = d.fz[1 + group];
+    d.id = bidx;
+    return d;
+}
+
+}
diff --git a/qwen3_tts_axera_russian_amd/csrc/q3_sample.hip b/qwen3_tts_axera_russian_amd/csrc/q3_sample.hip
--- a/qwen3_tts_axera_russian_amd/csrc/q3_sample.hip
+++ b/qwen3_tts_axera_russian_amd/csrc/q3_sample.hip
@@ -1,4 +1,5 @@
 #include "q3_kdev.h"
+#include "q3_pick.h"
 
 namespace q3 {
 
@@ -28,8 +29,6 @@
     z = z ^ (z >> 31);
     return (float)(z >> 40) * (1.0f / 16777216.0f);
 }
-
-__device__ __forceinline__ float nan_as_inf(float l) { return l != l ? INFINITY : l; }
 
 constexpr int SAMPLE_SEL_CAP = 64;
 constexpr int SAMPLE_SORT_CAP = 4096;
@@ -193,9 +192,12 @@
 __device__ __forceinline__ SlotParams uniform_slot(const SlotParams* p, int r) { return uniform_entry(p, r); }
 __device__ __forceinline__ SlotRules uniform_rules(const SlotRules* p, int r) { return uniform_entry(p, r); }
 
-template <bool SLOTS, bool RULES = false, bool SCORES = false>
+template <bool SLOTS, bool RULES = false, bool SCORES = false, bool BITMAP = !SLOTS>
 __device__ __forceinline__ void talker_sample_row(const TalkerSampleArgs& a) {
     Q3_TL(42);
+    constexpr bool GATHER = BITMAP && !SLOTS && !RULES && !SCORES;
+    __shared__ unsigned wbits[BITMAP ? SAMPLE_SORT_CAP / 32 : 1];
+    __shared__ int emb_id;
     __shared__ float sv[16];
     __shared__ int si[16];
     __shared__ float sc_wm[SCORES ? 16 : 1], sc_ws[SCORES ? 16 : 1];
@@ -243,10 +245,20 @@
             if (rep_window == 0) seen_row = a.seen + (size_t)r * ((a.audio_vocab + 31) / 32);
         }
     }
+    const bool use_bits = BITMAP && a.V <= SAMPLE_SORT_CAP;
+    if constexpr (BITMAP)
+        if (use_bits && threadIdx.x < SAMPLE_SORT_CAP / 32) wbits[threadIdx.x] = 0u;
     if (threadIdx.x == 0) nwin = np < rep_window ? np : rep_window;
+    int wtok = -1;
     if (threadIdx.x < rep_window && threadIdx.x < np) {
-        win[threadIdx.x] = a.past[r * 32 + ((np - 1 - threadIdx.x) & 31)];
-    }
+        wtok = a.past[r * 32 + ((np - 1 - threadIdx.x) & 31)];
+        win[threadIdx.x] = wtok;
+    }
+    if constexpr (BITMAP)
+        if (use_bits) {
+            __syncthreads();
+            if (wtok >= 0 && wtok < a.V) atomicOr(&wbits[wtok >> 5], 1u << (wtok & 31));
+        }
     __syncthreads();
     double progress = 0.0;
     float boost = 0.f;
@@ -287,7 +299,9 @@
             else if (nt > 0 && progress > 0.8 && add_boost) l += boost;
         }
         bool rep = false;
-        for (int i = 0; i < nw_; i++) rep |= (win[i] == v);
+        if (BITMAP && use_bits) rep = (wbits[v >> 5] >> (v & 31)) & 1u;
+        else
+            for (int i = 0; i < nw_; i++) rep |= (win[i] == v);
         if constexpr (RULES)
             if (seen_row && v < a.audio_vocab) rep = (seen_row[v >> 5] >> (v & 31)) & 1u;
         if (rep) l = l > 0.f ? __fdiv_rn(l, rep_penalty) : l * rep_penalty;
@@ -356,9 +370,32 @@
             a.n_past[r] = np + 1;
             a.pos[r] = a.pos0[r] + np;
         }
+        if constexpr (GATHER) {
+            if (a.emb_table) {
+                int t = keep ? (fin ? -1 : code) : (a.frame_cap > 0 ? a.codes[((size_t)(a.frame_cap - 1) * RT + r) * 16] : -1);
+                if (a.forced && a.frame_cap > 0) {
+                    const int fz = a.forced[((size_t)(keep ? f : a.frame_cap - 1) * RT + r) * 16];
+                    if (fz >= 0 && t >= 0) t = fz;
+                }
+                emb_id = t;
+            }
+        }
+    }
+    if constexpr (GATHER) {
+        if (a.emb_table) {
+            __syncthreads();
+            const int t = emb_id;
+            const bool ok = t >= 0 && t < a.emb_V;
+            for (int k4 = threadIdx.x; k4 < a.emb_H / 4; k4 += blockDim.x) {
+                float4 v = make_float4(0.f, 0.f, 0.f, 0.f);
+                if (ok) v = *(const float4*)(a.emb_table + (size_t)t * a.emb_H + k4 * 4);
+                store_row_ssq(a.emb_h, a.emb_ssq, r, a.emb_H, k4, v, a.emb_xh, a.emb_gamma);
+            }
+        }
     }
 }
 __global__ void talker_sample_kernel(TalkerSampleArgs a) { talker_sample_row<false>(a); }
+__global__ void talker_sample_kernel_window(TalkerSampleArgs a) { talker_sample_row<false, false, false, false>(a); }
 __global__ void talker_sample_kernel_slots(TalkerSampleArgs a) { talker_sample_row<true>(a); }
 __global__ void talker_sample_kernel_rules(TalkerSampleArgs a) { talker_sample_row<true, true>(a); }
 __global__ void talker_sample_kernel_scores(TalkerSampleArgs a) { talker_sample_row<false, false, true>(a); }
@@ -379,8 +416,16 @@
     return 0;
 }
 
+static int g_sample_bitmap = 1;
+int set_sample_bitmap(int on) { g_sample_bitmap = on; return 0; }
+
 int launch_talker_sample(hipStream_t s, const TalkerSampleArgs& a) {
     if (a.R <= 0) return 0;
+    if (a.emb_table && (a.slots || a.rules || a.seen || a.scores || a.text_avail || a.held || !g_sample_bitmap || !a.emb_h ||
+                        !a.emb_ssq || a.emb_H <= 0 || a.emb_H % 16 || (a.emb_xh != nullptr) != (a.emb_gamma != nullptr))) {
+        Q3_LOG("talker_sample: the folded gather needs plain mode and h / ssq of a row width that is a multiple of 16 (H %d)", a.emb_H);
+        return -1;
+    }
     if ((a.text_avail && !a.held) || ((a.text_avail || a.held) && !a.slots)) {
         Q3_LOG("talker_sample: text_avail / held need each other and per-slot mode (text_avail %p, held %p, slots %p)",
                (const void*)a.text_avail, (const void*)a.held, (const void*)a.slots);
@@ -398,7 +443,9 @@
     static void (*const kernels[2][3])(TalkerSampleArgs) = {
         {talker_sample_kernel, talker_sample_kernel_slots, talker_sample_kernel_rules},
         {talker_sample_kernel_scores, talker_sample_kernel_slots_scores, talker_sample_kernel_rules_scores}};
-    hipLaunchKernelGGL(kernels[a.scores ? 1 : 0][(a.rules || a.seen) ? 2 : a.slots ? 1 : 0], dim3(a.R), dim3(256), lds, s, a2);
+    void (*kernel)(TalkerSampleArgs) = kernels[a.scores ? 1 : 0][(a.rules || a.seen) ? 2 : a.slots ? 1 : 0];
+    if (kernel == talker_sample_kernel && !g_sample_bitmap) kernel = talker_sample_kernel_window;
+    hipLaunchKernelGGL(kernel, dim3(a.R), dim3(256), lds, s, a2);
     Q3_HIP(hipGetLastError(), -1);
     return 0;
 }
@@ -419,8 +466,6 @@
     __shared__ int si[4];
     const int r = a.row0 + blockIdx.x, tid = threadIdx.x;
     const int RT = a.R_total > 0 ? a.R_total : a.R;
-    float best = -INFINITY;
-    int bidx = 0x7fffffff;
     const float4* lg = (const float4*)(a.logits + (size_t)r * a.V);
     const int n4 = a.V / 4;
     float4 l0 = make_float4(-INFINITY, -INFINITY, -INFINITY, -INFINITY), l1 = l0;
@@ -439,96 +484,56 @@
         if (a.talker_emb && a.text_rows) text_avail = uniform_load(a.text_avail + r);
     }
     Q3_PH(0);
-    {
-        const float e[8] = {nan_as_inf(l0.x), nan_as_inf(l0.y), nan_as_inf(l0.z), nan_as_inf(l0.w),
-                            nan_as_inf(l1.x), nan_as_inf(l1.y), nan_as_inf(l1.z), nan_as_inf(l1.w)};
+    float sc_m = -INFINITY;
+    float sc_sum = 0.f;
+    __shared__ float sc_ws[SCORES ? 4 : 1];
+    extern __shared__ float slg[];
+    __shared__ float selv[64];
+    __shared__ int seli[64];
+    __shared__ float sv2[16];
+    __shared__ int si2[16];
+    const CpDecision dec = cp_decide(
+        l0, l1, lg, n4, a.V, nf_r, a.frame_cap, RT, r, a.group, a.codes, a.forced, held, tid == 0, sv, si, [&](float best, int& bidx) {
+            Q3_PH(1);
+            sc_m = best;
+            if constexpr (SCORES) {
+                const float e[8] = {nan_as_inf(l0.x), nan_as_inf(l0.y), nan_as_inf(l0.z), nan_as_inf(l0.w),
+                                    nan_as_inf(l1.x), nan_as_inf(l1.y), nan_as_inf(l1.z), nan_as_inf(l1.w)};
+                float s = 0.f;
 #pragma unroll
-        for (int j = 0; j < 8; j++) {
-            const int idx = (j < 4 ? tid : tid + 256) * 4 + (j & 3);
-            if (e[j] > best) {
-                best = e[j];
-                bidx = idx;
-            }
-        }
-    }
-    for (int v4 = tid + 512; v4 < n4; v4 += 256) {
-        const float4 l = lg[v4];
-        const float e[4] = {nan_as_inf(l.x), nan_as_inf(l.y), nan_as_inf(l.z), nan_as_inf(l.w)};
-#pragma unroll
-        for (int j = 0; j < 4; j++)
-            if (e[j] > best) {
-                best = e[j];
-                bidx = v4 * 4 + j;
-            }
-    }
-    group_argmax_down<64>(best, bidx);
-    if ((tid & 63) == 0) {
-        sv[tid >> 6] = best;
-        si[tid >> 6] = bidx;
-    }
-    __syncthreads();
-    Q3_PH(1);
-    best = sv[0];
-    bidx = si[0];
-#pragma unroll
-    for (int i = 1; i < 4; i++)
-        if (sv[i] > best || (sv[i] == best && si[i] < bidx)) {
-            best = sv[i];
-            bidx = si[i];
-        }
-    const float sc_m = best;
-    float sc_sum = 0.f;
-    if constexpr (SCORES) {
-        __shared__ float sc_ws[4];
-        const float e[8] = {nan_as_inf(l0.x), nan_as_inf(l0.y), nan_as_inf(l0.z), nan_as_inf(l0.w),
-                            nan_as_inf(l1.x), nan_as_inf(l1.y), nan_as_inf(l1.z), nan_as_inf(l1.w)};
-        float s = 0.f;
-#pragma unroll
-        for (int j = 0; j < 8; j++) s += expf(e[j] - sc_m);
-        for (int v4 = tid + 512; v4 < n4; v4 += 256) {
-            const float4 l = lg[v4];
-            s += expf(nan_as_inf(l.x) - sc_m);
-            s += expf(nan_as_inf(l.y) - sc_m);
-            s += expf(nan_as_inf(l.z) - sc_m);
-            s += expf(nan_as_inf(l.w) - sc_m);
-        }
-        s = wave_sum(s);
-        if ((tid & 63) == 0) sc_ws[tid >> 6] = s;
-        __syncthreads();
-        sc_sum = ((sc_ws[0] + sc_ws[1]) + sc_ws[2]) + sc_ws[3];
-    }
-    if (temperature > 1e-6f) {
-        extern __shared__ float slg[];
-        __shared__ float selv[64];
-        __shared__ int seli[64];
-        __shared__ float sv2[16];
-        __shared__ int si2[16];
-        __syncthreads();
-        for (int v = tid; v < a.V; v += 256) slg[v] = nan_as_inf(a.logits[(size_t)r * a.V + v]);
-        __syncthreads();
-        float u;
-        if constexpr (SLOTS) {
-            const SlotParams sp = uniform_slot(a.slots, r);
-            u = uniform01(sp.seed, sp.no_row ? 0u : (unsigned)r, (unsigned)nf_r, 1u + (unsigned)a.group);
-        } else {
-            u = uniform01(a.seed_ptr ? a.seed_ptr[r] : a.seed, (unsigned)r, (unsigned)nf_r, 1u + (unsigned)a.group);
-        }
-        float top_p = 0.f;
-        if constexpr (RULES) top_p = uniform_rules(a.rules, r).cp_top_p;
-        bidx = block_sample_topk(slg, a.V, top_k, temperature, top_p, u, sv2, si2, selv, seli);
-    }
-    if (bidx < 0 || bidx >= a.V) bidx = 0;
-    int f = nf_r - 1;
-    if (f < 0) f = 0;
-    const bool keep = f < a.frame_cap;
-    if (!keep) f = a.frame_cap - 1;
-    int* fc = a.codes + ((size_t)f * RT + r) * 16;
-    if (SLOTS && held) {
-        bidx = fc[1 + a.group];
-        if (bidx < 0 || bidx >= a.V) bidx = 0;
-    } else if (tid == 0 && keep) fc[1 + a.group] = bidx;
-    const int* fz = (a.forced && keep) ? a.forced + ((size_t)f * RT + r) * 16 : nullptr;
-    if (fz && fz[1 + a.group] >= 0) bidx = fz[1 + a.group];
+                for (int j = 0; j < 8; j++) s += expf(e[j] - sc_m);
+                for (int v4 = tid + 512; v4 < n4; v4 += 256) {
+                    const float4 l = lg[v4];
+                    s += expf(nan_as_inf(l.x) - sc_m);
+                    s += expf(nan_as_inf(l.y) - sc_m);
+                    s += expf(nan_as_inf(l.z) - sc_m);
+                    s += expf(nan_as_inf(l.w) - sc_m);
+                }
+                s = wave_sum(s);
+                if ((tid & 63) == 0) sc_ws[tid >> 6] = s;
+                __syncthreads();
+                sc_sum = ((sc_ws[0] + sc_ws[1]) + sc_ws[2]) + sc_ws[3];
+            }
+            if (temperature > 1e-6f) {
+                __syncthreads();
+                for (int v = tid; v < a.V; v += 256) slg[v] = nan_as_inf(a.logits[(size_t)r * a.V + v]);
+                __syncthreads();
+                float u;
+                if constexpr (SLOTS) {
+                    const SlotParams sp = uniform_slot(a.slots, r);
+                    u = uniform01(sp.seed, sp.no_row ? 0u : (unsigned)r, (unsigned)nf_r, 1u + (unsigned)a.group);
+                } else {
+                    u = uniform01(a.seed_ptr ? a.seed_ptr[r] : a.seed, (unsigned)r, (unsigned)nf_r, 1u + (unsigned)a.group);
+                }
+                float top_p = 0.f;
+                if constexpr (RULES) top_p = uniform_rules(a.rules, r).cp_top_p;
+                bidx = block_sample_topk(slg, a.V, top_k, temperature, top_p, u, sv2, si2, selv, seli);
+            }
+        });
+    const int bidx = dec.id, f = dec.f;
+    const bool keep = dec.keep;
+    int* const fc = dec.fc;
+    const int* const fz = dec.fz;
     if constexpr (SCORES) {
         if (a.scores && tid == 0 && keep && !(SLOTS && held)) {
             const float zu = bidx >= 0 && bidx < a.V ? nan_as_inf(a.logits[(size_t)r * a.V + bidx]) : -INFINITY;
diff --git a/qwen3_tts_axera_russian_amd/csrc/q3_test_api.hip b/qwen3_tts_axera_russian_amd/csrc/q3_test_api.hip
--- a/qwen3_tts_axera_russian_amd/csrc/q3_test_api.hip
+++ b/qwen3_tts_axera_russian_amd/csrc/q3_test_api.hip
@@ -1624,3 +1624,185 @@
             for (int c = 0; c < C; c++) outside += o.h[(size_t)r * C + c] != OP_GUARD;
     return outside ? -3 : 0;
 }
+
+extern "C" int q3t_cp_pick_case(int fused, int R, int pos, int group, const float* logits, int V, int H, const int* n_frames,
+                                int frame_cap, int* codes, const int* forced, const float* table, const float* qkv_rows,
+                                const float* gamma, const float* q_norm, const float* k_norm, float eps, const float* rope_cos,
+                                const float* rope_sin, int max_pos, uint16_t* kc, uint16_t* vc, int n_ctx, uint16_t* attn,
+                                float* h, float* ssq, uint16_t* xh) {
+    constexpr int NH = 16, NKV = 8, D = 128, LD = (NH + 2 * NKV) * D, OW = NH * D;
+    constexpr uint16_t GUARD = 0x7d5au;
+    if (R <= 0 || pos < 1 || pos > 15 || pos >= n_ctx || pos >= max_pos || group < 0 || group > 13 || V <= 0 || V % 4 || H <= 0 ||
+        H % 32 || frame_cap < 1 || !logits || !n_frames || !codes || !table || !qkv_rows || !gamma || !q_norm || !k_norm ||
+        !rope_cos || !rope_sin || !kc || !vc || !attn || !h || !ssq || !xh)
+        return -2;
+    for (int r = 0; r < R; r++)
+        if (n_frames[r] < 0) return -2;
+    const size_t nc = (size_t)frame_cap * R * 16, cache = (size_t)R * NKV * n_ctx * D;
+    const int Rp = (R + 15) / 16 * 16;
+    std::vector<uint16_t> ho((size_t)Rp * OW, GUARD);
+    DBuf dl, dnf, dcodes, dfz, dtab, dqr, dg, dqn, dkn, dcs, dsn, dkc, dvc, dout, dq;
+    if (!dl.up(logits, (size_t)R * V * 4) || !dnf.up(n_frames, (size_t)R * 4) || !dcodes.up(codes, nc * 4) ||
+        !dtab.up(table, (size_t)V * H * 4) || !dqr.up(qkv_rows, (size_t)V * LD * 4) || !dg.up(gamma, (size_t)H * 4) ||
+        !dqn.up(q_norm, D * 4) || !dkn.up(k_norm, D * 4) || !dcs.up(rope_cos, (size_t)max_pos * 64 * 4) ||
+        !dsn.up(rope_sin, (size_t)max_pos * 64 * 4) || !dkc.up(kc, cache * 2) || !dvc.up(vc, cache * 2) ||
+        !dout.up(ho.data(), ho.size() * 2) || !dq.alloc((size_t)Rp * LD * 4))
+        return -1;
+    if (forced && !dfz.up(forced, nc * 4)) return -1;
+    Q3_HIP(hipMemset(dq.p, 0, (size_t)Rp * LD * 4), -1);
+    RowOut o;
+    if (!o.init(R, H, true, true, true)) return -1;
+    AttnArgs t;
+    t.qkv = (float*)dq.p;
+    t.ld = LD;
+    t.R = R;
+    t.row0 = 0;
+    t.q_norm = (const float*)dqn.p;
+    t.k_norm = (const float*)dkn.p;
+    t.eps = eps;
+    t.rope_cos = (const float*)dcs.p;
+    t.rope_sin = (const float*)dsn.p;
+    t.slot_base = 0;
+    t.slot_stride = 1;
+    t.pos_base = pos;
+    t.pos_stride = 0;
+    t.kc = (half_t*)dkc.p;
+    t.vc = (half_t*)dvc.p;
+    t.n_ctx = n_ctx;
+    t.n_kv = NKV;
+    t.n_heads = NH;
+    t.out = (half_t*)dout.p;
+    t.scale = 1.0f / sqrtf((float)D);
+    t.threads = 256;
+    Q3_HIP(hipDeviceSynchronize(), -1);
+    if (fused) {
+        CpPickArgs p;
+        p.logits = (const float*)dl.p;
+        p.V = V;
+        p.H = H;
+        p.R_total = R;
+        p.group = group;
+        p.codes = (int*)dcodes.p;
+        p.n_frames = (const int*)dnf.p;
+        p.frame_cap = frame_cap;
+        p.forced = forced ? (const int*)dfz.p : nullptr;
+        p.table = (const float*)dtab.p;
+        p.qkv_rows = (const float*)dqr.p;
+        p.h_out = o.ph();
+        p.ssq_out = o.ps();
+        p.xh_out = o.px();
+        p.gamma_next = (const float*)dg.p;
+        t.qkv = nullptr;
+        if (launch_cp_pick_attn(nullptr, t, p)) return -1;
+    } else {
+        CpArgmaxArgs x;
+        x.logits = (const float*)dl.p;
+        x.V = V;
+        x.R = R;
+        x.R_total = R;
+        x.H = H;
+        x.group = group;
+        x.codes = (int*)dcodes.p;
+        x.n_frames = (const int*)dnf.p;
+        x.frame_cap = frame_cap;
+        x.forced = forced ? (const int*)dfz.p : nullptr;
+        x.next_table = (const float*)dtab.p;
+        x.h_out = o.ph();
+        x.ssq_out = o.ps();
+        x.xh_out = o.px();
+        x.gamma_next = (const float*)dg.p;
+        x.next_qkv = (const float*)dqr.p;
+        x.qkv_out = (float*)dq.p;
+        x.qkv_ld = LD;
+        if (launch_cp_argmax(nullptr, x) || launch_attn(nullptr, t, ATTN_FUSED)) return -1;
+    }
+    Q3_HIP(hipDeviceSynchronize(), -1);
+    Q3_HIP(hipMemcpy(codes, dcodes.p, nc * 4, hipMemcpyDeviceToHost), -1);
+    Q3_HIP(hipMemcpy(kc, dkc.p, cache * 2, hipMemcpyDeviceToHost), -1);
+    Q3_HIP(hipMemcpy(vc, dvc.p, cache * 2, hipMemcpyDeviceToHost), -1);
+    Q3_HIP(hipMemcpy(ho.data(), dout.p, ho.size() * 2, hipMemcpyDeviceToHost), -1);
+    int outside = 0;
+    for (int r = 0; r < Rp; r++)
+        for (int k = 0; k < OW; k++) {
+            if (r < R) attn[(size_t)r * OW + k] = ho[frag_idx(r, k, OW)];
+            else if (ho[frag_idx(r, k, OW)] != GUARD) outside++;
+        }
+    const int c = o.collect([&](int r) { return r < R; }, h, ssq, xh);
+    return c < 0 ? -1 : (c || outside) ? -3 : 0;
+}
+
+extern "C" int q3t_talker_sample_fold_case(int fold, const float* logits, int V, int R_total, int row0, int R, int* past,
+                                           int* n_past, const int* n_text, int* done, int* n_frames, const int* pos0, int* pos,
+                                           int* codes, int frame_cap, const int* forced, int audio_vocab, int eos, int ignore_eos,
+                                           int max_frames, float rep_penalty, float temperature, int top_k, float top_p,
+                                           unsigned long long seed, const float* emb, int emb_V, int H, const float* gamma,
+                                           float* h, float* ssq, uint16_t* xh) {
+    if (!logits || V <= 0 || R <= 0 || row0 < 0 || row0 + R > R_total || frame_cap < 1 || eos < 0 || eos >= V || !emb ||
+        emb_V <= 0 || H <= 0 || H % 32 || !gamma || !h || !ssq || !xh)
+        return -2;
+    for (int r = row0; r < row0 + R; r++)
+        if (n_frames[r] < 0 || n_past[r] < 0) return -2;
+    const size_t rt = (size_t)R_total, nc = (size_t)frame_cap * rt * 16;
+    DBuf dl, dpast, dn, dnt, ddone, dcodes, dnf, dpos0, dpos, dforced, demb, dg;
+    if (!dl.up(logits, rt * V * 4) || !dpast.up(past, rt * 32 * 4) || !dn.up(n_past, rt * 4) || !dnt.up(n_text, rt * 4) ||
+        !ddone.up(done, rt * 4) || !dcodes.up(codes, nc * 4) || !dnf.up(n_frames, rt * 4) || !dpos0.up(pos0, rt * 4) ||
+        !dpos.up(pos, rt * 4) || !demb.up(emb, (size_t)emb_V * H * 4) || !dg.up(gamma, (size_t)H * 4))
+        return -1000;
+    if (forced && !dforced.up(forced, nc * 4)) return -1000;
+    RowOut o;
+    if (!o.init(R_total, H, true, true, true)) return -1000;
+    TalkerSampleArgs a;
+    a.logits = (const float*)dl.p;
+    a.V = V;
+    a.R = R;
+    a.row0 = row0;
+    a.R_total = R_total;
+    a.audio_vocab = audio_vocab;
+    a.eos = eos;
+    a.past = (int*)dpast.p;
+    a.n_past = (int*)dn.p;
+    a.n_text = (const int*)dnt.p;
+    a.done = (int*)ddone.p;
+    a.codes = (int*)dcodes.p;
+    a.n_frames = (int*)dnf.p;
+    a.frame_cap = frame_cap;
+    a.pos0 = (const int*)dpos0.p;
+    a.pos = (int*)dpos.p;
+    a.ignore_eos = ignore_eos;
+    a.max_frames = max_frames;
+    a.rep_penalty = rep_penalty;
+    a.temperature = temperature;
+    a.top_p = top_p;
+    a.top_k = top_k;
+    a.seed = seed;
+    a.forced = forced ? (const int*)dforced.p : nullptr;
+    Q3_HIP(hipDeviceSynchronize(), -1000);
+    int rc;
+    if (fold) {
+        a.emb_table = (const float*)demb.p;
+        a.emb_V = emb_V;
+        a.emb_H = H;
+        a.emb_h = o.ph();
+        a.emb_ssq = o.ps();
+        a.emb_xh = o.px();
+        a.emb_gamma = (const float*)dg.p;
+        rc = launch_talker_sample(nullptr, a);
+    } else {
+        set_sample_bitmap(0);
+        rc = launch_talker_sample(nullptr, a);
+        set_sample_bitmap(1);
+        if (!rc)
+            rc = launch_gather_embed(nullptr, (const float*)demb.p, emb_V, H, (const int*)dcodes.p, 0, (const int*)dnf.p, frame_cap,
+                                     0, o.ph(), o.ps(), R, row0, R_total, a.forced, o.px(), (const float*)dg.p);
+    }
+    if (rc) return rc;
+    Q3_HIP(hipDeviceSynchronize(), -1000);
+    Q3_HIP(hipMemcpy(past, dpast.p, rt * 32 * 4, hipMemcpyDeviceToHost), -1000);
+    Q3_HIP(hipMemcpy(n_past, dn.p, rt * 4, hipMemcpyDeviceToHost), -1000);
+    Q3_HIP(hipMemcpy(done, ddone.p, rt * 4, hipMemcpyDeviceToHost), -1000);
+    Q3_HIP(hipMemcpy(n_frames, dnf.p, rt * 4, hipMemcpyDeviceToHost), -1000);
+    Q3_HIP(hipMemcpy(pos, dpos.p, rt * 4, hipMemcpyDeviceToHost), -1000);
+    Q3_HIP(hipMemcpy(codes, dcodes.p, nc * 4, hipMemcpyDeviceToHost), -1000);
+    const int c = o.collect([&](int r) { return r >= row0 && r < row0 + R; }, h, ssq, xh);
+    return c < 0 ? -1000 : c ? -3 : 0;
+}
diff --git a/qwen3_tts_axera_russian_amd/hiplib.py b/qwen3_tts_axera_russian_amd/hiplib.py
--- a/qwen3_tts_axera_russian_amd/hiplib.py
+++ b/qwen3_tts_axera_russian_amd/hiplib.py
@@ -312,6 +312,11 @@
     _sig(lib, "q3t_enc_stream_unfold_case", c_int, [f32p, c_int, c_int, c_int, c_int, c_int, c_int, c_int, c_int, c_int, c_int, f32p, c_int,
                                                     i32p, i32p, f32p])
     _sig(lib, "q3t_enc_stream_emit_case", c_int, [f32p, c_int, c_int, c_int, c_int, i32p, c_int, f32p])
+    _sig(lib, "q3t_cp_pick_case", c_int, [c_int, c_int, c_int, c_int, f32p, c_int, c_int, i32p, c_int, i32p, i32p, f32p, f32p,
+                                          f32p, f32p, f32p, c_float, f32p, f32p, c_int, u16p, u16p, c_int, u16p, f32p, f32p, u16p])
+    _sig(lib, "q3t_talker_sample_fold_case", c_int, [c_int, f32p, c_int, c_int, c_int, c_int, i32p, i32p, i32p, i32p, i32p, i32p,
+                                                     i32p, i32p, c_int, i32p, c_int, c_int, c_int, c_int, c_float, c_float, c_int,
+                                                     c_float, u64, f32p, c_int, c_int, f32p, f32p, f32p, u16p])
     _test_lib = lib
     return lib
 
```

Result: faster. 10720 codec_frames/s, median of 6 (+1.3%).
